# rabbitmq/ra

Measured on AMD Instinct MI355X. Metric: append_entries decisions/sec across N Raft groups; achieved HBM GB/s vs peak, higher is better.
Workload: dtype u64

## Files before the change

ra_amd/csrc/rgb_api.hip:

```cpp
#include <hip/hip_runtime.h>

#include <atomic>
#include <chrono>
#include <condition_variable>
#include <cstdio>
#include <cstdlib>
#include <cstring>
#include <memory>
#include <mutex>
#include <thread>
#include <new>
#include <vector>

#if defined(__x86_64__)
#include <emmintrin.h>
#endif

#include "rgb_internal.h"
#include "../../include/ra_gpu_batch_synth.h"

#define RGB_STREAM_COPY_MIN (1u << 20)
#ifndef RGB_COPY_STREAM_MIN
#define RGB_COPY_STREAM_MIN (2u << 20)
#endif
// ... 209 lines not shown
  if (s.d_res) (void)hipFree(s.d_res);
  if (s.h_stamps) (void)hipHostFree(s.h_stamps);
  if (s.d_stamps) (void)hipFree(s.d_stamps);
  if (s.h_plan) (void)hipHostFree(s.h_plan);
  if (s.d_plan) (void)hipFree(s.d_plan);
  if (s.h_rows) (void)hipHostFree(s.h_rows);
  if (s.d_rows) (void)hipFree(s.d_rows);
  if (s.d_ctl) (void)hipFree(s.d_ctl);
  if (s.h_ranges) (void)hipHostFree(s.h_ranges);
  if (s.d_ranges) (void)hipFree(s.d_ranges);
  s.h_ranges = s.d_ranges = nullptr; s.ranges_cap = 0;
  if (s.h_touched) (void)hipHostFree(s.h_touched);
  if (s.d_touched) (void)hipFree(s.d_touched);
  if (s.d_undo) (void)hipFree(s.d_undo);
  if (s.done) (void)hipEventDestroy(s.done);
  if (s.copied) (void)hipEventDestroy(s.copied);
  s.copied = nullptr;
  s.h_msgs = nullptr; s.h_dec = nullptr; s.d_msgs = nullptr; s.d_dec = nullptr; s.d_rpcs = nullptr; s.h_rpcs = nullptr;
  s.h_nrpc = nullptr; s.d_res = nullptr;
  s.h_stamps = s.d_stamps = nullptr; s.h_plan = s.d_plan = nullptr; s.h_rows = s.d_rows = nullptr; s.done = nullptr;
  s.d_ctl = nullptr; s.h_touched = s.d_touched = nullptr; s.d_undo = nullptr;
  s.h_pos = s.d_pos = nullptr;
}

void rgb_close(rgb_ctx *ctx) {
  if (!ctx) return;
  if (ctx->stream) (void)hipStreamSynchronize(ctx->stream);
  rgb_wal_release(ctx);
  rgb_seg_release(ctx);
  for (u32 k = 0; k < ctx->ring_size; ++k) free_slot(ctx->ring_mem[k]);
  if (ctx->dev.dbg_buf) (void)hipFree(ctx->dev.dbg_buf);
  if (ctx->dev.hot) (void)hipFree(ctx->dev.hot);
  if (ctx->dev.peers) (void)hipFree(ctx->dev.peers);
  if (ctx->dev.runs) (void)hipFree(ctx->dev.runs);
  if (ctx->dev.cond) (void)hipFree(ctx->dev.cond);
  if (ctx->dev.qry) (void)hipFree(ctx->dev.qry);
  if (ctx->dev.seq) (void)hipFree(ctx->dev.seq);
  if (ctx->d_stage) (void)hipFree(ctx->d_stage);
  if (ctx->h_stage) (void)hipHostFree(ctx->h_stage);
  if (ctx->d_rows) (void)hipFree(ctx->d_rows);
  if (ctx->d_sums) (void)hipFree(ctx->d_sums);
  if (ctx->lb_stream) { (void)hipStreamSynchronize(ctx->lb_stream); (void)hipStreamDestroy(ctx->lb_stream); }
  if (ctx->copy_stream) { (void)hipStreamSynchronize(ctx->copy_stream); (void)hipStreamDestroy(ctx->copy_stream); }
  if (ctx->d_lb_gather) (void)hipFree(ctx->d_lb_gather);
  if (ctx->h_lb_pinned) (void)hipHostFree(ctx->h_lb_pinned);
  if (ctx->lb_event) (void)hipEventDestroy(ctx->lb_event);
  if (ctx->d_synth) (void)hipFree(ctx->d_synth);
  if (ctx->d_synth_sent) (void)hipFree(ctx->d_synth_sent);
  if (ctx->d_train_ctl) (void)hipFree(ctx->d_train_ctl);
  if (ctx->d_seq_cnt) (void)hipFree(ctx->d_seq_cnt);

  if (ctx->stream) (void)hipStreamDestroy(ctx->stream);
  delete ctx;
}

int rgb_open(const rgb_config *cfg_in, rgb_ctx **out) {
  if (!out) return RGB_E_INVAL;
  *out = nullptr;
  rgb_config cfg;
  if (cfg_in) cfg = *cfg_in; else rgb_default_config(&cfg);
  if (cfg.abi_version != RGB_ABI_VERSION) return RGB_E_INVAL;
  if (cfg.max_runs < 2 || cfg.max_runs > RGB_MAX_RUNS) return RGB_E_INVAL;
  if (cfg.ring_slots < 1 || cfg.ring_slots > 64 || cfg.ring_capacity < 1) return RGB_E_INVAL;
  if (cfg.max_pipeline_count == 0) cfg.max_pipeline_count = RGB_DEFAULT_MAX_PIPELINE_COUNT;
  if (cfg.max_aer_batch == 0) cfg.max_aer_batch = RGB_AER_CHUNK_SIZE;
  if (cfg.max_aer_batch > 65535) return RGB_E_INVAL;
  int ndev = 0;
  hipError_t e = hipGetDeviceCount(&ndev);
  if (e != hipSuccess || ndev <= 0) return RGB_E_NODEVICE;
  if (cfg.device < 0 || cfg.device >= ndev) return RGB_E_INVAL;
  rgb_ctx *ctx = new (std::nothrow) rgb_ctx();
  if (!ctx) return RGB_E_NOMEM;
  ctx->cfg = cfg;
  memset(&ctx->dev, 0, sizeof ctx->dev);
  e = hipSetDevice(cfg.device);
  if (e == hipSuccess) e = hipStreamCreateWithFlags(&ctx->stream, hipStreamNonBlocking);
  if (e == hipSuccess) e = hipStreamCreateWithFlags(&ctx->copy_stream, hipStreamNonBlocking);

  if (e != hipSuccess) { delete ctx; return RGB_E_HIP; }
  *out = ctx;
  return RGB_OK;
}

uint32_t rgb_n_servers(const rgb_ctx *ctx) { return ctx ? ctx->dev.n_servers : 0; }

static int alloc_slot(rgb_ctx *ctx, rgb_slot &s) {
  const u32 cap = ctx->cfg.ring_capacity;
  HIPCHK(ctx, hipHostMalloc((void **)&s.h_msgs, (size_t)cap * (sizeof(rgb_msg) + sizeof(u32)), hipHostMallocDefault));
  HIPCHK(ctx, hipHostMalloc((void **)&s.h_dec, (size_t)cap * sizeof(rgb_decision), hipHostMallocDefault));
  HIPCHK(ctx, hipMalloc((void **)&s.d_msgs, (size_t)cap * (sizeof(rgb_msg) + sizeof(u32))));
  HIPCHK(ctx, hipMalloc((void **)&s.d_dec, (size_t)cap * sizeof(rgb_decision)));
  s.h_pos = reinterpret_cast<u32 *>(s.h_msgs + cap); s.d_pos = reinterpret_cast<u32 *>(s.d_msgs + cap);
  HIPCHK(ctx, hipMalloc((void **)&s.d_rpcs, (size_t)ctx->rpc_cap * sizeof(rgb_rpc)));
  HIPCHK(ctx, hipHostMalloc((void **)&s.h_rpcs, (size_t)ctx->rpc_cap * sizeof(rgb_rpc), hipHostMallocDefault));
  HIPCHK(ctx, hipEventCreateWithFlags(&s.done, hipEventDisableTiming));
  HIPCHK(ctx, hipEventCreateWithFlags(&s.copied, hipEventDisableTiming));
  HIPCHK(ctx, hipHostMalloc((void **)&s.h_nrpc, 64, hipHostMallocDefault));
  HIPCHK(ctx, hipMalloc((void **)&s.d_res, ((size_t)rgb_results_blocks(cap) + 1u) * sizeof(u32)));
  HIPCHK(ctx, hipMemsetAsync(s.d_res, 0, ((size_t)rgb_results_blocks(cap) + 1u) * sizeof(u32), ctx->stream));
  HIPCHK(ctx, hipHostMalloc((void **)&s.h_stamps, cap, hipHostMallocDefault));
  HIPCHK(ctx, hipMalloc((void **)&s.d_stamps, cap));
  HIPCHK(ctx, hipHostMalloc((void **)&s.h_plan, RGB_SUBMIT_TRAIN_ROUNDS * sizeof(rgb_train_tick), hipHostMallocDefault));
  HIPCHK(ctx, hipMalloc((void **)&s.d_plan, RGB_SUBMIT_TRAIN_ROUNDS * sizeof(rgb_train_tick)));
  s.rows_cap = (cap / 32u + 2u * RGB_N_CLASSES * RGB_SUBMIT_TRAIN_ROUNDS + 64u);
  HIPCHK(ctx, hipHostMalloc((void **)&s.h_rows, (size_t)s.rows_cap * RGB_SUBMIT_TRAIN_ROUNDS * sizeof(u32), hipHostMallocDefault));
  HIPCHK(ctx, hipMalloc((void **)&s.d_rows, (size_t)s.rows_cap * RGB_SUBMIT_TRAIN_ROUNDS * sizeof(u32)));
  HIPCHK(ctx, hipMalloc((void **)&s.d_ctl, RGB_TRAIN_CTL_WORDS * sizeof(u32)));
  HIPCHK(ctx, hipMemsetAsync(s.d_ctl, 0, RGB_TRAIN_CTL_WORDS * sizeof(u32), ctx->stream));
  HIPCHK(ctx, hipHostMalloc((void **)&s.h_touched, (size_t)cap * sizeof(u32), hipHostMallocDefault));
  HIPCHK(ctx, hipMalloc((void **)&s.d_touched, (size_t)cap * sizeof(u32)));
  return RGB_OK;
}

int rgb_upload_state(rgb_ctx *ctx, uint32_t first, uint32_t n, const rgb_server_state *in);

int rgb_register_groups(rgb_ctx *ctx, uint32_t n_groups, uint32_t n_members) {
  if (!ctx) return RGB_E_INVAL;
  if (ctx->registered) return RGB_E_STATE;
  if (n_members < 1 || n_members > RGB_MAX_MEMBERS || n_groups < 1) return RGB_E_INVAL;
  const uint64_t S64 = (uint64_t)n_groups * n_members;
  if (S64 > 0x7FFFFFFFull) return RGB_E_INVAL;
  const u32 S = (u32)S64;
  HIPCHK(ctx, hipSetDevice(ctx->cfg.device));
  rgb_dev &d = ctx->dev;
  d.n_servers = S; d.n_members = n_members; d.max_runs = ctx->cfg.max_runs;
  d.peer_stride = rgb_peer_stride(n_members);
  d.max_pipeline_count = ctx->cfg.max_pipeline_count;
  d.max_aer_batch = ctx->cfg.max_aer_batch;
  d.dbg = 0; d.dbg_buf = nullptr;
  d.synth_hint = ctx->synth_hint;
  d.fuse_pipeline = (ctx->cfg.flags & RGB_CFG_FUSE_PIPELINE) ? 1u : 0u;
  d.seq_ranges = nullptr; d.n_seq_ranges = 0;
#ifdef RGB_PROFILE
  { const char *e = getenv("RGB_DEBUG"); d.dbg = e ? (u32)atoi(e) : 0u; }
  if (d.dbg & 16u) {
    HIPCHK(ctx, hipMalloc((void **)&d.dbg_buf, (size_t)(S / 64 + 16) * 8 * sizeof(u64)));
    HIPCHK(ctx, hipMemsetAsync(d.dbg_buf, 0, (size_t)(S / 64 + 16) * 8 * sizeof(u64), ctx->stream));
  }
#endif
#ifdef RGB_X_DECLINE_HIST
  HIPCHK(ctx, hipMalloc((void **)&d.dbg_buf, 128 * sizeof(u64)));
  HIPCHK(ctx, hipMemsetAsync(d.dbg_buf, 0, 128 * sizeof(u64), ctx->stream));
#endif
#ifdef RGB_X_TRAIN_TIMELINE
  HIPCHK(ctx, hipMalloc((void **)&d.dbg_buf, (size_t)(1u << 20) * 8 * sizeof(u64)));
  HIPCHK(ctx, hipMemsetAsync(d.dbg_buf, 0, (size_t)(1u << 20) * 8 * sizeof(u64), ctx->stream));
#endif
  HIPCHK(ctx, hipMalloc((void **)&d.hot, (size_t)S * RGB_HOT_WORDS * sizeof(u64)));
  HIPCHK(ctx, hipMalloc((void **)&d.peers, (size_t)S * d.peer_stride * sizeof(u64)));
  HIPCHK(ctx, hipMalloc((void **)&d.runs, (size_t)S * d.max_runs * 2 * sizeof(u64)));
  HIPCHK(ctx, hipMalloc((void **)&d.cond, (size_t)S * 4 * sizeof(u64)));
  HIPCHK(ctx, hipMalloc((void **)&d.qry, (size_t)S * RGB_QRY_WORDS * sizeof(u64)));
  HIPCHK(ctx, hipMemsetAsync(d.runs, 0, (size_t)S * d.max_runs * 2 * sizeof(u64), ctx->stream));
  d.seq_stride = (((n_groups + RGB_TRAIN_SHARDS - 1u) / RGB_TRAIN_SHARDS) * n_members * RGB_SEQ_SPREAD + 255u) & ~255u;
  HIPCHK(ctx, hipMalloc((void **)&d.seq, (size_t)d.seq_stride * RGB_TRAIN_SHARDS));
  HIPCHK(ctx, hipMemsetAsync(d.seq, 0, (size_t)d.seq_stride * RGB_TRAIN_SHARDS, ctx->stream));
  ctx->stage_cap = S < 16384u ? S : 16384u;
  HIPCHK(ctx, hipMalloc((void **)&ctx->d_stage, (size_t)ctx->stage_cap * sizeof(rgb_server_state)));
  HIPCHK(ctx, hipHostMalloc((void **)&ctx->h_stage, (size_t)ctx->stage_cap * sizeof(rgb_server_state),
                            hipHostMallocDefault));
  HIPCHK(ctx, hipMalloc((void **)&ctx->d_rows, (size_t)n_groups * sizeof(rgb_leaderboard_row)));
  HIPCHK(ctx, hipMalloc((void **)&ctx->d_sums, (size_t)S * sizeof(u64)));
  ctx->rpc_stride = n_members > 1 ? n_members - 1 : 1;
  ctx->rpc_cap = ctx->cfg.ring_capacity * ctx->rpc_stride;
  ctx->ring_mem.reset(new (std::nothrow) rgb_slot[ctx->cfg.ring_slots]);
  if (!ctx->ring_mem) return RGB_E_NOMEM;
  ctx->ring_size = ctx->cfg.ring_slots;
  for (u32 k = 0; k < ctx->ring_size; ++k) {
    rgb_slot &s = ctx->ring_mem[k];
    int rc = alloc_slot(ctx, s);
    if (rc) return rc;
  }
  ctx->registered = true;
  std::vector<rgb_server_state> init(ctx->stage_cap);
  for (u32 base = 0; base < S; base += ctx->stage_cap) {
    u32 cnt = S - base < ctx->stage_cap ? S - base : ctx->stage_cap;
    for (u32 k = 0; k < cnt; ++k) {
      rgb_server_state &h = init[k];
      memset(&h, 0, sizeof h);
      h.snapshot_index = RGB_UNDEF; h.snapshot_term = RGB_UNDEF;
      h.pending_first = 1;
      for (unsigned i = 0; i < n_members; ++i) h.next_index[i] = 1;
      h.role = RGB_ROLE_FOLLOWER; h.self = (uint8_t)((base + k) % n_members);
      h.n_members = (uint8_t)n_members; h.voted_for = RGB_NONE; h.leader_id = RGB_NONE;
      h.cond_leader = RGB_NONE; h.n_runs = 1;
      h.present_mask = (uint8_t)((1u << n_members) - 1u); h.voter_mask = h.present_mask;
      h.status_mask = 0xFF;
    }
    int rc = rgb_upload_state(ctx, base, cnt, init.data());
    if (rc) return rc;
  }
  return RGB_OK;
}

static int validate_state(const rgb_ctx *ctx, const rgb_server_state &h) {
  if (h.n_members != ctx->dev.n_members) return RGB_E_INVAL;
  if (h.self >= RGB_MAX_MEMBERS) return RGB_E_INVAL;
  if (h.role > RGB_ROLE_AWAIT_CONDITION || h.cond_reason > RGB_COND_TRANSFER_LEADERSHIP) return RGB_E_INVAL;
  if (h.n_runs > RGB_MAX_RUNS || h.votes > 15) return RGB_E_INVAL;
  if (h.voted_for != RGB_NONE && h.voted_for >= RGB_MAX_MEMBERS) return RGB_E_INVAL;
  if (h.leader_id != RGB_NONE && h.leader_id >= RGB_MAX_MEMBERS) return RGB_E_INVAL;
  if (h.cond_leader != RGB_NONE && h.cond_leader >= RGB_MAX_MEMBERS) return RGB_E_INVAL;
  if (h.first_index <= h.last_index) {
    if (h.n_runs == 0 || h.run_start[0] != h.first_index) return RGB_E_INVAL;
    for (unsigned r = 1; r < h.n_runs; ++r)
      if (!(h.run_start[r] > h.run_start[r - 1] && h.run_start[r] <= h.last_index)) return RGB_E_INVAL;
    if (h.run_term[h.n_runs - 1] != h.last_term) return RGB_E_INVAL;
  }
  if (h.n_pending_old > 2) return RGB_E_INVAL;
  uint64_t above = h.pending_first;
  for (int k = (int)h.n_pending_old - 1; k >= 0; --k) {
    const uint64_t s = h.pending_old[k][0], e = h.pending_old[k][1];
    if (s > e || e == RGB_UNDEF || !(e + 1 < above)) return RGB_E_INVAL;
    above = s;
  }
  return RGB_OK;
}

int rgb_upload_state(rgb_ctx *ctx, uint32_t first, uint32_t n, const rgb_server_state *in) {
  if (!ctx || (!in && n)) return RGB_E_INVAL;
  if (!ctx->registered) return RGB_E_STATE;
  if ((uint64_t)first + n > ctx->dev.n_servers) return RGB_E_INVAL;
  for (u32 k = 0; k < n; ++k) {
    int rc = validate_state(ctx, in[k]);
    if (rc) return rc;
  }
  HIPCHK(ctx, hipSetDevice(ctx->cfg.device));
  rgb_stream_turn turn(ctx);
  if (turn.rc) return turn.rc;
  for (u32 base = 0; base < n; base += ctx->stage_cap) {
    u32 cnt = n - base < ctx->stage_cap ? n - base : ctx->stage_cap;
    memcpy(ctx->h_stage, in + base, (size_t)cnt * sizeof(rgb_server_state));
    HIPCHK(ctx, hipMemcpyAsync(ctx->d_stage, ctx->h_stage, (size_t)cnt * sizeof(rgb_server_state),
                               hipMemcpyHostToDevice, ctx->stream));
    int rc = rgb_launch_pack(ctx->dev, ctx->d_stage, first + base, cnt, ctx->stream);
    if (rc) { ctx->last_hip.store(rc, std::memory_order_relaxed); return RGB_E_HIP; }
    HIPCHK(ctx, hipStreamSynchronize(ctx->stream));
  }
  return RGB_OK;
}

int rgb_download_state(rgb_ctx *ctx, uint32_t first, uint32_t n, rgb_server_state *out) {
  if (!ctx || (!out && n)) return RGB_E_INVAL;
  if (!ctx->registered) return RGB_E_STATE;
  if ((uint64_t)first + n > ctx->dev.n_servers) return RGB_E_INVAL;
  HIPCHK(ctx, hipSetDevice(ctx->cfg.device));
  rgb_stream_turn turn(ctx);
  if (turn.rc) return turn.rc;
  for (u32 base = 0; base < n; base += ctx->stage_cap) {
    u32 cnt = n - base < ctx->stage_cap ? n - base : ctx->stage_cap;
    int rc = rgb_launch_unpack(ctx->dev, ctx->d_stage, first + base, cnt, ctx->stream);
    if (rc) { ctx->last_hip.store(rc, std::memory_order_relaxed); return RGB_E_HIP; }
    HIPCHK(ctx, hipMemcpyAsync(ctx->h_stage, ctx->d_stage, (size_t)cnt * sizeof(rgb_server_state),
                               hipMemcpyDeviceToHost, ctx->stream));
    HIPCHK(ctx, hipStreamSynchronize(ctx->stream));
    memcpy(out + base, ctx->h_stage, (size_t)cnt * sizeof(rgb_server_state));
  }
  return RGB_OK;
}

static int validate_msg(const rgb_ctx *ctx, const rgb_msg &m) {
  if (m.kind > RGB_MSG_KIND_MAX) return RGB_E_INVAL;
  if (m.kind == RGB_MSG_NOP) return RGB_OK;
  if (m.server >= ctx->dev.n_servers) return RGB_E_INVAL;
  if (m.from != RGB_NONE && m.from >= RGB_MAX_MEMBERS) return RGB_E_INVAL;
  if (m.kind == RGB_MSG_AER && m.n_run0 > m.n_entries) return RGB_E_INVAL;
  if (m.kind == RGB_MSG_WRITTEN && m.a > m.b) return RGB_E_INVAL;
  if (m.kind == RGB_MSG_WRITTEN && (m.flags & RGB_MF_SEQ2) &&
      !(m.run0_term <= m.run1_term && m.run1_term != RGB_UNDEF && m.run1_term + 1 < m.a)) return RGB_E_INVAL;
  if (m.kind == RGB_MSG_WRITTEN && (m.flags & RGB_MF_SEQX) && !(m.flags & RGB_MF_SEQ2)) return RGB_E_INVAL;
  return RGB_OK;
}
static int validate_seqx(const rgb_msg &m, const uint64_t *ranges, uint32_t n_ranges) {
  if (m.kind != RGB_MSG_WRITTEN || !(m.flags & RGB_MF_SEQX)) return RGB_OK;
  if (!ranges || m.n_entries == 0 || m.c > n_ranges || (uint64_t)m.c + m.n_entries > n_ranges) return RGB_E_INVAL;
  uint64_t prev_last = 0; bool have = false;
  for (uint32_t k = 0; k < m.n_entries; ++k) {
    const uint64_t f = ranges[2 * (m.c + k)], l = ranges[2 * (m.c + k) + 1];
    if (f > l || l == RGB_UNDEF || (have && !(prev_last + 1 < f))) return RGB_E_INVAL;
    prev_last = l; have = true;
  }
  return prev_last + 1 < m.run0_term ? RGB_OK : RGB_E_INVAL;
}

static int train_scratch(rgb_ctx *ctx);

#define RGB_FAULT_STAMP 1u
#define RGB_FAULT_SHARD 2u

static rgb_dev slot_dev(const rgb_ctx *ctx, const rgb_slot &s) {
  rgb_dev d = ctx->dev;
  d.seq_ranges = s.n_ranges ? s.d_ranges : nullptr;
  d.n_seq_ranges = s.n_ranges;
  return d;
}

static int enqueue_rounds(rgb_ctx *ctx, rgb_slot &s) {
  const rgb_dev dv = slot_dev(ctx, s);
  auto fail = [&](int lr) { ctx->last_hip.store(lr, std::memory_order_relaxed); return RGB_E_HIP; };
  for (u32 r = 0; r < s.n_rounds; ++r) {
    const u32 off = s.round_start[r], cnt = s.round_start[r + 1] - s.round_start[r];
    u32 cc[RGB_N_CLASSES], real = 0, before_written = 0;
    for (int c = 0; c < RGB_N_CLASSES; ++c) {
      cc[c] = s.round_cc[(size_t)r * RGB_N_CLASSES + c];
      real += cc[c];
      if (c < 2) before_written += cc[c];
// ... 1043 lines not shown
```

ra_amd/csrc/rgb_internal.h:

```cpp
#ifndef RGB_INTERNAL_H
#define RGB_INTERNAL_H

#include <stdint.h>
#include "../../include/ra_gpu_batch.h"

typedef unsigned long long u64;
typedef uint32_t u32;

#define RGB_HOT_WORDS 16
#define RGB_QRY_WORDS 16

#define HOT_CT    0
#define HOT_PK    1
#define HOT_LRT   2
#define HOT_PRS   3
#define HOT_CI    4
#define HOT_LA    5
#define HOT_LI    6
#define HOT_LT    7
#define HOT_SI    8
#define HOT_ST    9
#define HOT_FIRST 10
#define HOT_LRS   11
#define HOT_LWI   12
#define HOT_LWT   13
#define HOT_PRT   14
#define HOT_PEND  15
#define HOT_P_TERM  0
#define HOT_P_LRT   1
#define HOT_P_CI    2
#define HOT_P_LI    3
#define HOT_P_SI    4
#define HOT_P_FIRST 5
#define HOT_P_LW    6
#define HOT_P_PEND  7
#define PEER_MI(i, N) (2u * (unsigned)(i))
#define PEER_NI(i, N) (2u * (unsigned)(i) + 1u)
#define PEER_CS(i, N) (2u * (unsigned)(N) + (unsigned)(i))

#define PK_ROLE_SH      0
#define PK_COND_SH      3
#define PK_SELF_SH      5
#define PK_VOTES_SH     9
#define PK_NRUNS_SH     13
#define PK_NONVOTER_SH  18
#define PK_CONDTO_SH    19
#define PK_VOTED_SH     20
#define PK_LEADER_SH    24
#define PK_CONDLDR_SH   28
#define PK_PRESENT_SH   32
#define PK_VOTER_SH     40
#define PK_STATUS_SH    48
#define PK_QSELF_SH     56
#define PK_QPEER_SH     57
#define PK_BACKOFF_SH   58
#define PK_PENDX_SH     59
static inline __host__ __device__ unsigned pk_cond_reason(u64 pk) {
  const unsigned c = (unsigned)((pk >> PK_COND_SH) & 3ull), to = (unsigned)((pk >> PK_CONDTO_SH) & 1ull);
  return to == 0u ? c : c == RGB_COND_WAL_DOWN ? (unsigned)RGB_COND_WAL_DOWN_LEADER : (unsigned)RGB_COND_TRANSFER_LEADERSHIP;
}
static inline __host__ __device__ u64 pk_with_cond_reason(u64 pk, unsigned reason) {
  const u64 c = reason == RGB_COND_WAL_DOWN_LEADER ? (u64)RGB_COND_WAL_DOWN : reason == RGB_COND_TRANSFER_LEADERSHIP ? 0ull : (u64)reason;
  const u64 to = (reason == RGB_COND_WAL_DOWN_LEADER || reason == RGB_COND_TRANSFER_LEADERSHIP) ? 1ull : 0ull;
  return (pk & ~((3ull << PK_COND_SH) | (1ull << PK_CONDTO_SH))) | (c << PK_COND_SH) | (to << PK_CONDTO_SH);
}
#define QRY_PEND_LO     12
#define QRY_PEND_HI     14
#define QRY_BACKOFF     9
#define QRY_TOKEN       10
#define QRY_MACVER      11

#define RGB_N_CLASSES 15
static inline __host__ __device__ unsigned rgb_kind_rank(unsigned kind) {
  switch (kind) {
    case RGB_MSG_AER: return 0;
    case RGB_MSG_AER_REPLY: return 1;
    case RGB_MSG_WRITTEN: return 2;
    case RGB_MSG_APPEND: return 3;
    case RGB_MSG_PIPELINE_RPCS: return 4;
    case RGB_MSG_REQUEST_VOTE: return 5;
    case RGB_MSG_VOTE_RESULT: return 6;
    case RGB_MSG_AWAIT_TIMEOUT: return 7;
    case RGB_MSG_ELECTION_TIMEOUT: return 8;
    case RGB_MSG_PRE_VOTE_RPC: return 9;
    case RGB_MSG_PRE_VOTE_RESULT: return 10;
    case RGB_MSG_SNAPSHOT_WRITTEN: return 11;
    case RGB_MSG_HEARTBEAT_RPC: return 12;
    case RGB_MSG_HEARTBEAT_REPLY: return 13;
    case RGB_MSG_CONSISTENT_QUERY: return 14;
    case RGB_MSG_TRANSFER_LEADERSHIP: return 14;
    default: return 15;
  }
}
#define RGB_N_FAMILIES 32
static inline __host__ __device__ unsigned rgb_family(unsigned kind, unsigned flags) {
  return 2u * rgb_kind_rank(kind) + ((flags & RGB_MF_SUCCESS) ? 1u : 0u);
}
static inline unsigned rgb_class_of_kind(unsigned kind) { return rgb_kind_rank(kind); }

#define RGB_TRAIN_SHARDS 8u
#define RGB_N_BUCKETS ((RGB_N_CLASSES + 1u) * RGB_TRAIN_SHARDS * 2u)
#define RGB_TRAIN_CTL_WORDS (320u + 32u * 64u)
static inline __host__ __device__ unsigned rgb_shard_of_server(unsigned server, unsigned n_members) {
  return (server / n_members) & (RGB_TRAIN_SHARDS - 1u);
}
static inline __host__ __device__ unsigned rgb_bucket(unsigned kind, unsigned flags, unsigned server, unsigned n_members) {
  return (rgb_kind_rank(kind) * RGB_TRAIN_SHARDS + rgb_shard_of_server(server, n_members)) * 2u +
         ((flags & RGB_MF_SUCCESS) ? 1u : 0u);
}
static inline __host__ __device__ unsigned rgb_bucket_hinted(unsigned kind, unsigned flags, unsigned server,
                                                             unsigned n_members, bool off_steady) {
  const bool hinted_kind = kind == RGB_MSG_WRITTEN || kind == RGB_MSG_AER;
  return rgb_bucket(kind, flags, server, n_members) | ((hinted_kind && off_steady) ? 1u : 0u);
}
#ifndef RGB_SEQ_SPREAD
#define RGB_SEQ_SPREAD 1u
#endif
static inline __host__ __device__ unsigned rgb_seq_index(unsigned server, unsigned n_members, unsigned seq_stride) {
  const unsigned g = server / n_members, m = server - g * n_members;
  return (g & (RGB_TRAIN_SHARDS - 1u)) * seq_stride + ((g / RGB_TRAIN_SHARDS) * n_members + m) * RGB_SEQ_SPREAD;
}
#define RGB_TRAIN_MAX_TICKS 255u
#define RGB_N_PCLASSES (2u * RGB_N_CLASSES)
#define RGB_PC_SNAP RGB_N_PCLASSES
#define RGB_SNAP_LEAD 0.5f
struct rgb_train_tick {
  u32 n_rows;
  u32 msg_base;
  u32 snap;
  u32 pad[13];
  u32 off[RGB_N_PCLASSES][RGB_TRAIN_SHARDS];
  u32 cnt[RGB_N_PCLASSES][RGB_TRAIN_SHARDS];
};
#define RGB_SYNTH_FIXED_WORDS (RGB_N_FAMILIES + 2u * RGB_N_BUCKETS)
u32 rgb_synth_scratch_words(u32 n_groups);

static inline __host__ __device__ unsigned rgb_peer_stride(unsigned n_members) {
  return (3u * n_members + 7u) & ~7u;
}

struct rgb_dev {
  u64 *hot;
  u64 *peers;
  u64 *runs;
  u64 *cond;
  u64 *qry;
  u32 n_servers;
  u32 n_members;
  u32 max_runs;
  u32 peer_stride;
  u32 max_pipeline_count;
  u32 max_aer_batch;
  unsigned char *seq;
  u32 seq_stride;
  const u64 *seq_ranges;
  u32 n_seq_ranges;
  u32 fuse_pipeline;
  u32 synth_hint;
  u32 dbg;
  u64 *dbg_buf;
};

#define RGB_TICK_CLS_WRITTEN_SEQX 32
#define RGB_TICK_CLS_NOP 33
int rgb_launch_tick(const rgb_dev &dev, int cls, const rgb_msg *d_msgs, u32 n, const u32 *d_n,
                    rgb_decision *d_dec, rgb_rpc *d_rpcs, u32 rpc_slot_base, u32 msg_index_base, void *stream);
int rgb_launch_tick_classes(const rgb_dev &dev, const rgb_msg *d_msgs, const u32 counts[RGB_N_CLASSES],
                            const u32 *d_family_totals, u32 max_msgs, rgb_decision *d_dec, rgb_rpc *d_rpcs,
                            u32 rpc_slot_base, u32 msg_index_base, void *stream);
int rgb_launch_synth(const rgb_dev &dev, u64 seed, u64 tick, rgb_msg *d_msgs, u32 *d_scratch,
                     u32 *d_kind_counts, u32 *d_n, u32 *d_bucket_counts, unsigned char *d_stamps, unsigned char *d_sent,
                     void *stream);
int rgb_launch_train(const rgb_dev &dev, const rgb_msg *d_msgs, const unsigned char *d_stamps, u32 tick_stride,
                     const rgb_train_tick *d_plan, const u32 *d_row_tab, u32 n_ticks, u32 bpt, rgb_decision *d_dec,
                     rgb_rpc *d_rpcs, u32 rpc_ring, u32 index_base, u32 *d_ctl, u32 n_xcc, u32 n_blocks, void *stream,
                     const unsigned char *d_snap_stamps = nullptr, rgb_leaderboard_row *d_snap_rows = nullptr,
                     u32 tab_rpt = 0 );
u32 rgb_train_resident_blocks(unsigned n_members);
int rgb_launch_train_verify(u32 *d_ctl, void *stream);
int rgb_launch_train_seq(const rgb_dev &dev, const rgb_msg *d_msgs, u32 n, unsigned char *d_seq_cnt,
                         unsigned char *d_stamps, void *stream);
int rgb_launch_train_calibrate(u32 *d_out, void *stream);
u32 rgb_train_make_tick(const u32 *bucket_counts, unsigned n_members, rgb_train_tick *out, u32 *row_tab, u32 row_cap,
                        u32 snap_rows = 0);
int rgb_launch_train_plan(const u32 *d_bucket_counts, rgb_train_tick *d_ticks, u32 *d_rows, u32 rpt, u32 first_tick,
                          u32 n_ticks, u32 snapshot_every, u32 n_groups, u32 n_members, u32 *d_err, void *stream);
u32 rgb_train_rows_bound(u32 n_servers, u32 n_members, bool with_snapshot);
static inline u32 rgb_train_snap_rows(u32 n_groups) {
  return ((n_groups + RGB_TRAIN_SHARDS - 1u) / RGB_TRAIN_SHARDS + 63u) / 64u;
}
int rgb_launch_seq_bump(unsigned char *d_seq, unsigned char *d_out, u32 n_bytes, void *stream);
int rgb_launch_pack(const rgb_dev &dev, const rgb_server_state *d_in, u32 first, u32 n, void *stream);
int rgb_launch_unpack(const rgb_dev &dev, rgb_server_state *d_out, u32 first, u32 n, void *stream);
int rgb_launch_leaderboard(const rgb_dev &dev, rgb_leaderboard_row *d_rows, void *stream);
int rgb_launch_checksum(const rgb_dev &dev, u32 first, u32 n, u64 *d_out, void *stream);
int rgb_launch_stamp_rounds(const rgb_dev &dev, const rgb_msg *d_msgs, u32 n, unsigned char *d_stamps, void *stream);
u32 rgb_results_blocks(u32 n);
int rgb_launch_results(const rgb_decision *d_dec, const u32 *d_pos, u32 n, u32 cap, const rgb_rpc *d_rpcs, u32 rpc_stride, u32 *d_scratch,
                       const u32 *d_ctl, rgb_decision *out_dec, rgb_rpc *out_rpcs, u32 *out_hdr, void *stream);
u32 rgb_undo_pieces(const rgb_dev &dev);
int rgb_launch_undo(const rgb_dev &dev, const u32 *d_ids, u32 n, void *d_undo, u32 restore, void *stream);

#endif
```

ra_amd/csrc/rgb_kernels.hip:

```cpp
#include <hip/hip_runtime.h>
#include "rgb_internal.h"

#define UNDEF 0xFFFFFFFFFFFFFFFFull
#define SLOT_NONE4 0xFu

#ifdef RGB_PROFILE
#define RGB_KNOB(dev, bit) (((dev).dbg & (bit)) != 0)
#else
#define RGB_KNOB(dev, bit) false
#endif

#ifndef RGB_TICK_BLOCK
#define RGB_TICK_BLOCK 64
#endif
#ifndef RGB_CLASS_MIN_WAVES
#define RGB_CLASS_MIN_WAVES(N) ((N) <= 5 ? 4 : 3)
#endif
#ifndef RGB_MIN_WAVES
#define RGB_MIN_WAVES(N) 2
#endif

namespace {

#ifndef RGB_X_LEAD32
#define RGB_X_LEAD32 1
#endif
__host__ __device__ constexpr bool rgb_lead_class(int c) { return c == 1 || c == 3 || c == 4; }
#ifndef RGB_X_HINT
#define RGB_X_HINT 1
#endif
#ifndef RGB_X_HALFMSG
#define RGB_X_HALFMSG 1
#endif
__host__ __device__ constexpr bool rgb_half_msg_class(int c) {
  return RGB_X_HALFMSG && (c == 2 || c == 4 || c == 5 || c == 6 || c == 7 || c == 11 || c == 12 || c == 13 || c == 14);
}
__host__ __device__ __forceinline__ constexpr u32 rgb_class_slice(int c, unsigned n_members) {
  return (RGB_X_LEAD32 && rgb_lead_class(c) && ((3u * n_members + 7u) & ~7u) == 16u) ? 32u : (u32)RGB_TICK_BLOCK;
}
#ifndef RGB_X_NORPC
#define RGB_X_NORPC 0
#endif
#ifndef RGB_X_LEAD32_WIDE
#define RGB_X_LEAD32_WIDE 1
#endif
#ifndef RGB_TRAIN_RUNS_LDS
#define RGB_TRAIN_RUNS_LDS 1
#endif
__host__ __device__ __forceinline__ constexpr bool rgb_wide_peers(unsigned n_members) { return ((3u * n_members + 7u) & ~7u) == 24u; }
__host__ __device__ __forceinline__ constexpr u32 rgb_train_class_slice(int c, unsigned n_members) {
  return (RGB_X_LEAD32 && RGB_X_LEAD32_WIDE && RGB_TRAIN_RUNS_LDS && rgb_lead_class(c) && rgb_wide_peers(n_members)) ? 32u
                                                                                                                  : rgb_class_slice(c, n_members);
}


__device__ __forceinline__ void store16_nt(void *p, ulonglong2 v) {
  typedef unsigned v4u __attribute__((ext_vector_type(4)));
  v4u d;
  d.x = (unsigned)v.x; d.y = (unsigned)(v.x >> 32); d.z = (unsigned)v.y; d.w = (unsigned)(v.y >> 32);
  __builtin_nontemporal_store(d, reinterpret_cast<v4u *>(p));
}
#define ST16(ptr, val) do { *(ptr) = (val); } while (0)
#define ST8(ptr, val) do { *(ptr) = (val); } while (0)

#ifndef RGB_X_RPC_ST8
#define RGB_X_RPC_ST8 0
#endif
typedef unsigned long long rgb_u64x2_a8 __attribute__((ext_vector_type(2), aligned(8)));
__device__ __forceinline__ void store_rpc(rgb_rpc *slot, u64 w0, u64 w1, u64 w2, u64 w3, u64 w4, u64 w5, u64 w6) {
  u64 *o = reinterpret_cast<u64 *>(slot);
#if RGB_X_RPC_ST8 || defined(RGB_HOST_EMULATION)
  ST8(o + 0, w0); ST8(o + 1, w1); ST8(o + 2, w2); ST8(o + 3, w3); ST8(o + 4, w4); ST8(o + 5, w5); ST8(o + 6, w6);
#else
  rgb_u64x2_a8 a, b, c;
  a.x = w0; a.y = w1; b.x = w2; b.y = w3; c.x = w4; c.y = w5;
  *reinterpret_cast<rgb_u64x2_a8 *>(o + 0) = a;
  *reinterpret_cast<rgb_u64x2_a8 *>(o + 2) = b;
  *reinterpret_cast<rgb_u64x2_a8 *>(o + 4) = c;
  ST8(o + 6, w6);
#endif
}
#ifndef RGB_X_RPC_DEFER
#define RGB_X_RPC_DEFER 1
#endif
template <class Lane>
__device__ __forceinline__ void emit_rpc(Lane &L, rgb_rpc *rpcs, u32 slot_base, unsigned ord, u32 msg_index, u64 w1,
                                         u64 rp_idx, u64 rp_term, u64 new_ni) {
  if (rpcs == nullptr || RGB_X_NORPC) return;
  if (RGB_X_RPC_DEFER && L.rpc_stash != nullptr && ord < 4u) {
    L.rpc_stash[2u * ord] = make_ulonglong2(w1, rp_idx);
    L.rpc_stash[2u * ord + 1u] = make_ulonglong2(rp_term, new_ni);
    return;
  }
  store_rpc(rpcs + (size_t)slot_base + ord, (u64)msg_index | ((u64)L.server << 32), w1, L.ct, rp_idx, rp_term, L.ci, new_ni);
}

#if defined(RGB_X_MARK) && !defined(RGB_HOST_EMULATION)
#define RGB_MARK(what, rank) asm volatile("; RGB_MARK " what " %0" ::"n"(rank));
#else
#define RGB_MARK(what, rank)
#endif

enum { GLDS_DEFAULT = 0, GLDS_NT = 2, GLDS_SC1 = 16 };
template <int POLICY>
__device__ __forceinline__ void glds16(const void *g, void *lds_base) {
#ifdef RGB_HOST_EMULATION
  memcpy(static_cast<char *>(lds_base) + 16 * emu::lane(), g, 16);
#else
  __builtin_amdgcn_global_load_lds((const __attribute__((address_space(1))) void *)g,
                                   (__attribute__((address_space(3))) void *)lds_base, 16, 0, POLICY);
#endif
}
__device__ __forceinline__ void glds_wait() {
#ifndef RGB_HOST_EMULATION
  __builtin_amdgcn_s_waitcnt(0x0F70);
  asm volatile("" ::: "memory");
#endif
}

__device__ __forceinline__ void lds_barrier() {
#ifdef RGB_HOST_EMULATION
  __syncthreads();
#else
  __builtin_amdgcn_fence(__ATOMIC_RELEASE, "workgroup", "local");
  __builtin_amdgcn_s_barrier();
  __builtin_amdgcn_fence(__ATOMIC_ACQUIRE, "workgroup", "local");
#endif
}

typedef unsigned long long v2u64 __attribute__((ext_vector_type(2)));
template <bool NT>
__device__ __forceinline__ ulonglong2 ld16(const ulonglong2 *p) {
  if (NT) {
    v2u64 v = __builtin_nontemporal_load(reinterpret_cast<const v2u64 *>(p));
    return make_ulonglong2(v.x, v.y);
  }
  return *p;
}

__device__ __forceinline__ u64 ldg8(bool coh, const u64 *p) {
#ifndef RGB_HOST_EMULATION
  if (coh) return __hip_atomic_load(p, __ATOMIC_RELAXED, __HIP_MEMORY_SCOPE_AGENT);
#endif
  return *p;
}
__device__ __forceinline__ ulonglong2 ldg16(bool coh, const ulonglong2 *p) {
#ifndef RGB_HOST_EMULATION
  if (coh) {
    const u64 *q = reinterpret_cast<const u64 *>(p);
    const u64 x = __hip_atomic_load(q, __ATOMIC_RELAXED, __HIP_MEMORY_SCOPE_AGENT);
    const u64 y = __hip_atomic_load(q + 1, __ATOMIC_RELAXED, __HIP_MEMORY_SCOPE_AGENT);
    return make_ulonglong2(x, y);
  }
#endif
  return *p;
}

__device__ __forceinline__ u64 pk_get(u64 pk, int sh, int w) { return (pk >> sh) & ((1ull << w) - 1ull); }
__device__ __forceinline__ u64 pk_set(u64 pk, int sh, int w, u64 v) {
  const u64 m = ((1ull << w) - 1ull) << sh;
  return (pk & ~m) | ((v << sh) & m);
}
__device__ __forceinline__ unsigned slot8to4(unsigned s) { return s >= 8u ? SLOT_NONE4 : s; }
__device__ __forceinline__ unsigned slot4to8(unsigned s) { return s >= 8u ? (unsigned)RGB_NONE : s; }

template <bool COH, bool WC = false, bool SEQX = false>
struct LaneT {
  static constexpr bool coh = COH;
  static constexpr bool seqx_ok = SEQX;
  static constexpr bool walk_cache = WC;
  int wc_k;
  u64 wc_start, wc_term, wc_next;
  u64 ct, ci, la, li, lt, lwi, lwt, pk, si, st, first, lrs, lrt, prs, prt, pend;
  u64 token, macver;
  u32 server, n_entries, n_run0;
  unsigned kind, from, mflags, gap;
  u64 term, a, b, c, run0_term, run1_term;
  const u64 *seqx;
  u32 n_seqx;
  const u64 *runs;
  u64 *peers;
  const ulonglong2 *peers_lds;
  unsigned peers_swz;
  const ulonglong2 *runs_lds;
  ulonglong2 *rpc_stash;
  u32 max_runs;
  u32 flags;
  u32 inv;
  bool has_reply;
  unsigned reply_to;
  u64 r_term, r_next, r_last, r_lterm;
  u64 w_first, w_last;
  bool vote_reqs;
  unsigned n_runs;
  unsigned push_cnt;
  bool cond_dirty;
  u64 cr0, cr1, cr2, cr3;
  u64 po_floor, po_cut;
  u64 pmi[8], pni[8], pcs[8];
  unsigned dmi, dni, dcs;
  unsigned pdirty;
  unsigned dcs_ci;
  bool peers_loaded;
  u64 *qry_base;
  u64 qself, qp[8];
  bool q_loaded;
  unsigned q_dirty;
  unsigned hb_mask;
  unsigned cancel_mask;
#ifdef RGB_X_DECLINE_HIST
  const u64 *dbg_hist;
#endif
#ifdef RGB_PROFILE
  unsigned prof_nloads;
  bool prof_noprobe;
#endif
  u64 hb_term, hb_qi, q_consensus;
};

template <int N, class Lane>
__device__ __forceinline__ void load_peers(Lane &L) {
  if (L.peers_loaded) return;
  constexpr int PS = (3 * N + 7) & ~7;
  u64 w[PS];
  if ((PS == 16 || PS == 24) && L.peers_lds != nullptr) {
    const unsigned sw = PS == 24 ? L.peers_swz << 1 : L.peers_swz;
#pragma unroll
    for (int k = 0; k < PS / 2; ++k) {
      if (2 * k < 3 * N) { ulonglong2 v = L.peers_lds[(unsigned)k ^ sw]; w[2 * k] = v.x; w[2 * k + 1] = v.y; }
    }
  } else {
    const ulonglong2 *pp = reinterpret_cast<const ulonglong2 *>(L.peers);
#pragma unroll
    for (int k = 0; k < PS / 2; ++k) {
      if (2 * k < 3 * N) { ulonglong2 v = ldg16(L.coh, pp + k); w[2 * k] = v.x; w[2 * k + 1] = v.y; }
    }
  }
#pragma unroll
  for (int i = 0; i < N; ++i) { L.pmi[i] = w[PEER_MI(i, N)]; L.pni[i] = w[PEER_NI(i, N)]; L.pcs[i] = w[PEER_CS(i, N)]; }
  L.peers_loaded = true;
}

template <int N>
__device__ __forceinline__ u64 peer_get(const u64 (&a)[8], unsigned p) {
  u64 r = 0;
#pragma unroll
  for (int i = 0; i < N; ++i) r = ((unsigned)i == p) ? a[i] : r;
  return r;
}
template <int N>
__device__ __forceinline__ void peer_set(u64 (&a)[8], unsigned &dirty, unsigned p, u64 v) {
#pragma unroll
  for (int i = 0; i < N; ++i)
    if ((unsigned)i == p) { a[i] = v; dirty |= 1u << i; }
}

template <class Lane>
__device__ __forceinline__ unsigned prow_at(const Lane &L, unsigned w) { return (((w >> 1) ^ L.peers_swz) << 1) | (w & 1u); }
template <class Lane>
__device__ __forceinline__ u64 prow_get(const Lane &L, unsigned w) {
  return reinterpret_cast<const u64 *>(L.peers_lds)[prow_at(L, w)];
}
template <class Lane>
__device__ __forceinline__ void prow_set(Lane &L, unsigned w, u64 v) {
  const_cast<u64 *>(reinterpret_cast<const u64 *>(L.peers_lds))[prow_at(L, w)] = v;
  L.pdirty |= 1u << w;
}
template <int N, bool PL, class Lane> __device__ __forceinline__ u64 mi_get(const Lane &L, int i) { return PL ? prow_get(L, PEER_MI(i, N)) : L.pmi[i]; }
template <int N, bool PL, class Lane> __device__ __forceinline__ u64 ni_get(const Lane &L, int i) { return PL ? prow_get(L, PEER_NI(i, N)) : L.pni[i]; }
template <int N, bool PL, class Lane> __device__ __forceinline__ u64 cs_get(const Lane &L, int i) { return PL ? prow_get(L, PEER_CS(i, N)) : L.pcs[i]; }
template <int N, bool PL, class Lane> __device__ __forceinline__ void ni_set(Lane &L, int i, u64 v) {
  if (PL) prow_set(L, PEER_NI(i, N), v); else { L.pni[i] = v; L.dni |= 1u << i; }
}
template <int N, bool PL, class Lane> __device__ __forceinline__ u64 mi_of(const Lane &L, unsigned p) { return PL ? (p < (unsigned)N ? prow_get(L, PEER_MI(p, N)) : 0) : peer_get<N>(L.pmi, p); }
template <int N, bool PL, class Lane> __device__ __forceinline__ u64 ni_of(const Lane &L, unsigned p) { return PL ? (p < (unsigned)N ? prow_get(L, PEER_NI(p, N)) : 0) : peer_get<N>(L.pni, p); }
template <int N, bool PL, class Lane> __device__ __forceinline__ void mi_put(Lane &L, unsigned p, u64 v) {
  if (PL) { if (p < (unsigned)N) prow_set(L, PEER_MI(p, N), v); } else peer_set<N>(L.pmi, L.dmi, p, v);
}
template <int N, bool PL, class Lane> __device__ __forceinline__ void ni_put(Lane &L, unsigned p, u64 v) {
  if (PL) { if (p < (unsigned)N) prow_set(L, PEER_NI(p, N), v); } else peer_set<N>(L.pni, L.dni, p, v);
}

template <class Lane>
__device__ __forceinline__ bool range_nonempty(const Lane &L) { return L.first <= L.li; }

#define RGB_RUNS_LDS 8
#ifndef RGB_TRAIN_RUNS_LDS
#define RGB_TRAIN_RUNS_LDS 1
#endif
template <class Lane>
__device__ __forceinline__ ulonglong2 run_pair(const Lane &L, int k) {
  if (L.runs_lds != nullptr && k < RGB_RUNS_LDS) return L.runs_lds[(unsigned)k ^ L.peers_swz];
  return ldg16(L.coh, reinterpret_cast<const ulonglong2 *>(L.runs) + k);
}
template <class Lane>
__device__ __forceinline__ u64 run_word(const Lane &L, int i) {
#ifdef RGB_PROFILE
  const_cast<Lane &>(L).prof_nloads += 1;
#endif
  if (L.runs_lds != nullptr && i < 2 * RGB_RUNS_LDS) {
    const ulonglong2 v = L.runs_lds[(unsigned)(i >> 1) ^ L.peers_swz];
    return (i & 1) ? v.y : v.x;
  }
  return ldg8(L.coh, L.runs + i);
}

template <class Lane>
__device__ __forceinline__ int run_search(const Lane &L, u64 idx, u64 &term) {
  int k = (int)L.n_runs - 3;
  if (k < 0) return -1;
  if (Lane::walk_cache && L.wc_k >= 0 && L.wc_k <= k && idx >= L.wc_start && idx < L.wc_next) {
    term = L.wc_term;
    return L.wc_k;
  }
  ulonglong2 cur = run_pair(L, k);
  u64 upper = L.prs;
#pragma unroll 1
  for (; k >= 0; --k) {
    const ulonglong2 nxt = run_pair(L, k > 0 ? k - 1 : 0);
#ifdef RGB_PROFILE
    const_cast<Lane &>(L).prof_nloads += 2u;
#endif
    if (idx >= cur.x) {
      term = cur.y;
      if (Lane::walk_cache) {
        Lane &M = const_cast<Lane &>(L);
        M.wc_k = k; M.wc_start = cur.x; M.wc_term = cur.y; M.wc_next = upper;
      }
      return k;
    }
    upper = cur.x;
    cur = nxt;
  }
  return -1;
}

template <class Lane>
__device__ __forceinline__ u64 fetch_term(const Lane &L, u64 idx) {
  if (!(range_nonempty(L) && idx >= L.first && idx <= L.li)) return UNDEF;
  if (idx >= L.lrs) return L.lrt;
#ifdef RGB_PROFILE
  if (L.prof_noprobe) return L.lrt;
#endif
  if (L.n_runs >= 2 && idx >= L.prs) return L.prt;
  u64 term = UNDEF;
  run_search(L, idx, term);
  return term;
}

template <class Lane>
__device__ __forceinline__ u64 srv_fetch_term(const Lane &L, u64 idx) {
  u64 t = fetch_term(L, idx);
  if (t == UNDEF && L.si != UNDEF && L.si == idx) return L.st;
  return t;
}

template <class Lane>
__device__ __forceinline__ int find_run(const Lane &L, u64 idx) {
  if (L.n_runs == 0) return -1;
  if (idx >= L.lrs) return (int)L.n_runs - 1;
#ifdef RGB_PROFILE
  if (L.prof_noprobe) return (int)L.n_runs - 1;
#endif
  if (L.n_runs >= 2 && idx >= L.prs) return (int)L.n_runs - 2;
  u64 term;
  return run_search(L, idx, term);
}


template <class Lane>
__device__ __forceinline__ u64 next_log_index(const Lane &L) {
  if (range_nonempty(L)) return L.li + 1;
  if (L.si != UNDEF) return L.si + 1;
  return 0;
}

enum { HLE_OK = 0, HLE_MISMATCH = 1, HLE_MISSING = 2 };
template <class Lane>
__device__ __forceinline__ int has_log_entry_or_snapshot(const Lane &L, u64 idx, u64 term) {
  u64 t = fetch_term(L, idx);
  if (t == UNDEF) {
    if (L.si != UNDEF && L.si == idx) return L.st == term ? HLE_OK : HLE_MISMATCH;
    return HLE_MISSING;
  }
  return t == term ? HLE_OK : HLE_MISMATCH;
}

template <class Lane>
__device__ __forceinline__ unsigned role_of(const Lane &L) { return (unsigned)pk_get(L.pk, PK_ROLE_SH, 3); }
template <class Lane>
__device__ __forceinline__ unsigned self_of(const Lane &L) { return (unsigned)pk_get(L.pk, PK_SELF_SH, 4); }
template <class Lane>
__device__ __forceinline__ bool present(const Lane &L, unsigned i) {
  return i < 8u && ((L.pk >> (PK_PRESENT_SH + i)) & 1ull);
}
template <class Lane>
__device__ __forceinline__ bool voter(const Lane &L, unsigned i) { return (L.pk >> (PK_VOTER_SH + i)) & 1ull; }
template <class Lane>
__device__ __forceinline__ bool status_normal(const Lane &L, unsigned i) { return (L.pk >> (PK_STATUS_SH + i)) & 1ull; }

template <class Lane>
__device__ __forceinline__ void set_role(Lane &L, unsigned role) {
  unsigned old = role_of(L);
  if (old != role) L.flags |= RGB_F_ROLE_CHANGED;
  if (role == RGB_ROLE_FOLLOWER && old != RGB_ROLE_FOLLOWER) {
    L.pk = pk_set(L.pk, PK_STATUS_SH, 8, 0xFF);
    L.pk = pk_set(L.pk, PK_BACKOFF_SH, 1, 0);
  }
  if (role != RGB_ROLE_AWAIT_CONDITION) L.pk &= ~((3ull << PK_COND_SH) | (1ull << PK_CONDTO_SH));
  L.pk = pk_set(L.pk, PK_ROLE_SH, 3, role);
}

template <class Lane>
__device__ __forceinline__ void update_term_and_voted_for(Lane &L, u64 term, unsigned voted4) {
  unsigned cur = (unsigned)pk_get(L.pk, PK_VOTED_SH, 4);
  if (term == L.ct && voted4 == cur) return;
  L.flags |= RGB_F_PERSIST;
  L.ct = term;
  L.pk = pk_set(L.pk, PK_VOTED_SH, 4, voted4);
  if (pk_get(L.pk, PK_QPEER_SH, 1)) {
    L.pk = pk_set(L.pk, PK_QPEER_SH, 1, 0);
    if (L.q_loaded) {
#pragma unroll
      for (int i = 0; i < 8; ++i) L.qp[i] = 0;
    }
  }
}

template <class Lane>
__device__ __forceinline__ u64 *qry_row(const Lane &L) { return L.qry_base + (size_t)L.server * RGB_QRY_WORDS; }

template <int N, class Lane>
__device__ __forceinline__ void load_qry(Lane &L) {
  if (L.q_loaded) return;
  const ulonglong2 *qp = reinterpret_cast<const ulonglong2 *>(qry_row(L));
  u64 w[N + 2];
#pragma unroll
  for (int k = 0; k < (N + 2) / 2; ++k) { ulonglong2 v = ldg16(L.coh, qp + k); w[2 * k] = v.x; w[2 * k + 1] = v.y; }
  L.qself = w[0];
  if (pk_get(L.pk, PK_QPEER_SH, 1)) {
#pragma unroll
    for (int i = 0; i < N; ++i) L.qp[i] = w[1 + i];
  }
  L.q_loaded = true;
}

template <class Lane>
__device__ __forceinline__ void heartbeat_reply(Lane &L, u64 term, u64 query_index, unsigned to8) {
  L.has_reply = true;
  L.flags |= RGB_F_REPLY | RGB_F_REPLY_HEARTBEAT;
  L.r_term = term; L.r_next = query_index; L.r_last = 0; L.r_lterm = 0;
  L.reply_to = to8;
}
// ... 433 lines not shown
    if (c + 1 > L.pend) L.pend = c + 1;
    pend_canon(L);
  }
  pend_old_floor(L, c + 1);
  if (first_clause) {
    changed = !(L.lwi == c && L.lwt == term);
    L.lwi = c; L.lwt = term;
  }
  return 0;
}

template <class Lane>
__device__ __forceinline__ bool log_snapshot_written(Lane &L, u64 idx, u64 term) {
  if (!(range_nonempty(L) && idx >= L.first)) return false;
  bool changed = false;
  if (!(L.lwi > idx)) {
    changed = !(L.lwi == idx && L.lwt == term);
    L.lwi = idx; L.lwt = term;
  }
  if (idx >= L.li) {
    L.li = idx; L.lt = term; L.first = idx + 1; L.n_runs = 0;
  } else {
    const u64 nf = idx + 1;
    const int k = find_run(L, nf);
    u64 *runs = const_cast<u64 *>(L.runs);
    if (k > 0) {
      ulonglong2 *rp = reinterpret_cast<ulonglong2 *>(runs);
      const int n_mem = (int)L.n_runs - 2 - k;
#ifdef RGB_X_DECLINE_HIST
      atomicAdd(const_cast<u64 *>(L.dbg_hist) + 96 + (n_mem < 0 ? 0 : n_mem > 15 ? 15 : n_mem), 1ull);
#endif
#pragma unroll 1
      for (int i = 0; i < n_mem; i += 4) {
        ulonglong2 t0 = make_ulonglong2(0, 0), t1 = t0, t2 = t0, t3 = t0;
        t0 = ldg16(L.coh, rp + k + i);
        if (i + 1 < n_mem) t1 = ldg16(L.coh, rp + k + i + 1);
        if (i + 2 < n_mem) t2 = ldg16(L.coh, rp + k + i + 2);
        if (i + 3 < n_mem) t3 = ldg16(L.coh, rp + k + i + 3);
        ST16(rp + i, t0);
        if (i + 1 < n_mem) ST16(rp + i + 1, t1);
        if (i + 2 < n_mem) ST16(rp + i + 2, t2);
        if (i + 3 < n_mem) ST16(rp + i + 3, t3);
      }
      if ((int)L.n_runs - 2 >= k) ST16(rp + (L.n_runs - 2 - (unsigned)k), make_ulonglong2(L.prs, L.prt));
      ST16(rp + (L.n_runs - 1 - (unsigned)k), make_ulonglong2(L.lrs, L.lrt));
      L.n_runs -= (unsigned)k;
    }
    if (L.n_runs > 0) runs[0] = nf;
    if (L.lrs < nf) L.lrs = nf;
    if (L.n_runs == 2) L.prs = nf;
    L.first = nf;
  }
  L.si = idx; L.st = term;
  if (idx + 1 > L.pend) L.pend = idx + 1;
  pend_old_floor(L, idx + 1);
  pend_canon(L);
  return changed;
}


template <int N>
__device__ __forceinline__ u64 agreed_commit(const u64 (&v)[N], const bool (&use)[N], int n) {
  if (n <= 0) return UNDEF;
  u64 a[N];
#pragma unroll
  for (int i = 0; i < N; ++i) a[i] = use[i] ? v[i] : 0ull;
#pragma unroll
  for (int r = 0; r < N; ++r) {
#pragma unroll
    for (int i = r & 1; i + 1 < N; i += 2) {
      const bool sw = a[i + 1] > a[i];
      const u64 hi = sw ? a[i + 1] : a[i], lo = sw ? a[i] : a[i + 1];
      a[i] = hi; a[i + 1] = lo;
    }
  }
  const int k = n / 2;
  u64 res = a[0];
#pragma unroll
  for (int i = 1; i < N; ++i) res = (k == i) ? a[i] : res;
  return res;
}

template <int N, bool PL = false, class Lane>
__device__ __forceinline__ void evaluate_quorum(Lane &L) {
  u64 v[N + 1];
  bool use[N + 1];
  const unsigned self = self_of(L);
  int n = 1;
  v[N] = L.lwi; use[N] = true;
#pragma unroll
  for (int i = 0; i < N; ++i) {
    bool u = ((unsigned)i != self) && present(L, i) && voter(L, i);
    v[i] = mi_get<N, PL>(L, i); use[i] = u;
    n += u ? 1 : 0;
  }
  const u64 ci0 = L.ci;
  u64 p = agreed_commit<N + 1>(v, use, n);
  u64 t = srv_fetch_term(L, p);
  if (t != UNDEF && t == L.ct) L.ci = p;
  if (L.ci > ci0) L.flags |= RGB_F_AUX_EVAL;
  if (apply_to(L, L.ci)) L.flags |= RGB_F_APPLIED;
}

template <int N, bool EMIT, bool PL = false, class Lane>
__device__ __forceinline__ int pipeline_rpcs(Lane &L, bool force, u32 max_pipe, u32 max_batch, bool &more,
                             unsigned &n_out, rgb_rpc *rpcs, u32 slot_base, u32 msg_index) {
  const unsigned self = self_of(L);
  const u64 next_log = next_log_index(L);
  more = false;
  n_out = 0;
#pragma unroll
  for (int i = 0; i < N; ++i) {
    if ((unsigned)i == self || !present(L, i) || !status_normal(L, i)) continue;
    const u64 mi = mi_get<N, PL>(L, i), ni = ni_get<N, PL>(L, i), cis = cs_get<N, PL>(L, i);
    if (!(ni < next_log || cis < L.ci)) continue;
    long long inflight = (long long)(ni - mi) - 1;
    if (!(inflight < (long long)max_pipe || force)) continue;
    long long room = (long long)max_pipe - inflight;
    long long bs = (long long)max_batch < room ? (long long)max_batch : room;
    if (bs < 1) bs = 1;
    u64 prev = ni - 1;
    u64 prev_term = fetch_term(L, prev);
    u64 new_ni, rp_idx, rp_term;
    unsigned kind, n_ent = 0;
    if (prev_term == UNDEF && !(L.si != UNDEF && L.si == prev)) {
      if (L.si == UNDEF || !(ni == 0 || prev < L.si)) return RGB_INV_PIPELINE_PREV_UNDEFINED;
      kind = RGB_RPC_SNAPSHOT; rp_idx = L.si; rp_term = L.st; new_ni = L.si;
      if (EMIT) L.flags |= RGB_F_SEND_SNAPSHOT;
    } else {
      if (prev_term == UNDEF) prev_term = L.st;
      u64 to = prev + (u64)bs < L.li ? prev + (u64)bs : L.li;
      kind = RGB_RPC_AER; rp_idx = prev; rp_term = prev_term;
      n_ent = (unsigned)(to >= prev + 1 ? to - prev : 0);
      new_ni = to + 1;
    }
    if (!(new_ni >= ni)) return RGB_INV_NEXT_INDEX_REGRESSED;
    n_out += 1;
    long long new_inflight = (long long)(new_ni - mi) - 1;
    if (new_ni < next_log && new_inflight < (long long)max_pipe) more = true;
    if (EMIT) {
      ni_set<N, PL>(L, i, new_ni);
      L.dcs_ci |= 1u << i;
      emit_rpc(L, rpcs, slot_base, n_out - 1u, msg_index, (u64)(unsigned)i | ((u64)kind << 8) | ((u64)(n_ent & 0xFFFFu) << 16),
               rp_idx, rp_term, new_ni);
    }
  }
  return 0;
}


template <int N, class Lane>
__device__ __forceinline__ void become_leader(Lane &L) {
  const u64 ni = next_log_index(L);
  load_peers<N>(L);
#pragma unroll
  for (int i = 0; i < N; ++i) {
    if (!present(L, i)) continue;
    L.pmi[i] = 0; L.pni[i] = ni; L.pcs[i] = 0;
    L.dmi |= 1u << i; L.dni |= 1u << i; L.dcs |= 1u << i;
  }
  L.pk = pk_set(L.pk, PK_STATUS_SH, 8, 0xFF);
  L.pk = pk_set(L.pk, PK_BACKOFF_SH, 1, 0);
  set_leader_id(L, self_of(L));
  L.pk = pk_set(L.pk, PK_VOTES_SH, 4, 0);
  set_role(L, RGB_ROLE_LEADER);
  L.flags |= RGB_F_BECAME_LEADER;
}

template <int N, class Lane>
__device__ __forceinline__ void candidate_vote_granted(Lane &L) {
  unsigned nv = (unsigned)pk_get(L.pk, PK_VOTES_SH, 4) + 1;
  if (nv == required_quorum(L)) become_leader<N>(L);
  else L.pk = pk_set(L.pk, PK_VOTES_SH, 4, nv);
}

template <class Lane>
__device__ __forceinline__ void vote_requests(Lane &L, u64 term, bool pre) {
  L.flags &= ~(u32)RGB_F_PRE_VOTE_REQS;
  L.flags |= RGB_F_SEND_VOTE_REQUESTS | (pre ? RGB_F_PRE_VOTE_REQS : 0u);
  L.has_reply = false;
  L.r_term = term; L.r_next = pre ? L.token : 0; L.r_last = L.li; L.r_lterm = L.lt;
  L.vote_reqs = true;
}

template <int N, class Lane>
__device__ __forceinline__ void call_for_election_candidate(Lane &L) {
  const u64 new_term = L.ct + 1;
  update_term_and_voted_for(L, new_term, self_of(L));
  set_leader_id(L, SLOT_NONE4);
  L.pk = pk_set(L.pk, PK_VOTES_SH, 4, 0);
  set_role(L, RGB_ROLE_CANDIDATE);
  vote_requests(L, new_term, false);
  candidate_vote_granted<N>(L);
}

template <int N, class Lane>
__device__ __forceinline__ void call_for_election_pre_vote(Lane &L, u64 token) {
  update_term_and_voted_for(L, L.ct, self_of(L));
  set_leader_id(L, SLOT_NONE4);
  L.pk = pk_set(L.pk, PK_VOTES_SH, 4, 0);
  L.token = token;
  set_role(L, RGB_ROLE_PRE_VOTE);
  vote_requests(L, L.ct, true);
  if (!pk_get(L.pk, PK_NONVOTER_SH, 1)) {
    unsigned nv = (unsigned)pk_get(L.pk, PK_VOTES_SH, 4) + 1;
    if (nv == required_quorum(L)) call_for_election_candidate<N>(L);
    else L.pk = pk_set(L.pk, PK_VOTES_SH, 4, nv);
  }
}

template <class Lane>
__device__ __forceinline__ int process_pre_vote(Lane &L) {
  const u64 token = L.c;
  if (L.term >= L.ct) {
    update_term(L, L.term);
    const bool up = (L.b > L.lt) || (L.b == L.lt && L.a >= L.li);
    const u32 theirs = L.n_entries, ours = (u32)(L.macver & 0xFFFFFFFFull), eff = (u32)(L.macver >> 32);
    if (up && L.gap > RGB_PROTO_VERSION) {
      pre_vote_reply(L, L.term, token, false, L.from);
    } else if (up && (theirs == eff || (theirs >= eff && theirs <= ours))) {
      pre_vote_reply(L, L.term, token, true, L.from);
    } else if (up) {
      pre_vote_reply(L, L.term, token, false, L.from);
      L.flags |= RGB_F_START_ELECTION_TIMEOUT;
    } else if (role_of(L) == RGB_ROLE_FOLLOWER) {
      L.flags |= RGB_F_START_ELECTION_TIMEOUT;
    } else {
      pre_vote_reply(L, L.term, token, false, L.from);
    }
    return 0;
  }
  pre_vote_reply(L, L.ct, token, false, L.from);
  return 0;
}

template <int N, bool PL = false, class Lane>
__device__ __forceinline__ int make_all_rpcs(Lane &L, unsigned &n_out, rgb_rpc *rpcs, u32 slot_base,
                                             u32 msg_index, bool only_stale = false) {
  const unsigned self = self_of(L);
  update_heartbeat_rpc_effects<N>(L);
  if (!PL) load_peers<N>(L);
  n_out = 0;
  unsigned backoff = 0;
  if (!only_stale && pk_get(L.pk, PK_BACKOFF_SH, 1)) backoff = (unsigned)ldg8(L.coh, qry_row(L) + QRY_BACKOFF) & 0xFFu;
#pragma unroll
  for (int i = 0; i < N; ++i) {
    if ((unsigned)i == self || !present(L, i)) continue;
    if (!status_normal(L, i)) {
      if (!((backoff >> i) & 1u)) continue;
      L.cancel_mask |= 1u << i;
      L.flags |= RGB_F_CANCEL_SNAPSHOT_RETRY;
    }
    const u64 ni_i = ni_get<N, PL>(L, i);
    if (only_stale && !(mi_get<N, PL>(L, i) + 1 < ni_i || cs_get<N, PL>(L, i) < L.ci)) continue;
    const u64 prev = ni_i - 1;
    u64 prev_term = fetch_term(L, prev);
    u64 rp_idx, rp_term, new_ni;
    unsigned kind, n_ent = 0;
    if (prev_term == UNDEF && !(L.si != UNDEF && L.si == prev)) {
      if (L.si == UNDEF || !(ni_i == 0 || prev < L.si)) return RGB_INV_PIPELINE_PREV_UNDEFINED;
      kind = RGB_RPC_SNAPSHOT; rp_idx = L.si; rp_term = L.st; new_ni = L.si;
      L.flags |= RGB_F_SEND_SNAPSHOT;
    } else {
      if (prev_term == UNDEF) prev_term = L.st;
      u64 to = prev + 1 < L.li ? prev + 1 : L.li;
      kind = RGB_RPC_AER; rp_idx = prev; rp_term = prev_term;
      n_ent = (unsigned)(to >= prev + 1 ? to - prev : 0);
      new_ni = to + 1;
    }
    n_out += 1;
    emit_rpc(L, rpcs, slot_base, n_out - 1u, msg_index, (u64)(unsigned)i | ((u64)kind << 8) | ((u64)(n_ent & 0xFFFFu) << 16),
             rp_idx, rp_term, new_ni);
  }
  return 0;
}


template <class Lane>
__device__ __forceinline__ u32 drop_existing(const Lane &L) {
  if (L.n_entries == 0) return 0;
  const u64 base = L.a + 1 + (u64)L.gap;
  if (!range_nonempty(L) || base > L.li || base < L.first) return 0;
  u32 k = 0;
  for (int seg = 0; seg < 2; ++seg) {
    u32 cnt = seg == 0 ? L.n_run0 : L.n_entries - L.n_run0;
    if (seg == 0 && cnt > L.n_entries) cnt = L.n_entries;
    if (cnt == 0) continue;
    u64 s = base + k, e = s + cnt - 1;
    u64 t = seg == 0 ? L.run0_term : L.run1_term;
    if (s > L.li) return k;
    int r = find_run(L, s);
    if (r < 0) return k;
    const bool cached = Lane::walk_cache && r == L.wc_k;
    u64 rterm = ((unsigned)r == L.n_runs - 1) ? L.lrt : ((unsigned)r == L.n_runs - 2) ? L.prt :
                cached ? L.wc_term : run_word(L, 2 * r + 1);
    if (rterm != t) return k;
    u64 rend = ((unsigned)r == L.n_runs - 1) ? L.li : ((unsigned)r == L.n_runs - 2) ? L.lrs - 1 :
               ((unsigned)r == L.n_runs - 3) ? L.prs - 1 : cached ? L.wc_next - 1 : run_word(L, 2 * (r + 1)) - 1;
    if (rend >= e) { k += cnt; continue; }
    k += (u32)(rend - s + 1);
    return k;
  }
  return k;
}

template <class Lane>
__device__ __forceinline__ int follower_aer(Lane &L) {
// ... 440 lines not shown
      }
      return 0;
    }
    case RGB_MSG_SNAPSHOT_WRITTEN:
      log_snapshot_written(L, L.a, L.b);
      return 0;
    case RGB_MSG_HEARTBEAT_RPC:
      if (L.term >= L.ct) {
        update_term(L, L.term);
        L.pk = pk_set(L.pk, PK_VOTES_SH, 4, 0);
        set_role(L, RGB_ROLE_FOLLOWER);
        reprocess = true;
        return 0;
      }
      heartbeat_reply(L, L.ct, L.a, L.from);
      return 0;
    case RGB_MSG_HEARTBEAT_REPLY:
      if (L.term > L.ct) {
        update_term(L, L.term);
        L.pk = pk_set(L.pk, PK_VOTES_SH, 4, 0);
        set_role(L, RGB_ROLE_FOLLOWER);
        return 0;
      }
      L.flags |= RGB_F_UNHANDLED;
      return 0;
    case RGB_MSG_PRE_VOTE_RPC: return process_pre_vote(L);
    case RGB_MSG_ELECTION_TIMEOUT:
      call_for_election_pre_vote<N>(L, L.c);
      return 0;
    case RGB_MSG_TRANSFER_LEADERSHIP:
      call_reply(L, RGB_CALL_UNSUPPORTED, RGB_NONE);
      return 0;
    default: L.flags |= RGB_F_UNHANDLED; return 0;
  }
}

template <int N, class Lane>
__device__ __forceinline__ int handle_await_condition(Lane &L, bool &reprocess, const u64 *cond_row) {
  const bool wal_down = pk_get(L.pk, PK_COND_SH, 2) == RGB_COND_WAL_DOWN;
  const bool transfer = pk_cond_reason(L.pk) == RGB_COND_TRANSFER_LEADERSHIP;
  const bool can_write = (L.mflags & RGB_MF_CAN_WRITE) != 0;
  const unsigned back = pk_get(L.pk, PK_CONDTO_SH, 1) ? RGB_ROLE_LEADER : RGB_ROLE_FOLLOWER;
  switch (L.kind) {
    case RGB_MSG_REQUEST_VOTE:
      set_role(L, RGB_ROLE_FOLLOWER);
      reprocess = true;
      return 0;
    case RGB_MSG_AWAIT_TIMEOUT: {
      if (wal_down) {
        if (back == RGB_ROLE_LEADER && !can_write &&
            (pk_get(L.pk, PK_PRESENT_SH, 8) & ~(1ull << self_of(L))) != 0ull)
          L.flags |= RGB_F_TRANSFER_LEADERSHIP;
        set_role(L, back);
        return 0;
      }
      if (transfer) {
        set_role(L, RGB_ROLE_LEADER);
        return 0;
      }
      L.has_reply = true;
      L.flags |= RGB_F_REPLY | RGB_F_LEADER_MSG;
      L.r_term = ldg8(L.coh, cond_row); L.r_next = ldg8(L.coh, cond_row + 1);
      L.r_last = ldg8(L.coh, cond_row + 2); L.r_lterm = ldg8(L.coh, cond_row + 3);
      L.reply_to = slot4to8((unsigned)pk_get(L.pk, PK_CONDLDR_SH, 4));
      set_role(L, RGB_ROLE_FOLLOWER);
      return 0;
    }
    case RGB_MSG_WRITTEN:
      { bool changed; return log_written(L, L.term, L.a, L.b, changed); }
    case RGB_MSG_SNAPSHOT_WRITTEN:
      log_snapshot_written(L, L.a, L.b);
      return 0;
    case RGB_MSG_PRE_VOTE_RPC: return process_pre_vote(L);
    case RGB_MSG_ELECTION_TIMEOUT:
      if (pk_get(L.pk, PK_NONVOTER_SH, 1)) return 0;
      call_for_election_pre_vote<N>(L, L.c);
      return 0;
    case RGB_MSG_AER: {
      bool pred = false;
      if (wal_down) {
        pred = can_write;
      } else if (transfer) {
        pred = L.term > L.ct;
      } else if (L.term >= L.ct) {
        int h = has_log_entry_or_snapshot(L, L.a, L.b);
        if (h == HLE_OK) pred = true;
        else if (h == HLE_MISMATCH) pred = pk_get(L.pk, PK_COND_SH, 2) == RGB_COND_MISSING;
      }
      if (pred) { set_role(L, wal_down ? back : (unsigned)RGB_ROLE_FOLLOWER); reprocess = true; }
      return 0;
    }
    default:
      if (wal_down && can_write) { set_role(L, back); reprocess = true; }
      return 0;
  }
}

struct Dec { u64 w[8]; };

__device__ __forceinline__ void make_decision(Dec &d, u32 server, unsigned role, unsigned reply_to,
                                              unsigned n_rpcs, unsigned kind, u32 flags, u32 inv, u64 w2,
                                              u64 w3, u64 w4, u64 w5, u64 ci, u64 la, unsigned hb_mask = 0,
                                              unsigned cancel_mask = 0) {
  d.w[0] = (u64)server | ((u64)(role & 0xFF) << 32) | ((u64)(reply_to & 0xFF) << 40) |
           ((u64)(n_rpcs & 0xFF) << 48) | ((u64)(kind & 0xFF) << 56);
  d.w[1] = (u64)flags | ((u64)(inv & 0xFFFFu) << 32) | ((u64)(hb_mask & 0xFFu) << 48) |
           ((u64)(cancel_mask & 0xFFu) << 56);
  d.w[2] = w2; d.w[3] = w3; d.w[4] = w4; d.w[5] = w5; d.w[6] = ci; d.w[7] = la;
}

#ifndef RGB_X_COMPACT
#define RGB_X_COMPACT 1
#endif
__device__ __forceinline__ bool compact_decision(Dec &d) {
  if (!RGB_X_COMPACT) return false;
  const u32 flags = (u32)d.w[1];
  const unsigned kind = (unsigned)(d.w[0] >> 56);
  if ((d.w[1] >> 32) != 0ull || (flags & RGB_F_COMPACT)) return false;
  const u32 plain = RGB_F_LEADER_MSG | RGB_F_APPLIED | RGB_F_AUX_EVAL | RGB_F_PIPELINE;
  u64 A, B; u32 aux = 0;
  if ((flags & ~plain) == 0u && (kind == RGB_MSG_AER_REPLY || kind == RGB_MSG_WRITTEN)) {
    if ((d.w[2] | d.w[3] | d.w[4] | d.w[5]) != 0ull) return false;
    A = d.w[6]; B = d.w[7];
  } else if ((flags & ~plain) == RGB_F_WROTE && kind == RGB_MSG_AER) {
    const u64 fst = d.w[3], lst = d.w[4], la = d.w[7];
    if ((d.w[2] | d.w[5]) != 0ull || fst > lst || lst - fst > 0xFFFFull || la > lst || lst - la > 0xFFFFull) return false;
    A = lst; B = d.w[6];
    aux = (u32)(lst - fst) | ((u32)(lst - la) << 16);
  } else if ((flags & ~plain) == (RGB_F_REPLY | RGB_F_REPLY_SUCCESS) && (kind == RGB_MSG_AER || kind == RGB_MSG_WRITTEN)) {
    const u64 term = d.w[2], next = d.w[3], last = d.w[4], lterm = d.w[5], ci = d.w[6], la = d.w[7];
    if (next == 0ull) return false;
    A = next - 1ull; B = term;
    const u64 d1 = A - last, d2 = term - lterm, d3 = ci + 512ull - A, d4 = A + 1ull - la;
    if (last > A || d1 > 0xFFull || lterm > term || d2 > 0xFull || ci + 512ull < A || d3 > 0x3FFull || la > A + 1ull ||
        d4 > 0x3FFull)
      return false;
    aux = (u32)d1 | ((u32)d2 << 8) | ((u32)d3 << 12) | ((u32)d4 << 22);
  } else {
    return false;
  }
  d.w[1] = (u64)(flags | RGB_F_COMPACT) | ((u64)aux << 32);
  d.w[2] = A; d.w[3] = B;
  return true;
}

template <int N, int KIND, bool PRE = false, bool TR = false, bool SEQXP = (KIND < 0)>
__device__ __forceinline__ void process_message(const rgb_dev &dev, const ulonglong2 m0, const ulonglong2 m1,
                                                const ulonglong2 m2, const ulonglong2 m3, u32 i,
                                                rgb_rpc *__restrict__ rpcs, u32 rpc_slot_base,
                                                u32 msg_index_base, Dec &out, u64 *t_loaded = nullptr,
                                                const ulonglong2 *pre = nullptr, unsigned swz = 0,
                                                const ulonglong2 *prepeers = nullptr,
                                                const ulonglong2 *preruns = nullptr, ulonglong2 *rpc_stash = nullptr) {
  LaneT<TR, (N >= 6 && KIND == RGB_MSG_AER), SEQXP> L;
  L.rpc_stash = rpc_stash;
  L.wc_k = -1; L.wc_start = L.wc_term = L.wc_next = 0;
  L.server = (u32)(m0.x & 0xFFFFFFFFull);
  const unsigned wire_kind = (unsigned)((m0.x >> 32) & 0xFF);
  L.kind = KIND >= 0 ? (unsigned)KIND : wire_kind;
  L.from = (unsigned)((m0.x >> 40) & 0xFF);
  L.mflags = (unsigned)((m0.x >> 48) & 0xFF);
  L.gap = (unsigned)((m0.x >> 56) & 0xFF);
  L.term = m0.y; L.a = m1.x; L.b = m1.y; L.c = m2.x;
  L.n_entries = (u32)(m2.y & 0xFFFFFFFFull);
  L.n_run0 = (u32)(m2.y >> 32);
  L.run0_term = m3.x; L.run1_term = m3.y;
  if (L.n_run0 > L.n_entries) L.n_run0 = L.n_entries;

  if (L.kind == RGB_MSG_NOP) {
    make_decision(out, L.server, 0, RGB_NONE, 0, 0, 0, 0, 0, 0, 0, 0, 0, 0);
    return;
  }
  if (L.server >= dev.n_servers || wire_kind != L.kind) {
    make_decision(out, L.server, 0xFF, RGB_NONE, 0, wire_kind, RGB_F_UNHANDLED, 0, 0, 0, 0, 0, 0, 0);
    return;
  }
  u64 *hot = dev.hot + (size_t)L.server * RGB_HOT_WORDS;
  const ulonglong2 *hp = reinterpret_cast<const ulonglong2 *>(hot);
  ulonglong2 h0, h1, h2, h3, h4, h5, h6, h7;
  if (RGB_KNOB(dev, 8u)) { h0 = h1 = h2 = h3 = h4 = h5 = h6 = h7 = make_ulonglong2(0, 0); h0.y = 0x1Full << PK_PRESENT_SH; }
  else if (PRE) {
    h0 = pre[HOT_P_TERM ^ swz]; h1 = pre[HOT_P_CI ^ swz]; h2 = pre[HOT_P_LI ^ swz]; h3 = pre[HOT_P_LW ^ swz];
    h4 = pre[HOT_P_SI ^ swz]; h5 = pre[HOT_P_FIRST ^ swz]; h6 = pre[HOT_P_LRT ^ swz]; h7 = pre[HOT_P_PEND ^ swz];
  } else {
    h0 = ldg16(TR, hp + HOT_P_TERM); h1 = ldg16(TR, hp + HOT_P_CI); h2 = ldg16(TR, hp + HOT_P_LI); h3 = ldg16(TR, hp + HOT_P_LW);
    h4 = ldg16(TR, hp + HOT_P_SI); h5 = ldg16(TR, hp + HOT_P_FIRST); h6 = ldg16(TR, hp + HOT_P_LRT); h7 = ldg16(TR, hp + HOT_P_PEND);
  }
#ifdef RGB_PROFILE
  L.prof_noprobe = RGB_KNOB(dev, 32u); L.prof_nloads = 0;
#endif
#ifdef RGB_X_DECLINE_HIST
  L.dbg_hist = dev.dbg_buf;
#endif
  if (decltype(L)::seqx_ok) { L.seqx = dev.seq_ranges; L.n_seqx = dev.n_seq_ranges; } else { L.seqx = nullptr; L.n_seqx = 0; }
  L.qry_base = dev.qry;
  L.q_loaded = false; L.q_dirty = 0; L.hb_mask = 0;
  L.qself = 0; L.hb_term = L.hb_qi = L.q_consensus = 0; L.cancel_mask = 0;
#pragma unroll
  for (int i = 0; i < 8; ++i) L.qp[i] = 0;
  L.runs = dev.runs + (size_t)L.server * dev.max_runs * 2;
  L.peers = dev.peers + (size_t)L.server * dev.peer_stride;
  L.max_runs = dev.max_runs;
  L.peers_loaded = false; L.dmi = L.dni = L.dcs = 0; L.dcs_ci = 0;
  L.peers_lds = prepeers; L.peers_swz = swz; L.pdirty = 0;
  L.runs_lds = preruns;
#ifndef RGB_X_COMMIT_WAIT
#define RGB_X_COMMIT_WAIT 1
#endif
#ifndef RGB_X_PL
#define RGB_X_PL 0
#endif
#ifndef RGB_X_PL_TICK
#define RGB_X_PL_TICK 1
#endif
#ifndef RGB_X_REREAD_TICK
#define RGB_X_REREAD_TICK 1
#endif
  constexpr bool PL = (TR ? RGB_X_PL : RGB_X_PL_TICK) && PRE && rgb_class_slice(1, (unsigned)N) == 32u &&
                      (KIND == RGB_MSG_AER_REPLY || KIND == RGB_MSG_APPEND || KIND == RGB_MSG_PIPELINE_RPCS);
  if (!PL && (L.kind == RGB_MSG_AER_REPLY || L.kind == RGB_MSG_APPEND || L.kind == RGB_MSG_PIPELINE_RPCS ||
              L.kind == RGB_MSG_TRANSFER_LEADERSHIP) &&
      !RGB_KNOB(dev, 64u)) {
    load_peers<N>(L);
  }
#ifdef RGB_PROFILE
  if (RGB_KNOB(dev, 64u)) {
#pragma unroll
    for (int i = 0; i < 8; ++i) { L.pmi[i] = 0; L.pni[i] = 1; L.pcs[i] = 0; }
    L.peers_loaded = true;
  }
#endif
  if (t_loaded && RGB_KNOB(dev, 16u)) {
#ifndef RGB_HOST_EMULATION
    asm volatile("s_waitcnt vmcnt(0)" ::"v"(h0.x), "v"(h6.y) : "memory");
#endif
    *t_loaded = wall_clock64();
  }
  L.ct = h0.x; L.pk = h0.y; L.ci = h1.x; L.la = h1.y; L.li = h2.x; L.lt = h2.y; L.lwi = h3.x;
  L.lwt = h3.y; L.si = h4.x; L.st = h4.y; L.first = h5.x; L.lrs = h5.y; L.lrt = h6.x;
  L.prs = h6.y; L.prt = h7.x; L.pend = h7.y; L.vote_reqs = false;
  constexpr bool TM = KIND < 0 || KIND == RGB_MSG_ELECTION_TIMEOUT || KIND == RGB_MSG_PRE_VOTE_RPC ||
                      KIND == RGB_MSG_PRE_VOTE_RESULT;
  u64 token0 = 0;
  L.token = 0; L.macver = 0;
  if (TM && (L.kind == RGB_MSG_ELECTION_TIMEOUT || L.kind == RGB_MSG_PRE_VOTE_RPC || L.kind == RGB_MSG_PRE_VOTE_RESULT)) {
    const ulonglong2 tm = ldg16(TR, reinterpret_cast<const ulonglong2 *>(qry_row(L) + QRY_TOKEN));
    L.token = token0 = tm.x; L.macver = tm.y;
  }
  L.flags = 0; L.inv = 0; L.has_reply = false; L.reply_to = RGB_NONE;
  L.r_term = L.r_next = L.r_last = L.r_lterm = 0; L.w_first = L.w_last = 0;
  L.n_runs = (unsigned)pk_get(L.pk, PK_NRUNS_SH, 5);
  L.push_cnt = 0;
  L.cond_dirty = false; L.cr0 = L.cr1 = L.cr2 = L.cr3 = 0;
  L.po_floor = 0; L.po_cut = UNDEF;

  const unsigned role0 = role_of(L);
  const unsigned pkhi0 = (unsigned)(L.pk >> 56);
  const u64 ci0 = L.ci, la0 = L.la;
  const unsigned n_runs0 = L.n_runs;
  unsigned n_rpcs = 0;
  int rc = 0;
  unsigned role1 = role0;
  bool go = true;
  if (role0 == RGB_ROLE_AWAIT_CONDITION) {
    bool reprocess = false;
    rc = handle_await_condition<N>(L, reprocess, dev.cond + (size_t)L.server * 4);
    go = !rc && reprocess;
    if (go) { L.flags |= RGB_F_REPROCESSED; role1 = role_of(L); }
  }
  if (go && role1 != RGB_ROLE_FOLLOWER) {
    bool reprocess = false;
    switch (role1) {
      case RGB_ROLE_LEADER:          rc = handle_leader<N, PL>(L, reprocess, dev, rpcs,
                                                           (rpc_slot_base + i) * (N > 1 ? N - 1 : 1),
                                                           msg_index_base + i, n_rpcs); break;
      case RGB_ROLE_CANDIDATE:       rc = handle_candidate<N>(L, reprocess); break;
      case RGB_ROLE_PRE_VOTE:        rc = handle_pre_vote<N>(L, reprocess); break;
      default: L.flags |= RGB_F_UNHANDLED; break;
    }
    go = !rc && reprocess;
    if (go) L.flags |= RGB_F_REPROCESSED;
  }
  if (go) rc = handle_follower<N>(L);
#ifdef RGB_PROFILE
  if (t_loaded && RGB_KNOB(dev, 16u)) t_loaded[2] = wall_clock64();
#endif
  if (rc) {
    make_decision(out, L.server, role0, RGB_NONE, 0, L.kind, RGB_F_INVARIANT, (u32)rc, 0, 0, 0, 0, ci0, la0);
    return;
  }

#if RGB_X_COMMIT_WAIT && !defined(RGB_HOST_EMULATION)
  __builtin_amdgcn_s_waitcnt(0x0F70);
#endif
  if (RGB_KNOB(dev, 1u)) { L.n_runs = n_runs0; L.push_cnt = 0; L.cond_dirty = false; L.dmi = L.dni = L.dcs = 0; L.dcs_ci = 0; L.pdirty = 0; }
  if (L.n_runs != n_runs0 || L.push_cnt) {
    u64 *runs = const_cast<u64 *>(L.runs);
    unsigned nr = L.n_runs;
    if (nr > L.max_runs) {
      unsigned shift = nr - L.max_runs;
      unsigned in_mem = nr - L.push_cnt;
      for (unsigned k = shift; k < in_mem; ++k) {
        const u64 rs = ldg8(TR, runs + 2 * k), rt = ldg8(TR, runs + 2 * k + 1);
        runs[2 * (k - shift)] = rs;
        runs[2 * (k - shift) + 1] = rt;
      }
      nr = L.max_runs;
      L.flags |= RGB_F_RUNS_OVERFLOW;
      u64 nf;
      if (L.push_cnt >= nr) nf = (L.push_cnt == 2 && nr == 2) ? L.prs : L.lrs;
      else nf = ldg8(TR, runs);
      L.first = nf;
      L.n_runs = nr;
    }
    if (L.push_cnt == 2) { runs[2 * (nr - 2)] = L.prs; runs[2 * (nr - 2) + 1] = L.prt; }
    if (L.push_cnt >= 1) { runs[2 * (nr - 1)] = L.lrs; runs[2 * (nr - 1) + 1] = L.lrt; }
  }
  L.pk = pk_set(L.pk, PK_NRUNS_SH, 5, L.n_runs);
  if (L.cond_dirty) {
    ulonglong2 *cp = reinterpret_cast<ulonglong2 *>(dev.cond + (size_t)L.server * 4);
    ST16(cp, make_ulonglong2(L.cr0, L.cr1));
    ST16(cp + 1, make_ulonglong2(L.cr2, L.cr3));
  }
  const bool q_reset = ((pkhi0 >> (PK_QPEER_SH - 56)) & 1u) && !pk_get(L.pk, PK_QPEER_SH, 1);
  if ((L.q_dirty || q_reset) && !RGB_KNOB(dev, 1u)) {
    u64 *q = qry_row(L);
    if (L.q_dirty & 1u) q[0] = L.qself;
#pragma unroll
    for (int i = 0; i < N; ++i)
      if (q_reset || (L.q_dirty & (2u << i))) q[1 + i] = L.qp[i];
  }
  if (PL) {
    if (L.pdirty | L.dcs_ci) {
#pragma unroll
      for (int w = 0; w < 2 * N; ++w)
        if (L.pdirty & (1u << w)) ST8(L.peers + w, prow_get(L, (unsigned)w));
#pragma unroll
      for (int k = 0; k < N; ++k)
        if (L.dcs_ci & (1u << k)) ST8(L.peers + PEER_CS(k, N), L.ci);
    }
  } else if (L.dmi | L.dni | L.dcs | L.dcs_ci) {
#pragma unroll
    for (int k = 0; k < N; ++k) {
      if (L.dmi & (1u << k)) ST8(L.peers + PEER_MI(k, N), L.pmi[k]);
      if (L.dni & (1u << k)) ST8(L.peers + PEER_NI(k, N), L.pni[k]);
      if (L.dcs & (1u << k)) ST8(L.peers + PEER_CS(k, N), L.pcs[k]);
      else if (L.dcs_ci & (1u << k)) ST8(L.peers + PEER_CS(k, N), L.ci);
    }
  }
  if (((pkhi0 >> (PK_PENDX_SH - 56)) & 1u) && !RGB_KNOB(dev, 1u)) {
    u64 *q = qry_row(L);
    u64 s0 = ldg8(TR, q + QRY_PEND_LO), e0 = ldg8(TR, q + QRY_PEND_LO + 1), s1 = ldg8(TR, q + QRY_PEND_HI),
        e1 = ldg8(TR, q + QRY_PEND_HI + 1);
    if (s0 < L.po_floor) s0 = L.po_floor;
    if (s1 < L.po_floor) s1 = L.po_floor;
    if (L.po_cut != UNDEF) {
      if (L.po_cut == 0) { s0 = 1; e0 = 0; s1 = 1; e1 = 0; }
      else { if (e0 >= L.po_cut) e0 = L.po_cut - 1; if (e1 >= L.po_cut) e1 = L.po_cut - 1; }
    }
    bool v0 = s0 <= e0, v1 = s1 <= e1;
    const bool newest = range_nonempty(L) && L.pend <= L.li;
    if (v1 && newest && e1 + 1 == L.pend) { L.pend = s1; v1 = false; }
    else if (v1 && !newest && range_nonempty(L) && e1 == L.li) { L.pend = s1; v1 = false; }
    else if (!v1 && v0 && newest && e0 + 1 == L.pend) { L.pend = s0; v0 = false; }
    else if (!v1 && v0 && !newest && range_nonempty(L) && e0 == L.li) { L.pend = s0; v0 = false; }
    if (!v1 && v0) { s1 = s0; e1 = e0; v1 = true; v0 = false; }
    q[QRY_PEND_LO] = v0 ? s0 : 1; q[QRY_PEND_LO + 1] = v0 ? e0 : 0;
    q[QRY_PEND_HI] = v1 ? s1 : 1; q[QRY_PEND_HI + 1] = v1 ? e1 : 0;
    L.pk = pk_set(L.pk, PK_PENDX_SH, 1, v1 ? 1 : 0);
  }
  ulonglong2 *ho = reinterpret_cast<ulonglong2 *>(hot);
  if (!RGB_KNOB(dev, 1u)) {
  if (L.n_runs < 2) { L.prs = 0; L.prt = 0; }
#ifndef RGB_X_REREAD
#define RGB_X_REREAD 0
#endif
  if ((TR ? RGB_X_REREAD : RGB_X_REREAD_TICK) && PRE) {
#pragma unroll
    for (int k = 0; k < 8; ++k) {
      const ulonglong2 o = pre[(unsigned)k ^ swz];
      ulonglong2 n;
      switch (k) {
        case HOT_P_TERM: n = make_ulonglong2(L.ct, L.pk); break;
        case HOT_P_CI: n = make_ulonglong2(L.ci, L.la); break;
        case HOT_P_LI: n = make_ulonglong2(L.li, L.lt); break;
        case HOT_P_LW: n = make_ulonglong2(L.lwi, L.lwt); break;
        case HOT_P_SI: n = make_ulonglong2(L.si, L.st); break;
        case HOT_P_FIRST: n = make_ulonglong2(L.first, L.lrs); break;
        case HOT_P_LRT: n = make_ulonglong2(L.lrt, L.prs); break;
        default: n = make_ulonglong2(L.prt, L.pend); break;
      }
      if (n.x != o.x || n.y != o.y) ST16(ho + k, n);
    }
  } else {
  if (L.ct != h0.x || L.pk != h0.y) ST16(ho + HOT_P_TERM, make_ulonglong2(L.ct, L.pk));
  if (L.ci != h1.x || L.la != h1.y) ST16(ho + HOT_P_CI, make_ulonglong2(L.ci, L.la));
  if (L.li != h2.x || L.lt != h2.y) ST16(ho + HOT_P_LI, make_ulonglong2(L.li, L.lt));
  if (L.lwi != h3.x || L.lwt != h3.y) ST16(ho + HOT_P_LW, make_ulonglong2(L.lwi, L.lwt));
  if (L.si != h4.x || L.st != h4.y) ST16(ho + HOT_P_SI, make_ulonglong2(L.si, L.st));
  if (L.first != h5.x || L.lrs != h5.y) ST16(ho + HOT_P_FIRST, make_ulonglong2(L.first, L.lrs));
  if (L.lrt != h6.x || L.prs != h6.y) ST16(ho + HOT_P_LRT, make_ulonglong2(L.lrt, L.prs));
  if (L.prt != h7.x || L.pend != h7.y) ST16(ho + HOT_P_PEND, make_ulonglong2(L.prt, L.pend));
  }
  if (TM && L.token != token0) ST8(qry_row(L) + QRY_TOKEN, L.token);
  }

  u64 w2 = 0, w3 = 0, w4 = 0, w5 = 0;
  if (L.has_reply || L.vote_reqs) { w2 = L.r_term; w3 = L.r_next; w4 = L.r_last; w5 = L.r_lterm; }
  else if (L.flags & RGB_F_WROTE) { w3 = L.w_first; w4 = L.w_last; }
  if ((L.flags & RGB_F_SEND_HEARTBEATS) || L.kind == RGB_MSG_CONSISTENT_QUERY) { w2 = L.hb_term; w5 = L.hb_qi; }
  if (L.flags & RGB_F_QUERY_QUORUM) w3 = L.q_consensus;
  make_decision(out, L.server, role_of(L), L.has_reply ? L.reply_to : (unsigned)RGB_NONE, n_rpcs, L.kind,
                L.flags, 0, w2, w3, w4, w5, L.ci, L.la, L.hb_mask, L.cancel_mask);
#ifdef RGB_PROFILE
  if (t_loaded) { t_loaded[1] = L.prof_nloads; if (RGB_KNOB(dev, 16u)) t_loaded[3] = wall_clock64(); }
#endif
}

template <int N, bool TR>
__device__ __forceinline__ void fuse_pipeline_step(const rgb_dev &dev, Dec &d, u32 i, rgb_rpc *__restrict__ rpcs,
                                                   u32 rpc_slot_base, u32 msg_index_base) {
#ifndef RGB_HOST_EMULATION
  __builtin_amdgcn_s_waitcnt(0x0F70);
  asm volatile("" ::: "memory");
#endif
  const u64 m0x = (d.w[0] & 0xFFFFFFFFull) | ((u64)RGB_MSG_PIPELINE_RPCS << 32) | ((u64)RGB_NONE << 40);
  Dec e;
  process_message<N, RGB_MSG_PIPELINE_RPCS, false, TR>(dev, make_ulonglong2(m0x, 0), make_ulonglong2(0, 0), make_ulonglong2(0, 0),
                                                        make_ulonglong2(0, 0), i, rpcs, rpc_slot_base, msg_index_base, e);
  const u32 ef = (u32)e.w[1];
  if (ef & (RGB_F_INVARIANT | RGB_F_UNHANDLED)) return;
  d.w[0] = (d.w[0] & ~(0xFFull << 48)) | (e.w[0] & (0xFFull << 48));
  d.w[1] = (d.w[1] & ~(u64)RGB_F_PIPELINE) | (u64)ef;
}
__device__ __forceinline__ bool fuse_wanted(const rgb_dev &dev, const Dec &d) {
  const unsigned kind = (unsigned)(d.w[0] >> 56), role = (unsigned)((d.w[0] >> 32) & 0xFF);
  return dev.fuse_pipeline && ((u32)d.w[1] & RGB_F_PIPELINE) && !((u32)d.w[1] & RGB_F_INVARIANT) && role == RGB_ROLE_LEADER &&
         (kind == RGB_MSG_AER_REPLY || kind == RGB_MSG_WRITTEN);
}

#ifndef RGB_X_FAST
#define RGB_X_FAST 1
#endif
#if defined(RGB_X_DECLINE_HIST) && !defined(RGB_HOST_EMULATION)
#define FP_DECLINE(cls, code) do { atomicAdd(dev.dbg_buf + (cls) * 32 + (code), 1ull); return false; } while (0)
#define FP_TAKEN(cls) atomicAdd(dev.dbg_buf + (cls) * 32, 1ull)
#else
#define FP_DECLINE(cls, code) return false
#define FP_TAKEN(cls) do { } while (0)
#endif

#ifndef RGB_X_PAIR_STORE
#define RGB_X_PAIR_STORE 1
#endif
struct PairSt {
  ulonglong2 *p;
  ulonglong2 a, b;
  unsigned m;
};
__device__ __forceinline__ void pair_record(PairSt *ps, ulonglong2 *p, bool sa, const ulonglong2 a, bool sb, const ulonglong2 b) {
  if (RGB_X_PAIR_STORE && ps != nullptr) {
    ps->p = p; ps->a = a; ps->b = b; ps->m = (sa ? 1u : 0u) | (sb ? 2u : 0u);
  } else {
    if (sa) ST16(p, a);
    if (sb) ST16(p + 1, b);
  }
}
__device__ __forceinline__ u64 shfl64(u64 v, int src) {
  return (u64)(u32)__shfl((int)(u32)v, src, 64) | ((u64)(u32)__shfl((int)(u32)(v >> 32), src, 64) << 32);
}
__device__ __forceinline__ void pair_store(const PairSt &st, u32 lane) {
  const int t = (int)(threadIdx.x & ~63u) + (int)(lane & ~1u);
#pragma unroll
  for (int k = 0; k < 2; ++k) {
    const int src = t + k;
    const u64 pp = shfl64((u64)(uintptr_t)st.p, src);
    const unsigned m = (unsigned)__shfl((int)st.m, src, 64);
    const bool second = (lane & 1u) != 0u;
    const u64 ax = shfl64(st.a.x, src), ay = shfl64(st.a.y, src), bx = shfl64(st.b.x, src), by = shfl64(st.b.y, src);
    if (m & (second ? 2u : 1u))
      ST16(reinterpret_cast<ulonglong2 *>((uintptr_t)pp) + (second ? 1 : 0), second ? make_ulonglong2(bx, by) : make_ulonglong2(ax, ay));
  }
}

__device__ __forceinline__ bool fast_aer(const rgb_dev &dev, const ulonglong2 m0, const ulonglong2 m1, const ulonglong2 m2,
                                         const ulonglong2 m3, const ulonglong2 *pre, unsigned swz, Dec &out,
                                         PairSt *pst = nullptr) {
  const u32 server = (u32)(m0.x & 0xFFFFFFFFull);
  const unsigned wire_kind = (unsigned)((m0.x >> 32) & 0xFF), from = (unsigned)((m0.x >> 40) & 0xFF);
  const unsigned mflags = (unsigned)((m0.x >> 48) & 0xFF), gap = (unsigned)((m0.x >> 56) & 0xFF);
  const u32 n_entries = (u32)(m2.y & 0xFFFFFFFFull), n_run0 = (u32)(m2.y >> 32);
  if (wire_kind != RGB_MSG_AER || server >= dev.n_servers || from >= 8u || mflags != 0) FP_DECLINE(0, 1);
  if (gap != 0) FP_DECLINE(0, 2);
  if (n_run0 < n_entries) FP_DECLINE(0, 4);
  const ulonglong2 h0 = pre[HOT_P_TERM ^ swz], h1 = pre[HOT_P_CI ^ swz], h2 = pre[HOT_P_LI ^ swz], h3 = pre[HOT_P_LW ^ swz],
                   h5 = pre[HOT_P_FIRST ^ swz], h6 = pre[HOT_P_LRT ^ swz], h7 = pre[HOT_P_PEND ^ swz];
  const u64 ct = h0.x, pk = h0.y, la = h1.y, li = h2.x, lt = h2.y, lwi = h3.x, first = h5.x, lrs = h5.y, lrt = h6.x,
            pend = h7.y;
  if (pk_get(pk, PK_ROLE_SH, 3) != RGB_ROLE_FOLLOWER) FP_DECLINE(0, 5);
  if (pk_get(pk, PK_LEADER_SH, 4) != from) FP_DECLINE(0, 6);
  if (pk_get(pk, PK_PENDX_SH, 1) || pk_get(pk, PK_NRUNS_SH, 5) == 0) FP_DECLINE(0, 7);
  const u64 term = m0.y, pli = m1.x, plt = m1.y, leader_commit = m2.x, eterm = m3.x;
  if (term != ct) FP_DECLINE(0, 8);
  if (!(first <= li) || li == UNDEF) FP_DECLINE(0, 9);
  if (pli != li) FP_DECLINE(0, 10);
  if (li < lrs) FP_DECLINE(0, 11);
  if (plt != lrt) FP_DECLINE(0, 12);
  if (lt != lrt) FP_DECLINE(0, 13);
  if (n_entries != 0 && eterm != lrt) FP_DECLINE(0, 14);
  if (la > li + 1 || lwi > li || pend > li + 1) FP_DECLINE(0, 15);
  if (pk_get(pk, PK_NRUNS_SH, 5) < 2 && (h6.y | h7.x) != 0) FP_DECLINE(0, 16);
  FP_TAKEN(0);
  const u64 fst = li + 1, lst = li + n_entries;
  u32 flags = RGB_F_LEADER_MSG;
  const u64 ci = leader_commit;
  u64 nla = la;
  const u64 at = lst < ci ? lst : ci;
  if (at > la) { nla = at; flags |= RGB_F_APPLIED | RGB_F_AUX_EVAL; }
  ulonglong2 *ho = reinterpret_cast<ulonglong2 *>(dev.hot + (size_t)server * RGB_HOT_WORDS);
  static_assert(HOT_P_LI == HOT_P_CI + 1 && (HOT_P_CI & 1) == 0, "commit and last_index pieces: one aligned 32-byte unit");
  pair_record(pst, ho + HOT_P_CI, ci != h1.x || nla != la, make_ulonglong2(ci, nla), n_entries != 0, make_ulonglong2(li + n_entries, lt));
  if (n_entries == 0) {
    make_decision(out, server, RGB_ROLE_FOLLOWER, from, 0, RGB_MSG_AER, flags | RGB_F_REPLY | RGB_F_REPLY_SUCCESS, 0, term,
                  li + 1, lwi, h3.y, ci, nla);
    return true;
  }
  flags |= RGB_F_WROTE;
  make_decision(out, server, RGB_ROLE_FOLLOWER, RGB_NONE, 0, RGB_MSG_AER, flags, 0, 0, fst, lst, 0, ci, nla);
  return true;
}

__device__ __forceinline__ bool fast_written(const rgb_dev &dev, const ulonglong2 m0, const ulonglong2 m1,
                                             const ulonglong2 *pre, unsigned swz, Dec &out, PairSt *pst = nullptr) {
  const u32 server = (u32)(m0.x & 0xFFFFFFFFull);
  const unsigned wire_kind = (unsigned)((m0.x >> 32) & 0xFF), mflags = (unsigned)((m0.x >> 48) & 0xFF);
  if (wire_kind != RGB_MSG_WRITTEN || server >= dev.n_servers || mflags != 0) FP_DECLINE(2, 1);
  const ulonglong2 h0 = pre[HOT_P_TERM ^ swz], h1 = pre[HOT_P_CI ^ swz], h2 = pre[HOT_P_LI ^ swz], h3 = pre[HOT_P_LW ^ swz],
                   h4 = pre[HOT_P_SI ^ swz], h5 = pre[HOT_P_FIRST ^ swz], h6 = pre[HOT_P_LRT ^ swz], h7 = pre[HOT_P_PEND ^ swz];
  const u64 ct = h0.x, pk = h0.y, li = h2.x, si = h4.x, first = h5.x, lrs = h5.y, lrt = h6.x, pend = h7.y;
  const unsigned l4 = (unsigned)pk_get(pk, PK_LEADER_SH, 4);
  if (pk_get(pk, PK_ROLE_SH, 3) != RGB_ROLE_FOLLOWER) FP_DECLINE(2, 2);
  if (l4 == SLOT_NONE4) FP_DECLINE(2, 3);
  if (pk_get(pk, PK_PENDX_SH, 1) || pk_get(pk, PK_NRUNS_SH, 5) == 0) FP_DECLINE(2, 4);
  const u64 term = m0.y, from = m1.x, to = m1.y;
  if (!(first <= li) || li == UNDEF || from > to) FP_DECLINE(2, 5);
  if (to > li) FP_DECLINE(2, 6);
  if (to < lrs) FP_DECLINE(2, 7);
  if (to < first) FP_DECLINE(2, 8);
  if (lrt != term) FP_DECLINE(2, 9);
  if (si != UNDEF && si >= first) FP_DECLINE(2, 10);
  if (pend > li + 1) FP_DECLINE(2, 11);
  if (pk_get(pk, PK_NRUNS_SH, 5) < 2 && (h6.y | h7.x) != 0) FP_DECLINE(2, 12);
  if (pend <= li && pend <= to && pend < from) FP_DECLINE(2, 13);
  FP_TAKEN(2);
  u64 npend = pend;
  if (pend <= li && to + 1 > pend) npend = to + 1;
  const bool changed = !(h3.x == to && h3.y == term);
  ulonglong2 *ho = reinterpret_cast<ulonglong2 *>(dev.hot + (size_t)server * RGB_HOT_WORDS);
  static_assert(HOT_P_PEND == HOT_P_LW + 1 && (HOT_P_LW & 1) == 0, "last_written and pending pieces: one aligned 32-byte unit");
  pair_record(pst, ho + HOT_P_LW, changed, make_ulonglong2(to, term), npend != pend, make_ulonglong2(h7.x, npend));
  u32 flags = 0;
  u64 w2 = 0, w3 = 0, w4 = 0, w5 = 0;
  unsigned reply_to = RGB_NONE;
  if (changed) {
    flags = RGB_F_REPLY | RGB_F_REPLY_SUCCESS;
    w2 = ct; w3 = li + 1; w4 = to; w5 = term; reply_to = slot4to8(l4);
  }
  make_decision(out, server, RGB_ROLE_FOLLOWER, reply_to, 0, RGB_MSG_WRITTEN, flags, 0, w2, w3, w4, w5, h1.x, h1.y);
  return true;
}

template <int N, bool TR = false, bool PROW = false>
__device__ __forceinline__ bool fast_aer_reply(const rgb_dev &dev, const ulonglong2 m0, const ulonglong2 m1,
                                               const ulonglong2 *pre, unsigned swz, Dec &out,
                                               const ulonglong2 *prow = nullptr,
                                               const ulonglong2 *rrow = nullptr) {
  const u32 server = (u32)(m0.x & 0xFFFFFFFFull);
  const unsigned wire_kind = (unsigned)((m0.x >> 32) & 0xFF), peer = (unsigned)((m0.x >> 40) & 0xFF);
  const unsigned mflags = (unsigned)((m0.x >> 48) & 0xFF);
  const ulonglong2 h0 = pre[HOT_P_TERM ^ swz], h1 = pre[HOT_P_CI ^ swz], h2 = pre[HOT_P_LI ^ swz], h3 = pre[HOT_P_LW ^ swz],
                   h4 = pre[HOT_P_SI ^ swz], h5 = pre[HOT_P_FIRST ^ swz], h6 = pre[HOT_P_LRT ^ swz], h7 = pre[HOT_P_PEND ^ swz];
  const u64 ct = h0.x, pk = h0.y, ci0 = h1.x, la = h1.y, li = h2.x, lwi = h3.x, si = h4.x, st = h4.y, first = h5.x,
            lrs = h5.y, lrt = h6.x, prs = h6.y, prt = h7.x;
  const unsigned present = (unsigned)pk_get(pk, PK_PRESENT_SH, 8), voters = (unsigned)pk_get(pk, PK_VOTER_SH, 8);
  const unsigned self = (unsigned)pk_get(pk, PK_SELF_SH, 4), n_runs = (unsigned)pk_get(pk, PK_NRUNS_SH, 5);
#if defined(RGB_X_DECLINE_HIST) && !defined(RGB_HOST_EMULATION)
  if (wire_kind != RGB_MSG_AER_REPLY || server >= dev.n_servers || peer >= (unsigned)N) FP_DECLINE(1, 1);
  if (mflags != RGB_MF_SUCCESS) FP_DECLINE(1, 2);
  if (dev.fuse_pipeline) FP_DECLINE(1, 9);
  if (pk_get(pk, PK_ROLE_SH, 3) != RGB_ROLE_LEADER) FP_DECLINE(1, 3);
  if (m0.y != ct) FP_DECLINE(1, 4);
  if (!((present >> peer) & 1u)) FP_DECLINE(1, 5);
  if (n_runs < 2 && (h6.y | h7.x) != 0) FP_DECLINE(1, 6);
#else
  const bool ok = (wire_kind == RGB_MSG_AER_REPLY) & (server < dev.n_servers) & (peer < (unsigned)N) &
                  (mflags == RGB_MF_SUCCESS) & (dev.fuse_pipeline == 0u) &
                  (pk_get(pk, PK_ROLE_SH, 3) == RGB_ROLE_LEADER) & (m0.y == ct) & (((present >> (peer & 7u)) & 1u) != 0u) &
                  !((n_runs < 2) & ((h6.y | h7.x) != 0));
  if (!ok) return false;
#endif
  u64 *peers = dev.peers + (size_t)server * dev.peer_stride;
  u64 wm[N], wn[N];
  if (PROW || prow != nullptr) {
    const unsigned psw = rgb_wide_peers((unsigned)N) ? swz << 1 : swz;
#pragma unroll
    for (int k = 0; k < N; ++k) { const ulonglong2 v = prow[(unsigned)k ^ psw]; wm[k] = v.x; wn[k] = v.y; }
  } else {
    const ulonglong2 *pp = reinterpret_cast<const ulonglong2 *>(peers);
#pragma unroll
    for (int k = 0; k < N; ++k) { const ulonglong2 v = ldg16(TR, pp + k); wm[k] = v.x; wn[k] = v.y; }
  }
  u64 mi_new = 0, ni_new = 0; bool mi_dirty = false, ni_dirty = false;
  if (PROW) {
    const unsigned psw = rgb_wide_peers((unsigned)N) ? swz << 1 : swz;
    const ulonglong2 pv = prow[peer ^ psw];
    mi_dirty = m1.y > pv.x; ni_dirty = m1.x > pv.y;
    mi_new = mi_dirty ? m1.y : pv.x; ni_new = ni_dirty ? m1.x : pv.y;
#pragma unroll
    for (int i = 0; i < N; ++i) wm[i] = ((unsigned)i == peer) ? mi_new : wm[i];
  } else {
#pragma unroll
    for (int i = 0; i < N; ++i) {
      if ((unsigned)i != peer) continue;
      mi_new = wm[i]; ni_new = wn[i];
      if (m1.y > wm[i]) { mi_new = m1.y; mi_dirty = true; wm[i] = m1.y; }
      if (m1.x > wn[i]) { ni_new = m1.x; ni_dirty = true; }
    }
  }
  u64 v[N + 1]; bool use[N + 1]; int n = 1;
  v[N] = lwi; use[N] = true;
#pragma unroll
  for (int i = 0; i < N; ++i) {
    const bool u = ((unsigned)i != self) && ((present >> i) & 1u) && ((voters >> i) & 1u);
    v[i] = wm[i]; use[i] = u; n += u ? 1 : 0;
  }
  const u64 p = agreed_commit<N + 1>(v, use, n);
  u64 t = UNDEF;
  if (first <= li && p >= first && p <= li) {
    if (p >= lrs) t = lrt;
    else if (n_runs >= 2 && p >= prs) t = prt;
    else {
      bool found = false;
      const ulonglong2 *rt = reinterpret_cast<const ulonglong2 *>(dev.runs + (size_t)server * dev.max_runs * 2u);
      const int lds_runs = rrow != nullptr ? RGB_RUNS_LDS : 0;
#pragma unroll 1
      for (int k = (int)n_runs - 3; k >= lds_runs && !found; --k) {
        const ulonglong2 r = ldg16(TR, rt + k);
        if (p >= r.x) { t = r.y; found = true; }
      }
      if (rrow != nullptr) {
#pragma unroll
        for (int k = RGB_RUNS_LDS - 1; k >= 0; --k) {
          if (!found && (unsigned)k + 3u <= n_runs) {
            const ulonglong2 r = rrow[(unsigned)k ^ swz];
            if (p >= r.x) { t = r.y; found = true; }
          }
        }
      }
      if (!found) FP_DECLINE(1, 8);
    }
  }
  FP_TAKEN(1);
  if (t == UNDEF && si != UNDEF && si == p) t = st;
  u64 ci = ci0, nla = la;
  u32 flags = RGB_F_PIPELINE;
  if (t != UNDEF && t == ct) ci = p;
  if (ci > ci0) flags |= RGB_F_AUX_EVAL;
  if (ci > la) { const u64 to = li < ci ? li : ci; if (to >= la + 1) { nla = to; flags |= RGB_F_APPLIED; } }
  if (mi_dirty | ni_dirty) ST16(reinterpret_cast<ulonglong2 *>(peers) + peer, make_ulonglong2(mi_new, ni_new));
  if (ci != ci0 || nla != la)
    ST16(reinterpret_cast<ulonglong2 *>(dev.hot + (size_t)server * RGB_HOT_WORDS) + HOT_P_CI, make_ulonglong2(ci, nla));
  make_decision(out, server, RGB_ROLE_LEADER, RGB_NONE, 0, RGB_MSG_AER_REPLY, flags, 0, 0, 0, 0, 0, ci, nla);
  return true;
}

#define RGB_IO_SLOT 5
#define RGB_HOT_SLOT 9

template <int N, int KIND, bool SEQXP = (KIND < 0)>
__global__ __launch_bounds__(RGB_TICK_BLOCK, RGB_MIN_WAVES(N)) void rgb_tick_kernel(rgb_dev dev, const rgb_msg *__restrict__ msgs,
                                                                  u32 n, const u32 *__restrict__ n_dev,
                                                                  rgb_decision *__restrict__ dec,
                                                                  rgb_rpc *__restrict__ rpcs, u32 rpc_slot_base,
                                                                  u32 msg_index_base) {
  __shared__ ulonglong2 io[RGB_TICK_BLOCK * RGB_IO_SLOT];
  const u32 lane = threadIdx.x;
  const u32 base = blockIdx.x * RGB_TICK_BLOCK;
  if (n_dev != nullptr) {
    const u32 nd = *n_dev;
    n = nd < n ? nd : n;
    if (base >= n) return;
  }
  const u32 cnt = n - base < RGB_TICK_BLOCK ? n - base : RGB_TICK_BLOCK;
  const ulonglong2 *src = reinterpret_cast<const ulonglong2 *>(msgs + base);
  {
    const u32 last = cnt * 4u - 1u;
    ulonglong2 v[4];
#pragma unroll
    for (int k = 0; k < 4; ++k) {
      const u32 piece = k * RGB_TICK_BLOCK + lane;
      v[k] = ld16<true>(src + (piece < last ? piece : last));
    }
#pragma unroll
    for (int k = 0; k < 4; ++k) {
      const u32 piece = k * RGB_TICK_BLOCK + lane;
      io[(piece >> 2) * RGB_IO_SLOT + (piece & 3u)] = v[k];
    }
  }
  lds_barrier();
  const bool active = lane < cnt;
  Dec d;
  if (active) {
    const ulonglong2 m0 = io[lane * RGB_IO_SLOT + 0], m1 = io[lane * RGB_IO_SLOT + 1],
                     m2 = io[lane * RGB_IO_SLOT + 2], m3 = io[lane * RGB_IO_SLOT + 3];
    process_message<N, KIND, false, false, SEQXP>(dev, m0, m1, m2, m3, base + lane, rpcs, rpc_slot_base, msg_index_base, d);
    if (fuse_wanted(dev, d)) fuse_pipeline_step<N, false>(dev, d, base + lane, rpcs, rpc_slot_base, msg_index_base);
    (void)compact_decision(d);
    io[lane * RGB_IO_SLOT + 0] = make_ulonglong2(d.w[0], d.w[1]);
    io[lane * RGB_IO_SLOT + 1] = make_ulonglong2(d.w[2], d.w[3]);
    io[lane * RGB_IO_SLOT + 2] = make_ulonglong2(d.w[4], d.w[5]);
    io[lane * RGB_IO_SLOT + 3] = make_ulonglong2(d.w[6], d.w[7]);
  }
  lds_barrier();
  if (RGB_KNOB(dev, 2u)) return;
  ulonglong2 *dst = reinterpret_cast<ulonglong2 *>(dec + base);
#pragma unroll
  for (int k = 0; k < 4; ++k) {
    const u32 piece = k * RGB_TICK_BLOCK + lane;
    const u32 j = piece >> 2, part = piece & 3u;
    if (j < cnt && (part < 2u || !((u32)io[j * RGB_IO_SLOT].y & RGB_F_COMPACT)))
      store16_nt((void *)(dst + piece), io[j * RGB_IO_SLOT + part]);
  }
}


struct rgb_tick_plan {
  u32 blk_end[RGB_N_CLASSES];
  u32 off[RGB_N_CLASSES];
  u32 cnt[RGB_N_CLASSES];
};

#define RGB_CLASS_ORDER 0x201CDEB756A8943ull
__host__ __device__ constexpr int rgb_class_at(unsigned q) { return (int)((RGB_CLASS_ORDER >> (4u * q)) & 0xFu); }
static_assert(rgb_class_at(0) == 3 && rgb_class_at(1) == 4 && rgb_class_at(2) == 9 && rgb_class_at(3) == 8 &&
              rgb_class_at(4) == 10 && rgb_class_at(5) == 6 && rgb_class_at(6) == 5 && rgb_class_at(7) == 7 &&
              rgb_class_at(8) == 11 && rgb_class_at(9) == 14 && rgb_class_at(10) == 13 && rgb_class_at(11) == 12 &&
              rgb_class_at(12) == 1 && rgb_class_at(13) == 0 && rgb_class_at(14) == 2, "class order");

__host__ __device__ __forceinline__ void rgb_make_plan(const u32 (&n)[RGB_N_CLASSES], rgb_tick_plan &p, unsigned n_members) {
  u32 blocks = 0;
#pragma unroll
  for (int q = 0; q < RGB_N_CLASSES; ++q) {
    const int c = rgb_class_at((unsigned)q);
    u32 off = 0, cnt = 0;
#pragma unroll
    for (int k = 0; k < RGB_N_CLASSES; ++k) { off += k < c ? n[k] : 0u; cnt = k == c ? n[k] : cnt; }
    const u32 sl = rgb_class_slice(c, n_members);
    blocks += (cnt + sl - 1) / sl;
    p.blk_end[q] = blocks; p.off[q] = off; p.cnt[q] = cnt;
  }
}

__device__ __forceinline__ u32 rgb_xcc_id() {
#ifdef RGB_HOST_EMULATION
  return 0;
#else
  u32 xcc;
  asm volatile("s_getreg_b32 %0, hwreg(HW_REG_XCC_ID, 0, 4)" : "=s"(xcc));
  return xcc;
#endif
}

#ifndef RGB_TRAIN_SPIN_LIMIT
#ifdef RGB_HOST_EMULATION
#define RGB_TRAIN_SPIN_LIMIT 16u
#else
#define RGB_TRAIN_SPIN_LIMIT 20000u
#endif
#endif

#ifndef RGB_X_TICKET_AT
#define RGB_X_TICKET_AT 0
#endif
__device__ __forceinline__ u32 rgb_take_ticket(u32 *ctr, const u32 *err) {
  u32 v = 0;
#ifdef RGB_HOST_EMULATION
  if (threadIdx.x == 0) v = atomicAdd(ctr, 1u);
  if (threadIdx.x == 1) v = *err;
#else
#ifdef RGB_X_TICKET_WG
  if (threadIdx.x == 0) v = __hip_atomic_fetch_add(ctr, 1u, __ATOMIC_RELAXED, __HIP_MEMORY_SCOPE_WORKGROUP);
#else
  if (threadIdx.x == 0) v = __hip_atomic_fetch_add(ctr, 1u, __ATOMIC_RELAXED, __HIP_MEMORY_SCOPE_AGENT);
#endif
  if (threadIdx.x == 1) v = __hip_atomic_load(err, __ATOMIC_RELAXED, __HIP_MEMORY_SCOPE_AGENT);
#endif
  return v;
}
__device__ __forceinline__ u32 rgb_ticket_value(u32 raw) {
#ifdef RGB_HOST_EMULATION
  return __shfl(raw, 0, 64);
#else
  return (u32)__builtin_amdgcn_readfirstlane((int)raw);
#endif
}
__device__ __forceinline__ u32 rgb_ticket_err(u32 raw) {
#ifdef RGB_HOST_EMULATION
  return __shfl(raw, 1, 64);
#else
  return (u32)__builtin_amdgcn_readlane((int)raw, 1);
#endif
}

template <int N, bool TR>
__device__ __forceinline__ bool rgb_tick_slice(const rgb_dev &dev, ulonglong2 *io, const int cls, const u32 base,
                                               const u32 cnt, const u32 SL, const rgb_msg *__restrict__ msgs,
                                               rgb_decision *__restrict__ dec, rgb_rpc *__restrict__ rpcs,
                                               u32 rpc_slot_base, u32 msg_index_base, u32 *__restrict__ ctl,
                                               const unsigned char *__restrict__ stamps,
                                               u32 *__restrict__ ticket_ctr = nullptr, u32 *next_ticket = nullptr,
                                               u32 shard = 0, u32 lane_in = 0, const u32 *place_word = nullptr,
                                               u32 place_bit = 0) {
  const u32 lane = TR ? lane_in : (u32)threadIdx.x;
#ifdef RGB_PROFILE
  u64 t0 = 0, t1 = 0, t2 = 0, t2b = 0, tl[4] = {0, 0, 0, 0};
  if (!TR && RGB_KNOB(dev, 16u)) t0 = wall_clock64();
#endif
  const bool lead_cls = rgb_lead_class(cls);
  constexpr bool PEERS_LDS = rgb_class_slice(1, (unsigned)N) == 32u;
  constexpr bool PEERS_WIDE = TR && rgb_train_class_slice(1, (unsigned)N) == 32u && !PEERS_LDS;
  const bool RUNS_LDS = TR && RGB_TRAIN_RUNS_LDS && (PEERS_LDS || PEERS_WIDE) && dev.max_runs >= (u32)RGB_RUNS_LDS;
  bool AER_RUNS = false;
#if defined(RGB_X_TRAIN_TIMELINE) && !defined(RGB_HOST_EMULATION)
  u64 tt[7] = {0, 0, 0, 0, 0, 0, 0};
  unsigned tt_spins = 0;
#define RGB_TT(k) do { if (TR) tt[k] = wall_clock64(); } while (0)
#else
#define RGB_TT(k) do { } while (0)
#endif
  RGB_TT(0);
  if (TR && RGB_X_TICKET_AT == 2 && ticket_ctr != nullptr) *next_ticket = rgb_take_ticket(ticket_ctr, ctl);
  const ulonglong2 *src = reinterpret_cast<const ulonglong2 *>(msgs + base);
  unsigned need_raw = 0;
  if (TR && lane < cnt) need_raw = (unsigned)stamps[base + lane];
  {
    const u32 last = cnt * 4u - 1u;
    const bool half = rgb_half_msg_class(cls);
#pragma unroll
    for (int k = 0; k < 4; ++k) {
      if ((u32)k * 16u >= SL) break;
      const u32 piece = k * RGB_TICK_BLOCK + lane;
      const u32 r = piece >> 2;
      const u32 sp = (r << 2) | ((piece & 3u) ^ ((r >> 2) & 3u));
      if (!half || (sp & 2u) == 0u) glds16<GLDS_NT>(src + (sp < last ? sp : last), io + k * RGB_TICK_BLOCK);
    }
    glds_wait();
  }
  lds_barrier();
#ifdef RGB_PROFILE
  if (!TR && RGB_KNOB(dev, 16u)) t1 = wall_clock64();
#endif
  const bool active = lane < cnt;
  const u32 mswz = (lane >> 2) & 3u;
  const ulonglong2 m0 = io[lane * 4 + (0 ^ mswz)], m1 = io[lane * 4 + (1 ^ mswz)];
  ulonglong2 m2 = io[lane * 4 + (2 ^ mswz)], m3 = io[lane * 4 + (3 ^ mswz)];
  if (rgb_half_msg_class(cls)) {
    m2 = make_ulonglong2(0, 0); m3 = make_ulonglong2(0, 0);
    if (cls == 2 && active && (((m0.x >> 48) & 0xFFull) & RGB_MF_SEQ2)) m3 = ld16<true>(src + lane * 4u + 3u);
  }
  RGB_TT(1);
  if (TR && RGB_TRAIN_RUNS_LDS && !PEERS_LDS && cls == 0 && dev.max_runs >= (u32)RGB_RUNS_LDS)
    AER_RUNS = __ballot(active && m1.y != m0.y) != 0ull;
  const u32 sv = (u32)(m0.x & 0xFFFFFFFFull);
  const bool has_srv = TR && active && sv < dev.n_servers && ((m0.x >> 32) & 0xFFull) != RGB_MSG_NOP;
  unsigned char *seqp = nullptr;
  unsigned need = 0;
  if (TR) {
    if (__ballot(has_srv && rgb_shard_of_server(sv, (unsigned)N) != shard) != 0ull) {
      if (lane == 0) atomicOr(ctl, (u32)RGB_TRAIN_ERR_ORDER);
      return false;
    }
    seqp = dev.seq + rgb_seq_index(has_srv ? sv : 0u, dev.n_members, dev.seq_stride);
    need = has_srv ? need_raw : 0u;
    unsigned spins = 0;
    bool late = has_srv;
#ifdef RGB_X_TRAIN_NODEPS
    if (RGB_X_TRAIN_NODEPS == 1 || RGB_X_TRAIN_NODEPS == 3) late = false;
#endif
    for (;;) {
      if (late) {
#ifdef RGB_HOST_EMULATION
        const unsigned cur = *seqp;
#elif defined(RGB_X_POLL32)
        const uintptr_t pa = reinterpret_cast<uintptr_t>(seqp);
        const unsigned cur = (__hip_atomic_load(reinterpret_cast<const u32 *>(pa & ~(uintptr_t)3), __ATOMIC_RELAXED,
                                                __HIP_MEMORY_SCOPE_AGENT) >> (8u * (unsigned)(pa & 3u))) & 0xFFu;
#else
        const unsigned cur = __hip_atomic_load(seqp, __ATOMIC_RELAXED, __HIP_MEMORY_SCOPE_AGENT);
#endif
        late = cur != need;
#ifdef RGB_X_TRAIN_NODEPS
        if (RGB_X_TRAIN_NODEPS == 2) late = false;
#endif
      }
      if (__ballot(late) == 0ull) break;
      spins += 1;
#if defined(RGB_X_TRAIN_TIMELINE) && !defined(RGB_HOST_EMULATION)
      tt_spins = spins;
#endif
      bool give_up = spins > RGB_TRAIN_SPIN_LIMIT;
#ifndef RGB_HOST_EMULATION
      if ((spins & 15u) == 0u && __hip_atomic_load(ctl, __ATOMIC_RELAXED, __HIP_MEMORY_SCOPE_AGENT) != 0u) give_up = true;
#ifndef RGB_TRAIN_SLEEP
#define RGB_TRAIN_SLEEP 4
#endif
      __builtin_amdgcn_s_sleep(RGB_TRAIN_SLEEP);
      if (spins > 64u) __builtin_amdgcn_s_sleep(127);
#endif
      if (give_up) {
        if (lane == 0) atomicOr(ctl, (u32)RGB_TRAIN_ERR_SPIN);
        return false;
      }
    }
  }
  RGB_TT(2);
  constexpr bool PRE = true;
  constexpr int ROWS = TR ? GLDS_SC1 : GLDS_DEFAULT;
  u64 pf0 = 0, pf1 = 0;
  lds_barrier();
  {
    const u32 srv = (active && sv < dev.n_servers) ? sv : 0u;
    if (lead_cls && !PEERS_LDS && !PEERS_WIDE) {
      const u64 *pp = dev.peers + (size_t)srv * dev.peer_stride;
      pf0 = ldg8(TR, pp);
      if (3 * N > 16) pf1 = ldg8(TR, pp + 16);
    }
#pragma unroll
    for (int k = 0; k < 8; ++k) {
      if ((u32)k * 8u >= SL) break;
      const u32 r = 8 * k + (lane >> 3);
      const u32 sj = __shfl(srv, (int)r, 64);
      glds16<ROWS>(reinterpret_cast<const ulonglong2 *>(dev.hot + (size_t)sj * RGB_HOT_WORDS) + ((lane & 7u) ^ ((r >> 1) & 7u)),
                   io + k * RGB_TICK_BLOCK);
    }
    if (!PEERS_LDS && AER_RUNS) {
#pragma unroll
      for (int k = 0; k < 8; ++k) {
        const u32 r = 8 * k + (lane >> 3);
        const u32 sj = __shfl(srv, (int)r, 64);
        glds16<ROWS>(reinterpret_cast<const ulonglong2 *>(dev.runs + (size_t)sj * dev.max_runs * 2u) + ((lane & 7u) ^ ((r >> 1) & 7u)),
                     io + (8 + k) * RGB_TICK_BLOCK);
      }
    }
    if (PEERS_WIDE && lead_cls) {
#pragma unroll
      for (int k = 0; k < 8; ++k) {
        const u32 r = 4 * k + (lane >> 4);
        const u32 sj = __shfl(srv, (int)r, 64);
        const u32 pcx = (lane & 15u) ^ (((r >> 1) & 7u) << 1);
        if (pcx < 12u)
          glds16<ROWS>(reinterpret_cast<const ulonglong2 *>(dev.peers + (size_t)sj * 24u) + pcx, io + (4 + k) * RGB_TICK_BLOCK);
      }
      if (RUNS_LDS) {
#pragma unroll
        for (int k = 0; k < 4; ++k) {
          const u32 r = 8 * k + (lane >> 3);
          const u32 sj = __shfl(srv, (int)r, 64);
          glds16<ROWS>(reinterpret_cast<const ulonglong2 *>(dev.runs + (size_t)sj * dev.max_runs * 2u) + ((lane & 7u) ^ ((r >> 1) & 7u)),
                       io + (12 + k) * RGB_TICK_BLOCK);
        }
      }
    }
    if (PEERS_LDS && lead_cls) {
#pragma unroll
      for (int k = 0; k < 4; ++k) {
        const u32 r = 8 * k + (lane >> 3);
        const u32 sj = __shfl(srv, (int)r, 64);
        glds16<ROWS>(reinterpret_cast<const ulonglong2 *>(dev.peers + (size_t)sj * 16u) + ((lane & 7u) ^ ((r >> 1) & 7u)),
                     io + (4 + k) * RGB_TICK_BLOCK);
      }
      if (RUNS_LDS) {
#pragma unroll
        for (int k = 0; k < 4; ++k) {
          const u32 r = 8 * k + (lane >> 3);
          const u32 sj = __shfl(srv, (int)r, 64);
          glds16<ROWS>(reinterpret_cast<const ulonglong2 *>(dev.runs + (size_t)sj * dev.max_runs * 2u) + ((lane & 7u) ^ ((r >> 1) & 7u)),
                       io + (8 + k) * RGB_TICK_BLOCK);
        }
      }
    }
    glds_wait();
  }
  lds_barrier();
  RGB_TT(3);
  if (TR && RGB_X_TICKET_AT == 1 && ticket_ctr != nullptr) *next_ticket = rgb_take_ticket(ticket_ctr, ctl);
  const ulonglong2 *hrow = io + lane * 8;
  const unsigned hswz = (lane >> 1) & 7u;
  const ulonglong2 *prow = (PEERS_LDS && lead_cls) ? io + 4 * RGB_TICK_BLOCK + lane * 8
                           : (PEERS_WIDE && lead_cls) ? io + 4 * RGB_TICK_BLOCK + lane * 16 : nullptr;
  const ulonglong2 *rrow = (RUNS_LDS && PEERS_WIDE && lead_cls) ? io + 12 * RGB_TICK_BLOCK + lane * 8
                           : ((RUNS_LDS && PEERS_LDS && lead_cls) || (!PEERS_LDS && AER_RUNS)) ? io + 8 * RGB_TICK_BLOCK + lane * 8 : nullptr;
#ifndef RGB_HOST_EMULATION
  asm volatile("" ::"v"(pf0), "v"(pf1));
#endif
  Dec d;
  u64 *tlp = nullptr;
#ifdef RGB_PROFILE
  if (!TR) tlp = tl;
#endif
  const bool STASH = TR && RGB_X_RPC_DEFER && (PEERS_LDS || PEERS_WIDE) && lead_cls && rpcs != nullptr;
  ulonglong2 *stash = STASH ? io + lane * 8 : nullptr;
  u64 ct0 = 0;
  if (STASH) ct0 = hrow[HOT_P_TERM ^ hswz].x;
  bool done = false;
#if RGB_X_FAST
  PairSt pst;
  pst.p = nullptr; pst.a = pst.b = make_ulonglong2(0, 0); pst.m = 0;
  if (active) {
    if (cls == 0) done = fast_aer(dev, m0, m1, m2, m3, hrow, hswz, d, &pst);
    else if (cls == 1) done = fast_aer_reply<N, TR, (PEERS_LDS || PEERS_WIDE)>(dev, m0, m1, hrow, hswz, d, prow, rrow);
    else if (cls == 2) done = fast_written(dev, m0, m1, hrow, hswz, d, &pst);
  }
  if (RGB_X_PAIR_STORE && (cls == 0 || cls == 2)) pair_store(pst, lane);
#endif
#if defined(RGB_PROFILE) && !defined(RGB_HOST_EMULATION)
  u64 tf = 0; unsigned n_fast = 0;
  if (!TR && RGB_KNOB(dev, 16u)) { tf = wall_clock64(); n_fast = (unsigned)__popcll(__ballot(done)); }
#endif
  if (active && !done) {
#define RGB_CASE(RANK, KIND)                                                                            \
  case RANK:                                                                                            \
    RGB_MARK("begin", RANK)                                                                             \
    process_message<N, KIND, PRE, TR>(dev, m0, m1, m2, m3, base + lane, rpcs, rpc_slot_base, msg_index_base, d, tlp, \
                                      hrow, hswz, prow, rrow, stash);                                   \
    RGB_MARK("end", RANK)                                                                               \
    break;
    switch (cls) {
      RGB_CASE(0, RGB_MSG_AER) RGB_CASE(1, RGB_MSG_AER_REPLY) RGB_CASE(2, RGB_MSG_WRITTEN)
      RGB_CASE(3, RGB_MSG_APPEND) RGB_CASE(4, RGB_MSG_PIPELINE_RPCS) RGB_CASE(5, RGB_MSG_REQUEST_VOTE)
      RGB_CASE(6, RGB_MSG_VOTE_RESULT) RGB_CASE(7, RGB_MSG_AWAIT_TIMEOUT)
      RGB_CASE(8, RGB_MSG_ELECTION_TIMEOUT) RGB_CASE(9, RGB_MSG_PRE_VOTE_RPC)
      RGB_CASE(10, RGB_MSG_PRE_VOTE_RESULT) RGB_CASE(11, RGB_MSG_SNAPSHOT_WRITTEN)
      RGB_CASE(12, RGB_MSG_HEARTBEAT_RPC) RGB_CASE(13, RGB_MSG_HEARTBEAT_REPLY)
      default:
        if (((m0.x >> 32) & 0xFFull) == RGB_MSG_TRANSFER_LEADERSHIP)
          process_message<N, RGB_MSG_TRANSFER_LEADERSHIP, PRE, TR>(dev, m0, m1, m2, m3, base + lane, rpcs, rpc_slot_base,
                                                                   msg_index_base, d, tlp, hrow, hswz, prow);
        else
          process_message<N, RGB_MSG_CONSISTENT_QUERY, PRE, TR>(dev, m0, m1, m2, m3, base + lane, rpcs, rpc_slot_base,
                                                                msg_index_base, d, tlp, hrow, hswz, prow);
        break;
    }
#undef RGB_CASE
#if defined(RGB_PROFILE) && !defined(RGB_HOST_EMULATION)
    if (!TR && RGB_KNOB(dev, 16u)) { t2 = wall_clock64(); asm volatile("s_waitcnt vmcnt(0)" ::: "memory"); t2b = wall_clock64(); }
#endif
  }
  const unsigned n_parked = (STASH && active) ? (unsigned)((d.w[0] >> 48) & 0xFFull) : 0u;
  if (dev.fuse_pipeline && (cls == 1 || cls == 2)) {
    const bool want = active && fuse_wanted(dev, d);
    if (__ballot(want) != 0ull && want) fuse_pipeline_step<N, TR>(dev, d, base + lane, rpcs, rpc_slot_base, msg_index_base);
  }
  const bool is_compact = active && compact_decision(d);
  const u64 cmask = __ballot(is_compact);
  RGB_TT(4);
  if (TR) {
#if !defined(RGB_HOST_EMULATION) && !defined(RGB_X_TRAIN_NOWAIT)
    __builtin_amdgcn_s_waitcnt(0x0F70);
    asm volatile("" ::: "memory");
#endif
#if defined(RGB_X_TRAIN_NODEPS) && RGB_X_TRAIN_NODEPS == 3
    if (RGB_X_TRAIN_NODEPS == 1)
#endif
#if defined(RGB_X_XOR_PUBLISH) && !defined(RGB_HOST_EMULATION)
    if (has_srv && seqp != nullptr) {
      const uintptr_t a = reinterpret_cast<uintptr_t>(seqp);
      (void)__hip_atomic_fetch_xor(reinterpret_cast<u32 *>(a & ~(uintptr_t)3), ((need ^ (need + 1u)) & 0xFFu) << (8u * (unsigned)(a & 3u)),
                                   __ATOMIC_RELAXED, __HIP_MEMORY_SCOPE_AGENT);
    }
#else
    if (has_srv && seqp != nullptr) *seqp = (unsigned char)(need + 1u);
#endif
    if (RGB_X_TICKET_AT == 0 && ticket_ctr != nullptr) *next_ticket = rgb_take_ticket(ticket_ctr, ctl);
    if (place_word != nullptr && lane == 0) {
#ifdef RGB_HOST_EMULATION
      *const_cast<u32 *>(place_word) |= place_bit;
#else
      (void)__hip_atomic_fetch_or(const_cast<u32 *>(place_word), place_bit, __ATOMIC_RELAXED, __HIP_MEMORY_SCOPE_AGENT);
#endif
    }
  }
  if (STASH) {
    const unsigned n_rp = n_parked;
    if (__ballot(n_rp != 0u) != 0ull) {
      rgb_rpc *slot0 = rpcs + (size_t)(rpc_slot_base + base + lane) * (N > 1 ? N - 1 : 1);
      const u64 w0 = (u64)(msg_index_base + base + lane) | ((d.w[0] & 0xFFFFFFFFull) << 32);
#pragma unroll
      for (unsigned j = 0; j < (N > 1 ? (unsigned)N - 1u : 1u) && j < 4u; ++j) {
        if (j < n_rp) {
          const ulonglong2 a = stash[2u * j], b = stash[2u * j + 1u];
          store_rpc(slot0 + j, w0, a.x, ct0, a.y, b.x, d.w[6], b.y);
        }
      }
    }
  }
  RGB_TT(5);
  lds_barrier();
  if (active) {
    io[lane * RGB_IO_SLOT + 0] = make_ulonglong2(d.w[0], d.w[1]);
    io[lane * RGB_IO_SLOT + 1] = make_ulonglong2(d.w[2], d.w[3]);
    if (!is_compact) {
      io[lane * RGB_IO_SLOT + 2] = make_ulonglong2(d.w[4], d.w[5]);
      io[lane * RGB_IO_SLOT + 3] = make_ulonglong2(d.w[6], d.w[7]);
    }
  }
  lds_barrier();
  if (!TR && RGB_KNOB(dev, 2u)) return true;
#ifdef RGB_X_TRAIN_NODEC
  if (TR) return true;
#endif
  ulonglong2 *dst = reinterpret_cast<ulonglong2 *>(dec + base);
#pragma unroll
  for (int k = 0; k < 4; ++k) {
    const u32 piece = k * RGB_TICK_BLOCK + lane;
    const u32 j = piece >> 2, part = piece & 3u;
#ifdef RGB_X_HALFDEC
    if (j < cnt && part < 2u) store16_nt((void *)(dst + piece), io[j * RGB_IO_SLOT + part]);
#else
    if (j < cnt && (part < 2u || !((cmask >> j) & 1ull)))
      store16_nt((void *)(dst + piece), io[j * RGB_IO_SLOT + part]);
#endif
  }
#if defined(RGB_X_TRAIN_TIMELINE) && !defined(RGB_HOST_EMULATION)
  if (TR && dev.dbg_buf != nullptr && lane == 0 && blockIdx.x < (1u << 20)) {
    u64 *o = dev.dbg_buf + (size_t)blockIdx.x * 8;
    tt[6] = wall_clock64();
    for (int k = 0; k < 7; ++k) o[k] = tt[k];
    o[7] = (u64)(unsigned)cls | ((u64)cnt << 8) | ((u64)tt_spins << 32) | ((u64)rgb_xcc_id() << 56);
  }
#endif
#ifdef RGB_PROFILE
  if (!TR && RGB_KNOB(dev, 16u)) {
    unsigned mx = (unsigned)tl[1], sm = (unsigned)tl[1], nz = tl[1] ? 1u : 0u;
#pragma unroll
    for (int o = 32; o >= 1; o >>= 1) {
      const unsigned a = __shfl_xor(mx, o, 64), b = __shfl_xor(sm, o, 64), c = __shfl_xor(nz, o, 64);
      mx = a > mx ? a : mx; sm += b; nz += c;
    }
    if (lane == 0) {
      u64 *o = dev.dbg_buf + (size_t)blockIdx.x * 8;
      o[0] = t0; o[1] = t1 | ((tl[0] > t1 ? tl[0] - t1 : 0) << 40);
      o[2] = t2 | ((t2b > t2 ? t2b - t2 : 0) << 40) | ((u64)cls << 60); o[3] = wall_clock64();
      o[4] = mx; o[5] = sm | ((tl[2] > t1 ? tl[2] - t1 : 0) << 24); o[6] = nz | ((tl[3] > t1 ? tl[3] - t1 : 0) << 24);
      o[7] = cnt | ((u64)n_fast << 8) | ((tf > t1 ? tf - t1 : 0) << 24);
// ... 286 lines not shown

__device__ __forceinline__ u64 sm64(u64 &x) {
  x += 0x9E3779B97F4A7C15ull;
  u64 z = x;
  z = (z ^ (z >> 30)) * 0xBF58476D1CE4E5B9ull;
  z = (z ^ (z >> 27)) * 0x94D049BB133111EBull;
  return z ^ (z >> 31);
}

struct SynMember { u64 ct, ci, la, li, lt, lwi, lwt, pk, first, lrs, lrt, prs, prt; };

template <class Lane>
__device__ __forceinline__ void syn_lane(Lane &T, const SynMember &x, const u64 *runs) {
  T.first = x.first; T.li = x.li; T.lrs = x.lrs; T.lrt = x.lrt; T.prs = x.prs; T.prt = x.prt;
  T.push_cnt = 0; T.n_runs = (unsigned)pk_get(x.pk, PK_NRUNS_SH, 5);
  T.runs = runs; T.runs_lds = nullptr;
#ifdef RGB_PROFILE
  T.prof_noprobe = false; T.prof_nloads = 0;
#endif
}

struct SynMsg {
  u32 server; unsigned kind, from, flags, gap; u64 term, a, b, c; u32 n_entries, n_run0; u64 run0, run1;
  bool off_steady;
};

__device__ __forceinline__ void syn_store(rgb_msg *slot, const SynMsg &m) {
  ulonglong2 *o = reinterpret_cast<ulonglong2 *>(slot);
  u64 w0 = (u64)m.server | ((u64)(m.kind & 0xFF) << 32) | ((u64)(m.from & 0xFF) << 40) |
           ((u64)(m.flags & 0xFF) << 48) | ((u64)(m.gap & 0xFF) << 56);
  o[0] = make_ulonglong2(w0, m.term);
  o[1] = make_ulonglong2(m.a, m.b);
  o[2] = make_ulonglong2(m.c, (u64)m.n_entries | ((u64)m.n_run0 << 32));
  o[3] = make_ulonglong2(m.run0, m.run1);
}

__device__ __forceinline__ SynMsg syn_msg(u32 server, unsigned kind, unsigned from, unsigned flags, u64 term,
                                          u64 a, u64 b, u64 c, u32 n_entries = 0, u32 n_run0 = 0, u64 run0 = 0) {
  SynMsg m;
  m.server = server; m.kind = kind; m.from = from; m.flags = flags; m.gap = 0; m.term = term;
  m.a = a; m.b = b; m.c = c; m.n_entries = n_entries; m.n_run0 = n_run0; m.run0 = run0; m.run1 = 0;
  m.off_steady = false;
  return m;
}

template <int N, class Emit>
__device__ __forceinline__ void synth_group(const rgb_dev &dev, u64 seed, u64 tick, u32 g, Emit &&emit) {
  u64 rs = seed ^ (tick * 0xD1B54A32D192ED03ull) ^ ((u64)g * 0x9E3779B97F4A7C15ull);
  SynMember mb[N];
  int leader = -1, cand = -1, prev = -1, hi = 0;
  u64 lead_ct = 0, maxct = 0;
#pragma unroll
  for (int m = 0; m < N; ++m) {
    const ulonglong2 *hp = reinterpret_cast<const ulonglong2 *>(dev.hot + ((size_t)g * N + m) * RGB_HOT_WORDS);
    const ulonglong2 h0 = hp[HOT_P_TERM], h1 = hp[HOT_P_CI], h2 = hp[HOT_P_LI], h3 = hp[HOT_P_LW], h5 = hp[HOT_P_FIRST],
                     h6 = hp[HOT_P_LRT], h7 = hp[HOT_P_PEND];
    mb[m].ct = h0.x; mb[m].pk = h0.y; mb[m].ci = h1.x; mb[m].la = h1.y; mb[m].li = h2.x;
    mb[m].lt = h2.y; mb[m].lwi = h3.x; mb[m].lwt = h3.y; mb[m].first = h5.x; mb[m].lrs = h5.y;
    mb[m].lrt = h6.x; mb[m].prs = h6.y; mb[m].prt = h7.x;
  }
#pragma unroll
  for (int m = 0; m < N; ++m) {
    const unsigned role = (unsigned)pk_get(mb[m].pk, PK_ROLE_SH, 3);
    if (mb[m].ct > maxct) maxct = mb[m].ct;
    if (role == RGB_ROLE_LEADER && (leader < 0 || mb[m].ct > lead_ct)) { leader = m; lead_ct = mb[m].ct; }
  }
#pragma unroll
  for (int m = 0; m < N; ++m) {
    const unsigned role = (unsigned)pk_get(mb[m].pk, PK_ROLE_SH, 3);
    if (role == RGB_ROLE_CANDIDATE && mb[m].ct == maxct && cand < 0) cand = m;
    if (role == RGB_ROLE_PRE_VOTE && mb[m].ct == maxct && prev < 0) prev = m;
    const bool better = mb[m].ct > mb[hi].ct ||
                        (mb[m].ct == mb[hi].ct && (mb[m].lt > mb[hi].lt ||
                                                   (mb[m].lt == mb[hi].lt && mb[m].li > mb[hi].li)));
    if (better) hi = m;
  }
  auto sid = [&](int m) -> u32 { return g * N + (u32)m; };
  auto other = [&](int m, u64 r) -> int { return N > 1 ? (int)((m + 1 + r % (N - 1)) % N) : m; };

  const bool healthy = leader >= 0 && lead_ct == maxct;
  if (!healthy) {
    const u64 r = sm64(rs);
    if (leader >= 0) {
      int mh = hi == leader ? other(leader, r) : hi;
      emit(syn_msg(sid(leader), RGB_MSG_AER_REPLY, mh, 0, mb[mh].ct, mb[mh].li + 1, mb[mh].lwi, mb[mh].lwt));
    } else if (cand >= 0) {
      emit(syn_msg(sid(cand), RGB_MSG_VOTE_RESULT, other(cand, r), RGB_MF_SUCCESS, mb[cand].ct, 0, 0, 0));
    } else if (prev >= 0) {
      emit(syn_msg(sid(prev), RGB_MSG_PRE_VOTE_RESULT, other(prev, r), RGB_MF_SUCCESS, mb[prev].ct, 0, 0,
                   (dev.qry + (size_t)sid(prev) * RGB_QRY_WORDS)[QRY_TOKEN]));
    } else {
      emit(syn_msg(sid(hi), RGB_MSG_ELECTION_TIMEOUT, RGB_NONE, 0, 0, 0, 0, (r | 1ull) & 0xFFFFFFFFFFFFull));
    }
    return;
  }
  const int l = leader;
  const SynMember &ld = mb[l];
  bool used[N];
#pragma unroll
  for (int m = 0; m < N; ++m) used[m] = false;
  const u64 rc = sm64(rs);
  if (rc % 100 < 5 && !RGB_KNOB(dev, 128u)) {
    const int churn = (int)((rc >> 8) % N);
    const u64 r2 = sm64(rs);
    const u64 lli = mb[churn].li + (r2 % 3) > 0 ? mb[churn].li + (r2 % 3) - 1 : 0;
    emit(syn_msg(sid(churn), RGB_MSG_REQUEST_VOTE, other(churn, r2 >> 8), 0, mb[churn].ct + 1, lli,
                 mb[churn].lt, 0));
    used[churn] = true;
  }
#pragma unroll
  for (int m = 0; m < N; ++m) {
    if (used[m]) continue;
    const SynMember &x = mb[m];
    const unsigned nr = (unsigned)pk_get(x.pk, PK_NRUNS_SH, 5);
    if (nr < 4 || !(x.first <= x.li) || x.la < x.first || x.la > x.li) continue;
    LaneT<false> T;
    syn_lane(T, x, dev.runs + (size_t)sid(m) * dev.max_runs * 2);
    const u64 t = fetch_term(T, x.la);
    if (t == UNDEF) continue;
    emit(syn_msg(sid(m), RGB_MSG_SNAPSHOT_WRITTEN, RGB_NONE, 0, 0, x.la, t, 0));
    used[m] = true;
  }
  u64 lq = 0; int hb_lag = -1; unsigned hb_behind = 0;
  if (pk_get(ld.pk, PK_QSELF_SH, 1)) {
    const u64 *q = dev.qry + (size_t)sid(l) * RGB_QRY_WORDS;
    lq = q[0];
    const bool peers_nz = pk_get(ld.pk, PK_QPEER_SH, 1) != 0;
#pragma unroll
    for (int m = 0; m < N; ++m) {
      if (m == l) continue;
      const u64 qm = peers_nz ? q[1 + m] : 0;
      if (qm < lq) { hb_behind |= 1u << m; if (hb_lag < 0) hb_lag = m; }
    }
  }
  if (!used[l]) {
    const u64 r = sm64(rs), r2 = sm64(rs);
    const bool nonempty = ld.first <= ld.li;
    if (ld.lt != ld.ct || !nonempty) {
      emit(syn_msg(sid(l), RGB_MSG_APPEND, RGB_NONE, RGB_MF_FORCE, 0, 0, 0, 0, 1));
    } else if (ld.lwi < ld.li && (r & 3) == 0) {
      const u64 a = ld.lwi + 1 > ld.first ? ld.lwi + 1 : ld.first;
      SynMsg w = syn_msg(sid(l), RGB_MSG_WRITTEN, RGB_NONE, 0, ld.lt, a, ld.li, 0);
      w.off_steady = RGB_X_HINT && dev.synth_hint >= 1u;
      emit(w);
    } else if (hb_lag >= 0 && (r >> 40) % 3 == 0) {
      emit(syn_msg(sid(l), RGB_MSG_HEARTBEAT_REPLY, hb_lag, 0, ld.ct, lq, 0, 0));
    } else if ((r >> 44) % 50 == 0) {
      emit(syn_msg(sid(l), RGB_MSG_CONSISTENT_QUERY, RGB_NONE, 0, 0, 0, 0, 0));
    } else {
      unsigned v = (unsigned)((r >> 8) % 100);
      if (RGB_KNOB(dev, 128u) && v >= 75 && v < 80) v = 0;
      const int j = other(l, r >> 16);
      const u64 *pr = dev.peers + (size_t)sid(l) * dev.peer_stride;
      const u64 mi = pr[PEER_MI(j, N)];
      LaneT<false> T;
      syn_lane(T, ld, dev.runs + (size_t)sid(l) * dev.max_runs * 2);
      if (v < 75) {
        u64 last = mi + r2 % 5;
        if (mb[j].lwi > last) last = mb[j].lwi;
        if (last > ld.li) last = ld.li;
        u64 nxt = last + 1 + (r2 >> 8) % 3; if (nxt > ld.li + 1) nxt = ld.li + 1;
        u64 t = fetch_term(T, last); if (t == UNDEF) t = 0;
        emit(syn_msg(sid(l), RGB_MSG_AER_REPLY, j, RGB_MF_SUCCESS, ld.ct, nxt, last, t));
      } else if (v < 80) {
        u64 lo = ld.first > 0 ? ld.first - 1 : 0;
        u64 last = mi > r2 % 4 ? mi - r2 % 4 : 0; if (last < lo) last = lo;
        u64 t = fetch_term(T, last); if (t == UNDEF) t = 0;
        if ((r2 >> 8) & 1) t += 1;
        emit(syn_msg(sid(l), RGB_MSG_AER_REPLY, j, 0, ld.ct, last + 1, last, t));
      } else {
        emit(syn_msg(sid(l), RGB_MSG_APPEND, RGB_NONE, 0, 0, 0, 0, 0, 1 + (u32)(r2 % 4)));
      }
    }
  }
#pragma unroll
  for (int j = 0; j < N; ++j) {
    if (j == l || used[j]) continue;
    const SynMember &f = mb[j];
    const u64 r = sm64(rs), r2 = sm64(rs);
    if (((hb_behind >> j) & 1u) && (r >> 40) % 8 == 0) {
      emit(syn_msg(sid(j), RGB_MSG_HEARTBEAT_RPC, l, 0, ld.ct, lq, 0, 0));
    } else if ((r & 1) == 0) {
      unsigned v = (unsigned)((r >> 8) % 100);
      if (RGB_KNOB(dev, 128u)) v = 0;
      const u64 eterm = ld.ct > f.lt ? ld.ct : f.lt;
      u64 prev_i = f.li, prev_t = f.lt, run0 = eterm;
      u32 n_ent = 1 + (u32)(r2 % 8);
      if (v >= 80 && v < 85) { n_ent = 0; }
      else if (v >= 85 && v < 90) { prev_i = f.li + 1 + (r2 >> 8) % 3; prev_t = ld.ct; n_ent = (u32)((r2 >> 16) % 3); }
      else if (v >= 90 && v < 95) { prev_t = f.lt + 1; n_ent = 0; }
      else if (v >= 95) {
        const u64 back = 1 + (r2 >> 8) % 4;
        u64 floor_i = f.lrs > f.la ? f.lrs : f.la; if (f.first > floor_i) floor_i = f.first;
        if (f.first <= f.li && f.li >= back && f.li - back >= floor_i) {
          prev_i = f.li - back; prev_t = f.lt; n_ent = (u32)back; run0 = f.lt;
        }
      }
      SynMsg w = syn_msg(sid(j), RGB_MSG_AER, l, 0, ld.ct, prev_i, prev_t, ld.ci, n_ent, n_ent, run0);
      bool off = pk_get(f.pk, PK_ROLE_SH, 3) != RGB_ROLE_FOLLOWER;
      if (dev.synth_hint >= 2u)
        off = off || f.ct != ld.ct || (unsigned)pk_get(f.pk, PK_LEADER_SH, 4) != (unsigned)l || !(f.first <= f.li) ||
              prev_i != f.li || prev_t != f.lt || (n_ent != 0 && run0 != f.lt);
      w.off_steady = RGB_X_HINT && dev.synth_hint >= 1u && off;
      emit(w);
    } else if (f.lwi < f.li && f.first <= f.li && (r >> 8) % 10 < 8) {
      const u64 a = f.lwi + 1 > f.first ? f.lwi + 1 : f.first;
      SynMsg w = syn_msg(sid(j), RGB_MSG_WRITTEN, RGB_NONE, 0, f.lt, a, f.li, 0);
      bool off = pk_get(f.pk, PK_ROLE_SH, 3) != RGB_ROLE_FOLLOWER;
      if (dev.synth_hint >= 2u) off = off || (unsigned)pk_get(f.pk, PK_LEADER_SH, 4) == SLOT_NONE4;
      w.off_steady = RGB_X_HINT && dev.synth_hint >= 1u && off;
      emit(w);
    }
  }
}

template <int N, bool WRITE>
__global__ __launch_bounds__(64) void rgb_synth_kernel(rgb_dev dev, u64 seed, u64 tick, rgb_msg *__restrict__ out,
                                                       u32 *__restrict__ scratch, unsigned char *__restrict__ stamps,
                                                       unsigned char *__restrict__ sent) {
  __shared__ u32 cnt[RGB_N_BUCKETS], rank[RGB_N_BUCKETS];
  u32 *blk = scratch + RGB_SYNTH_FIXED_WORDS + (size_t)blockIdx.x * RGB_N_BUCKETS;
  for (u32 b = threadIdx.x; b < RGB_N_BUCKETS; b += blockDim.x) { cnt[b] = 0; rank[b] = 0; }
  __syncthreads();
  const u32 G = dev.n_servers / N;
  const u32 g = blockIdx.x * blockDim.x + threadIdx.x;
  auto bucket = [](const SynMsg &m) -> unsigned { return rgb_bucket_hinted(m.kind, m.flags, m.server, (unsigned)N, m.off_steady); };
  if (!WRITE) {
    if (g < G) synth_group<N>(dev, seed, tick, g, [&](const SynMsg &m) { atomicAdd(&cnt[bucket(m)], 1u); });
    __syncthreads();
    for (u32 b = threadIdx.x; b < RGB_N_BUCKETS; b += blockDim.x) blk[b] = cnt[b];
    return;
  }
  if (g < G)
    synth_group<N>(dev, seed, tick, g, [&](const SynMsg &m) {
      const unsigned b = bucket(m);
      const u32 slot = blk[b] + atomicAdd(&rank[b], 1u);
      syn_store(out + slot, m);
      if (stamps != nullptr) {
        const u32 q = rgb_seq_index(m.server, (unsigned)N, dev.seq_stride);
        const unsigned char c = sent[q];
        sent[q] = (unsigned char)(c + 1u);
        stamps[slot] = c;
      }
    });
}

__global__ void rgb_synth_scan_kernel(u32 *__restrict__ scratch, u32 n_blocks, u32 *__restrict__ kind_counts,
                                      u32 *__restrict__ d_n, u32 *__restrict__ bucket_counts) {
  __shared__ u32 tot[RGB_N_BUCKETS];
  u32 *fam_total = scratch, *bkt_total = scratch + RGB_N_FAMILIES, *bkt_base = bkt_total + RGB_N_BUCKETS;
  u32 *blk = scratch + RGB_SYNTH_FIXED_WORDS;
  const u32 b = threadIdx.x;
  u32 sum = 0;
  for (u32 k = 0; k < n_blocks; ++k) sum += blk[(size_t)k * RGB_N_BUCKETS + b];
  tot[b] = sum;
  bkt_total[b] = sum;
  if (bucket_counts != nullptr) bucket_counts[b] = sum;
  __syncthreads();
  u32 acc = 0;
  for (u32 k = 0; k < b; ++k) acc += tot[k];
  bkt_base[b] = acc;
  for (u32 k = 0; k < n_blocks; ++k) {
    const u32 c = blk[(size_t)k * RGB_N_BUCKETS + b];
    blk[(size_t)k * RGB_N_BUCKETS + b] = acc;
    acc += c;
  }
  if (b < RGB_N_FAMILIES) {
    u32 f = 0;
    for (u32 x = 0; x < RGB_TRAIN_SHARDS; ++x) f += tot[((b >> 1) * RGB_TRAIN_SHARDS + x) * 2u + (b & 1u)];
    fam_total[b] = f;
  }
  if (b == 0) {
    u32 total = 0;
    const unsigned kind_of_rank[RGB_N_CLASSES + 1] = {
        RGB_MSG_AER, RGB_MSG_AER_REPLY, RGB_MSG_WRITTEN, RGB_MSG_APPEND, RGB_MSG_PIPELINE_RPCS,
        RGB_MSG_REQUEST_VOTE, RGB_MSG_VOTE_RESULT, RGB_MSG_AWAIT_TIMEOUT, RGB_MSG_ELECTION_TIMEOUT,
        RGB_MSG_PRE_VOTE_RPC, RGB_MSG_PRE_VOTE_RESULT, RGB_MSG_SNAPSHOT_WRITTEN, RGB_MSG_HEARTBEAT_RPC,
        RGB_MSG_HEARTBEAT_REPLY, RGB_MSG_CONSISTENT_QUERY, RGB_MSG_NOP};
    for (unsigned c = 0; c <= RGB_N_CLASSES; ++c) {
      u32 ct = 0;
      for (u32 k = 0; k < 2u * RGB_TRAIN_SHARDS; ++k) ct += tot[c * 2u * RGB_TRAIN_SHARDS + k];
      total += ct;
      if (kind_counts != nullptr && ct) kind_counts[kind_of_rank[c]] += ct;
    }
    if (d_n != nullptr) *d_n = total;
  }
}


__global__ void rgb_pack_kernel(rgb_dev dev, const rgb_server_state *__restrict__ in, u32 first, u32 n) {
  const u32 k = blockIdx.x * blockDim.x + threadIdx.x;
  if (k >= n) return;
  const rgb_server_state &h = in[k];
  const u32 s = first + k;
  u64 *hot = dev.hot + (size_t)s * RGB_HOT_WORDS;
  const unsigned N = dev.n_members;
  u64 *runs = dev.runs + (size_t)s * dev.max_runs * 2;
  unsigned nr = 0;
  u64 first_index = h.first_index;
  u64 lrs = 0, lrt = 0, prs = 0, prt = 0;
  if (h.first_index <= h.last_index) {
    unsigned src_n = h.n_runs > RGB_MAX_RUNS ? RGB_MAX_RUNS : h.n_runs;
    unsigned canon = 0;
    for (unsigned r = 0; r < src_n; ++r)
      if (r == 0 || h.run_term[r] != h.run_term[r - 1]) canon++;
    unsigned skip = canon > dev.max_runs ? canon - dev.max_runs : 0;
    unsigned ci = 0;
    for (unsigned r = 0; r < src_n; ++r) {
      if (!(r == 0 || h.run_term[r] != h.run_term[r - 1])) continue;
      if (ci >= skip) {
        if (nr == 0 && skip) first_index = h.run_start[r];
        runs[2 * nr] = h.run_start[r]; runs[2 * nr + 1] = h.run_term[r];
        prs = lrs; prt = lrt;
        lrs = h.run_start[r]; lrt = h.run_term[r];
        nr++;
      }
      ci++;
    }
  }
  u64 pk = 0;
  pk = pk_set(pk, PK_ROLE_SH, 3, h.role);
  pk = pk_with_cond_reason(pk, h.cond_reason);
  pk = pk_set(pk, PK_SELF_SH, 4, h.self);
  pk = pk_set(pk, PK_VOTES_SH, 4, h.votes);
  pk = pk_set(pk, PK_NRUNS_SH, 5, nr);
  pk = pk_set(pk, PK_NONVOTER_SH, 1, h.self_nonvoter ? 1 : 0);
  pk = pk_set(pk, PK_VOTED_SH, 4, slot8to4(h.voted_for));
  pk = pk_set(pk, PK_LEADER_SH, 4, slot8to4(h.leader_id));
  pk = pk_set(pk, PK_CONDLDR_SH, 4, slot8to4(h.cond_leader));
  pk = pk_set(pk, PK_PRESENT_SH, 8, h.present_mask);
  pk = pk_set(pk, PK_VOTER_SH, 8, h.voter_mask);
  pk = pk_set(pk, PK_STATUS_SH, 8, h.status_mask);
  hot[HOT_CT] = h.current_term; hot[HOT_CI] = h.commit_index; hot[HOT_LA] = h.last_applied;
  hot[HOT_LI] = h.last_index; hot[HOT_LT] = h.last_term;
  hot[HOT_LWI] = h.last_written_index; hot[HOT_LWT] = h.last_written_term;
  hot[HOT_PK] = pk; hot[HOT_SI] = h.snapshot_index; hot[HOT_ST] = h.snapshot_term;
  hot[HOT_FIRST] = first_index; hot[HOT_LRS] = lrs; hot[HOT_LRT] = lrt;
  if (nr < 2) { prs = 0; prt = 0; }
  hot[HOT_PRS] = prs; hot[HOT_PRT] = prt;
  hot[HOT_PEND] = h.pending_first;
  {
    u64 *q = dev.qry + (size_t)s * RGB_QRY_WORDS;
    bool peer_nz = false;
    q[0] = h.query_index;
    for (unsigned i = 0; i < 8; ++i) { q[1 + i] = h.peer_query_index[i]; peer_nz = peer_nz || h.peer_query_index[i] != 0; }
    for (unsigned i = 9; i < RGB_QRY_WORDS; ++i) q[i] = 0;
    const unsigned backoff = (unsigned)h.backoff_mask & ~(unsigned)h.status_mask & (unsigned)h.present_mask &
                             ~(1u << h.self) & 0xFFu;
    q[QRY_BACKOFF] = backoff;
    q[QRY_TOKEN] = h.pre_vote_token;
    q[QRY_MACVER] = (u64)h.machine_version | ((u64)h.effective_machine_version << 32);
    const unsigned npo = h.n_pending_old > 2 ? 2u : h.n_pending_old;
    q[QRY_PEND_LO] = npo == 2 ? h.pending_old[0][0] : 1; q[QRY_PEND_LO + 1] = npo == 2 ? h.pending_old[0][1] : 0;
    q[QRY_PEND_HI] = npo ? h.pending_old[npo - 1][0] : 1; q[QRY_PEND_HI + 1] = npo ? h.pending_old[npo - 1][1] : 0;
    pk = pk_set(pk, PK_PENDX_SH, 1, npo ? 1 : 0);
    pk = pk_set(pk, PK_BACKOFF_SH, 1, backoff ? 1 : 0);
    pk = pk_set(pk, PK_QSELF_SH, 1, h.query_index != 0 ? 1 : 0);
    pk = pk_set(pk, PK_QPEER_SH, 1, peer_nz ? 1 : 0);
    hot[HOT_PK] = pk;
  }
  u64 *pr = dev.peers + (size_t)s * dev.peer_stride;
  for (unsigned i = 0; i < dev.peer_stride; ++i) pr[i] = 0;
  for (unsigned i = 0; i < N; ++i) {
    pr[PEER_MI(i, N)] = h.match_index[i]; pr[PEER_NI(i, N)] = h.next_index[i]; pr[PEER_CS(i, N)] = h.commit_index_sent[i];
  }
  u64 *cd = dev.cond + (size_t)s * 4;
  for (int i = 0; i < 4; ++i) cd[i] = h.cond_reply[i];
}

__global__ void rgb_unpack_kernel(rgb_dev dev, rgb_server_state *__restrict__ out, u32 first, u32 n) {
  const u32 k = blockIdx.x * blockDim.x + threadIdx.x;
  if (k >= n) return;
  const u32 s = first + k;
  rgb_server_state h;
  memset(&h, 0, sizeof h);
  const u64 *hot = dev.hot + (size_t)s * RGB_HOT_WORDS;
  const unsigned N = dev.n_members;
  const u64 pk = hot[HOT_PK];
  h.current_term = hot[HOT_CT]; h.commit_index = hot[HOT_CI]; h.last_applied = hot[HOT_LA];
  h.last_index = hot[HOT_LI]; h.last_term = hot[HOT_LT];
  h.last_written_index = hot[HOT_LWI]; h.last_written_term = hot[HOT_LWT];
  h.snapshot_index = hot[HOT_SI]; h.snapshot_term = hot[HOT_ST];
  h.first_index = hot[HOT_FIRST];
  const u64 *cd = dev.cond + (size_t)s * 4;
  for (int i = 0; i < 4; ++i) h.cond_reply[i] = cd[i];
  const u64 *pr = dev.peers + (size_t)s * dev.peer_stride;
  for (unsigned i = 0; i < N; ++i) {
    h.match_index[i] = pr[PEER_MI(i, N)]; h.next_index[i] = pr[PEER_NI(i, N)]; h.commit_index_sent[i] = pr[PEER_CS(i, N)];
  }
  unsigned nr = (unsigned)pk_get(pk, PK_NRUNS_SH, 5);
  const u64 *runs = dev.runs + (size_t)s * dev.max_runs * 2;
  if (!(h.first_index <= h.last_index)) { nr = 0; h.first_index = h.last_index + 1; }
  for (unsigned r = 0; r < nr && r < RGB_MAX_RUNS; ++r) { h.run_start[r] = runs[2 * r]; h.run_term[r] = runs[2 * r + 1]; }
  h.role = (uint8_t)pk_get(pk, PK_ROLE_SH, 3);
  h.cond_reason = (uint8_t)pk_cond_reason(pk);
  h.self = (uint8_t)pk_get(pk, PK_SELF_SH, 4);
  h.n_members = (uint8_t)N;
  h.voted_for = (uint8_t)slot4to8((unsigned)pk_get(pk, PK_VOTED_SH, 4));
  h.leader_id = (uint8_t)slot4to8((unsigned)pk_get(pk, PK_LEADER_SH, 4));
  h.votes = (uint8_t)pk_get(pk, PK_VOTES_SH, 4);
  h.n_runs = (uint8_t)nr;
  h.present_mask = (uint8_t)pk_get(pk, PK_PRESENT_SH, 8);
  h.voter_mask = (uint8_t)pk_get(pk, PK_VOTER_SH, 8);
  h.status_mask = (uint8_t)pk_get(pk, PK_STATUS_SH, 8);
  h.self_nonvoter = (uint8_t)pk_get(pk, PK_NONVOTER_SH, 1);
  h.cond_leader = (uint8_t)slot4to8((unsigned)pk_get(pk, PK_CONDLDR_SH, 4));
  {
    const u64 *q = dev.qry + (size_t)s * RGB_QRY_WORDS;
    h.pre_vote_token = q[QRY_TOKEN];
    h.machine_version = (uint32_t)(q[QRY_MACVER] & 0xFFFFFFFFull);
    h.effective_machine_version = (uint32_t)(q[QRY_MACVER] >> 32);
  }
  h.pending_first = hot[HOT_PEND];
  {
    const u64 *q = dev.qry + (size_t)s * RGB_QRY_WORDS;
    h.query_index = q[0];
    for (unsigned i = 0; i < 8; ++i) h.peer_query_index[i] = q[1 + i];
    h.backoff_mask = pk_get(pk, PK_BACKOFF_SH, 1) ? (uint8_t)(q[QRY_BACKOFF] & 0xFFu) : 0;
    if (pk_get(pk, PK_PENDX_SH, 1)) {
      const bool two = q[QRY_PEND_LO] <= q[QRY_PEND_LO + 1];
      h.n_pending_old = two ? 2 : 1;
      if (two) { h.pending_old[0][0] = q[QRY_PEND_LO]; h.pending_old[0][1] = q[QRY_PEND_LO + 1]; }
      h.pending_old[two ? 1 : 0][0] = q[QRY_PEND_HI]; h.pending_old[two ? 1 : 0][1] = q[QRY_PEND_HI + 1];
    }
  }
  out[k] = h;
}

__global__ void rgb_leaderboard_kernel(rgb_dev dev, rgb_leaderboard_row *__restrict__ rows, u32 n_groups) {
  const u32 g = blockIdx.x * blockDim.x + threadIdx.x;
  if (g >= n_groups) return;
  const unsigned N = dev.n_members;
  u32 leader = RGB_NONE, n_leaders = 0;
  u64 term = 0, lead_term = 0, ci = 0, la = 0, max_ci = 0, max_la = 0;
  for (unsigned m = 0; m < N; ++m) {
    const u64 *hot = dev.hot + ((size_t)g * N + m) * RGB_HOT_WORDS;
    const ulonglong2 h0 = reinterpret_cast<const ulonglong2 *>(hot)[HOT_P_TERM];
    const ulonglong2 h1 = reinterpret_cast<const ulonglong2 *>(hot)[HOT_P_CI];
    const u64 pk = hot[HOT_PK];
    const u64 ct = h0.x;
    if (ct > term) term = ct;
    if (h1.x > max_ci) max_ci = h1.x;
    if (h1.y > max_la) max_la = h1.y;
    if (pk_get(pk, PK_ROLE_SH, 3) == RGB_ROLE_LEADER) {
      n_leaders++;
      if (leader == RGB_NONE || ct > lead_term) { leader = m; lead_term = ct; ci = h1.x; la = h1.y; }
    }
  }
  rgb_leaderboard_row r;
  r.leader = leader; r.n_leaders = n_leaders; r.term = term;
  r.commit_index = leader == RGB_NONE ? max_ci : ci;
  r.last_applied = leader == RGB_NONE ? max_la : la;
  rows[g] = r;
}

__device__ __forceinline__ u64 fnv_word(u64 h, u64 w) {
#pragma unroll
  for (int i = 0; i < 8; ++i) { h ^= (w >> (8 * i)) & 0xFFull; h *= 0x100000001B3ull; }
  return h;
}

__global__ void rgb_checksum_kernel(rgb_dev dev, u32 first, u32 n, u64 *__restrict__ out) {
  const u32 k = blockIdx.x * blockDim.x + threadIdx.x;
  if (k >= n) return;
  const u32 s = first + k;
  const u64 *hot = dev.hot + (size_t)s * RGB_HOT_WORDS;
  const unsigned N = dev.n_members;
  const u64 pk = hot[HOT_PK];
  u64 li = hot[HOT_LI], fi = hot[HOT_FIRST];
  unsigned nr = (unsigned)pk_get(pk, PK_NRUNS_SH, 5);
  if (!(fi <= li)) { nr = 0; fi = li + 1; }
  u64 x = 0xCBF29CE484222325ull;
  x = fnv_word(x, hot[HOT_CT]); x = fnv_word(x, hot[HOT_CI]); x = fnv_word(x, hot[HOT_LA]);
  x = fnv_word(x, li); x = fnv_word(x, hot[HOT_LT]); x = fnv_word(x, hot[HOT_LWI]);
  x = fnv_word(x, hot[HOT_LWT]); x = fnv_word(x, hot[HOT_SI]); x = fnv_word(x, hot[HOT_ST]);
  x = fnv_word(x, fi);
  u64 packed = pk_get(pk, PK_ROLE_SH, 3) | ((u64)pk_cond_reason(pk) << 8) |
               (pk_get(pk, PK_SELF_SH, 4) << 16) | ((u64)N << 24) |
               ((u64)slot4to8((unsigned)pk_get(pk, PK_VOTED_SH, 4)) << 32) |
               ((u64)slot4to8((unsigned)pk_get(pk, PK_LEADER_SH, 4)) << 40) |
               (pk_get(pk, PK_VOTES_SH, 4) << 48) | ((u64)nr << 56);
  x = fnv_word(x, packed);
  u64 masks = pk_get(pk, PK_PRESENT_SH, 8) | (pk_get(pk, PK_VOTER_SH, 8) << 8) |
              (pk_get(pk, PK_STATUS_SH, 8) << 16) | (pk_get(pk, PK_NONVOTER_SH, 1) << 24);
  if (pk_get(pk, PK_BACKOFF_SH, 1)) masks |= ((dev.qry + (size_t)s * RGB_QRY_WORDS)[QRY_BACKOFF] & 0xFFull) << 32;
  x = fnv_word(x, masks);
  x = fnv_word(x, (dev.qry + (size_t)s * RGB_QRY_WORDS)[QRY_TOKEN]);
  x = fnv_word(x, hot[HOT_PEND]);
  if (pk_get(pk, PK_PENDX_SH, 1)) {
    const u64 *q = dev.qry + (size_t)s * RGB_QRY_WORDS;
    if (q[QRY_PEND_LO] <= q[QRY_PEND_LO + 1]) { x = fnv_word(x, q[QRY_PEND_LO]); x = fnv_word(x, q[QRY_PEND_LO + 1]); }
    x = fnv_word(x, q[QRY_PEND_HI]); x = fnv_word(x, q[QRY_PEND_HI + 1]);
  }
  {
    const u64 *q = dev.qry + (size_t)s * RGB_QRY_WORDS;
    x = fnv_word(x, q[0]);
    for (unsigned i = 0; i < N && i < 8; ++i) x = fnv_word(x, q[1 + i]);
  }
  x = fnv_word(x, (dev.qry + (size_t)s * RGB_QRY_WORDS)[QRY_MACVER]);
  const u64 *pr = dev.peers + (size_t)s * dev.peer_stride;
  for (unsigned i = 0; i < N; ++i) {
    x = fnv_word(x, pr[PEER_MI(i, N)]); x = fnv_word(x, pr[PEER_NI(i, N)]); x = fnv_word(x, pr[PEER_CS(i, N)]);
  }
  const u64 *runs = dev.runs + (size_t)s * dev.max_runs * 2;
  for (unsigned r = 0; r < nr; ++r) { x = fnv_word(x, runs[2 * r]); x = fnv_word(x, runs[2 * r + 1]); }
  out[k] = x;
}

__global__ void rgb_stamp_rounds_kernel(rgb_dev dev, const rgb_msg *__restrict__ msgs, u32 n, unsigned char *__restrict__ stamps) {
  const u32 i = blockIdx.x * blockDim.x + threadIdx.x;
  if (i >= n) return;
  const u64 w = *reinterpret_cast<const u64 *>(msgs + i);
  const u32 sv = (u32)(w & 0xFFFFFFFFull);
  if (((w >> 32) & 0xFFull) == RGB_MSG_NOP || sv >= dev.n_servers) { stamps[i] = 0; return; }
  stamps[i] = (unsigned char)(dev.seq[rgb_seq_index(sv, dev.n_members, dev.seq_stride)] + stamps[i]);
}
#define RGB_RES_BLOCK 128u
#define RGB_RES_MAX_STRIDE 7u
__global__ __launch_bounds__(RGB_RES_BLOCK) void rgb_results_sums_kernel(const rgb_decision *__restrict__ dec, const u32 *__restrict__ pos,
                                                                         u32 n, u32 rpc_stride, u32 *__restrict__ block_sums,
                                                                         u32 *__restrict__ err) {
  __shared__ u32 part[RGB_RES_BLOCK / 64u];
  const u32 i = blockIdx.x * RGB_RES_BLOCK + threadIdx.x;
  u32 v = i < n ? (u32)((reinterpret_cast<const u64 *>(dec + pos[i])[0] >> 48) & 0xFFull) : 0u;
  if (v > rpc_stride) { atomicOr(err, 1u); v = rpc_stride; }
#pragma unroll
  for (int o = 32; o >= 1; o >>= 1) v += __shfl_xor(v, o, 64);
  if ((threadIdx.x & 63u) == 0u) part[threadIdx.x >> 6] = v;
  __syncthreads();
  if (threadIdx.x == 0) {
    u32 t = 0;
#pragma unroll
    for (u32 w = 0; w < RGB_RES_BLOCK / 64u; ++w) t += part[w];
    block_sums[blockIdx.x] = t;
  }
}

__global__ __launch_bounds__(RGB_RES_BLOCK) void rgb_results_kernel(const ulonglong2 *__restrict__ dec, const u32 *__restrict__ pos, u32 n,
                                                                    const u32 *__restrict__ block_sums, const u64 *__restrict__ rpcs,
                                                                    u32 rpc_stride, u32 *__restrict__ err, const u32 *__restrict__ ctl,
                                                                    ulonglong2 *__restrict__ out_dec, u64 *__restrict__ out_rpcs,
                                                                    u32 *__restrict__ out_hdr) {
  __shared__ ulonglong2 sdec[RGB_RES_BLOCK * 4u];
  __shared__ u64 srec[RGB_RES_BLOCK * RGB_RES_MAX_STRIDE * 7u];
  __shared__ u32 sscan[RGB_RES_BLOCK];
  __shared__ u32 sred[RGB_RES_BLOCK];
  const u32 tid = threadIdx.x, b = blockIdx.x;
  const u32 i = b * RGB_RES_BLOCK + tid;
  u32 partial = 0;
  for (u32 k = tid; k < b; k += RGB_RES_BLOCK) partial += block_sums[k];
  sred[tid] = partial;
  u32 nr = 0, p = 0;
  if (i < n) {
    p = pos[i];
    const ulonglong2 *src = dec + (size_t)p * 4u;
    ulonglong2 a = src[0], bb = src[1], c, e;
    nr = (u32)((a.x >> 48) & 0xFFull);
    if (nr > rpc_stride) nr = rpc_stride;
    const u32 flags = (u32)a.y;
    if (flags & RGB_F_COMPACT) {
      const u32 aux = (u32)(a.y >> 32), f = flags & ~(u32)RGB_F_COMPACT;
      const u64 A = bb.x, B = bb.y;
      u64 w2 = 0, w3 = 0, w4 = 0, w5 = 0, ci, la;
      if (f & RGB_F_REPLY) {
        w3 = A + 1ull; w2 = B; w4 = A - (u64)(aux & 0xFFu); w5 = B - (u64)((aux >> 8) & 0xFu);
        ci = A + (u64)((aux >> 12) & 0x3FFu) - 512ull; la = A + 1ull - (u64)((aux >> 22) & 0x3FFu);
      } else if (f & RGB_F_WROTE) {
        w4 = A; w3 = A - (u64)(aux & 0xFFFFu); ci = B; la = A - (u64)(aux >> 16);
      } else { ci = A; la = B; }
      a.y = (u64)f;
      bb = make_ulonglong2(w2, w3); c = make_ulonglong2(w4, w5); e = make_ulonglong2(ci, la);
    } else { c = src[2]; e = src[3]; }
    sdec[tid * 4u + 0u] = a; sdec[tid * 4u + 1u] = bb; sdec[tid * 4u + 2u] = c; sdec[tid * 4u + 3u] = e;
  }
  sscan[tid] = nr;
  __syncthreads();
  for (u32 o = 1; o < RGB_RES_BLOCK; o <<= 1) {
    const u32 add = tid >= o ? sscan[tid - o] : 0u;
    const u32 r2 = (tid + o < RGB_RES_BLOCK && (tid & (2u * o - 1u)) == 0u) ? sred[tid + o] : 0u;
    __syncthreads();
    sscan[tid] += add;
    sred[tid] += r2;
    __syncthreads();
  }
  const u32 base = sred[0], mine = sscan[RGB_RES_BLOCK - 1u], off = sscan[tid] - nr;
  for (u32 q = 0; q < nr; ++q) {
    const u64 *r = rpcs + ((size_t)p * rpc_stride + q) * 7u;
    u64 *d = srec + (size_t)(off + q) * 7u;
    d[0] = (r[0] & 0xFFFFFFFF00000000ull) | (u64)i;
#pragma unroll
    for (int k = 1; k < 7; ++k) d[k] = r[k];
  }
  __syncthreads();
  const u32 first = b * RGB_RES_BLOCK, cnt = n - first < RGB_RES_BLOCK ? n - first : RGB_RES_BLOCK;
  ulonglong2 *od = out_dec + (size_t)first * 4u;
  for (u32 k = tid; k < cnt * 4u; k += RGB_RES_BLOCK) od[k] = sdec[k];
  u64 *orp = out_rpcs + (size_t)base * 7u;
  for (u32 k = tid; k < mine * 7u; k += RGB_RES_BLOCK) orp[k] = srec[k];
  if (b == gridDim.x - 1u && tid == 0u) {
    out_hdr[0] = base + mine;
    out_hdr[1] = ctl ? ctl[0] : 0u;
    out_hdr[2] = err[0];
    err[0] = 0u;
  }
}

__host__ __device__ __forceinline__ u32 rgb_undo_pieces_of(const rgb_dev &dev) {
  return RGB_HOT_WORDS / 2u + dev.peer_stride / 2u + dev.max_runs + 2u + RGB_QRY_WORDS / 2u + 1u;
}
__global__ void rgb_undo_kernel(rgb_dev dev, const u32 *__restrict__ ids, u32 n, ulonglong2 *__restrict__ undo, u32 restore) {
  const u32 P = rgb_undo_pieces_of(dev);
  const u64 idx = (u64)blockIdx.x * blockDim.x + threadIdx.x;
  const u32 i = (u32)(idx / P), p = (u32)(idx - (u64)i * P);
  if (i >= n) return;
  const u32 sv = ids[i];
  if (sv >= dev.n_servers) return;
  ulonglong2 *slot = undo + (size_t)i * P + p;
  u32 q = p;
  ulonglong2 *row;
  if (q < RGB_HOT_WORDS / 2u) row = reinterpret_cast<ulonglong2 *>(dev.hot + (size_t)sv * RGB_HOT_WORDS) + q;
  else if ((q -= RGB_HOT_WORDS / 2u) < dev.peer_stride / 2u) row = reinterpret_cast<ulonglong2 *>(dev.peers + (size_t)sv * dev.peer_stride) + q;
  else if ((q -= dev.peer_stride / 2u) < dev.max_runs) row = reinterpret_cast<ulonglong2 *>(dev.runs + (size_t)sv * dev.max_runs * 2u) + q;
  else if ((q -= dev.max_runs) < 2u) row = reinterpret_cast<ulonglong2 *>(dev.cond + (size_t)sv * 4u) + q;
  else if ((q -= 2u) < RGB_QRY_WORDS / 2u) row = reinterpret_cast<ulonglong2 *>(dev.qry + (size_t)sv * RGB_QRY_WORDS) + q;
  else {
    unsigned char *b = dev.seq + rgb_seq_index(sv, dev.n_members, dev.seq_stride);
    if (restore) *b = (unsigned char)slot->x; else *slot = make_ulonglong2((u64)*b, 0);
    return;
  }
  if (restore) *row = *slot; else *slot = *row;
}

}

#define RGB_BLOCK 256
#ifdef RGB_X_ONLY_N
#define RGB_LAUNCH_ALL_N LAUNCH(RGB_X_ONLY_N)
#else
#define RGB_LAUNCH_ALL_N LAUNCH(1) LAUNCH(2) LAUNCH(3) LAUNCH(4) LAUNCH(5) LAUNCH(6) LAUNCH(7) LAUNCH(8)
#endif

template <int KIND, bool SEQXP = (KIND < 0)>
static int launch_tick_kind(const rgb_dev &dev, const rgb_msg *d_msgs, u32 n, const u32 *d_n, rgb_decision *d_dec,
                            rgb_rpc *d_rpcs, u32 rpc_slot_base, u32 msg_index_base, hipStream_t st) {
  dim3 grid((n + RGB_TICK_BLOCK - 1) / RGB_TICK_BLOCK), block(RGB_TICK_BLOCK);
#define LAUNCH(NN)                                                                                   \
  case NN:                                                                                           \
    hipLaunchKernelGGL((rgb_tick_kernel<NN, KIND, SEQXP>), grid, block, 0, st, dev, d_msgs, n, d_n, d_dec, \
                       d_rpcs, rpc_slot_base, msg_index_base);                                       \
    break;
  switch (dev.n_members) {
    RGB_LAUNCH_ALL_N
    default: return -1;
  }
#undef LAUNCH
// ... 442 lines not shown
```

Measured before the change: 13.84 billion.

## Pack peer rows as 32-bit pairs and mirror recent log runs into them

For 3-5 member groups, the per-server peer row now stores match, next and commit-sent indices as packed 32-bit halves when they fit, flagged by a header word. The freed words hold a mirror of the most recent log run entries, anchored to the previous run start. The tick kernel's peer-row LDS load can then serve run lookups without a separate runs-table load, dropping the runs LDS prefetch for that path. Values that exceed 32 bits fall back to the wide layout. The cost is extra header checks, unpack and pack logic, mirror rebuilds on leadership or anchor changes, and added correctness risk.

Measured after the change: 13.21 billion. 4.5% lower.

```diff
diff --git a/ra_amd/csrc/rgb_api.hip b/ra_amd/csrc/rgb_api.hip
--- a/ra_amd/csrc/rgb_api.hip
+++ b/ra_amd/csrc/rgb_api.hip
@@ -385,6 +385,7 @@
   HIPCHK(ctx, hipMalloc((void **)&d.cond, (size_t)S * 4 * sizeof(u64)));
   HIPCHK(ctx, hipMalloc((void **)&d.qry, (size_t)S * RGB_QRY_WORDS * sizeof(u64)));
   HIPCHK(ctx, hipMemsetAsync(d.runs, 0, (size_t)S * d.max_runs * 2 * sizeof(u64), ctx->stream));
+  HIPCHK(ctx, hipMemsetAsync(d.peers, 0, (size_t)S * d.peer_stride * sizeof(u64), ctx->stream));
   d.seq_stride = (((n_groups + RGB_TRAIN_SHARDS - 1u) / RGB_TRAIN_SHARDS) * n_members * RGB_SEQ_SPREAD + 255u) & ~255u;
   HIPCHK(ctx, hipMalloc((void **)&d.seq, (size_t)d.seq_stride * RGB_TRAIN_SHARDS));
   HIPCHK(ctx, hipMemsetAsync(d.seq, 0, (size_t)d.seq_stride * RGB_TRAIN_SHARDS, ctx->stream));
diff --git a/ra_amd/csrc/rgb_internal.h b/ra_amd/csrc/rgb_internal.h
--- a/ra_amd/csrc/rgb_internal.h
+++ b/ra_amd/csrc/rgb_internal.h
@@ -139,6 +139,57 @@
   return (3u * n_members + 7u) & ~7u;
 }
 
+#define RGB_PEERS_HDR_WORD    15u
+#define RGB_PEERS_MIRROR_WORD 8u
+#define RGB_PEERS_MIRROR_MAX  7u
+#ifndef RGB_PEERS_FIT_LIMIT
+#define RGB_PEERS_FIT_LIMIT 0x100000000ull
+#endif
+static inline __host__ __device__ constexpr bool rgb_peers_compact_n(unsigned n_members) { return n_members >= 3u && n_members <= 5u; }
+static inline __host__ __device__ bool rgb_peers_fits(u64 v) { return v < (u64)RGB_PEERS_FIT_LIMIT; }
+static inline __host__ __device__ bool rgb_peers_hdr_compact(u64 hdr) { return (hdr & 15ull) == 1ull; }
+static inline __host__ __device__ unsigned rgb_peers_hdr_m(u64 hdr) { return (unsigned)((hdr >> 4) & 15ull); }
+#define RGB_PEERS_HDR_BUILD 0x100ull
+static inline __host__ __device__ u64 rgb_peers_hdr_anchor(u64 hdr) { return hdr >> 32; }
+static inline __host__ __device__ u64 rgb_peers_hdr(unsigned m, u64 anchor) { return 1ull | ((u64)m << 4) | (anchor << 32); }
+static inline __host__ __device__ u64 rgb_peers_pair(u64 lo, u64 hi) { return (lo & 0xFFFFFFFFull) | (hi << 32); }
+static inline __host__ __device__ unsigned rgb_peers_mirror_usable(u64 hdr, unsigned role, unsigned n_runs, u64 prs) {
+  if (!rgb_peers_hdr_compact(hdr) || (hdr & RGB_PEERS_HDR_BUILD) || role != (unsigned)RGB_ROLE_LEADER || n_runs < 3u ||
+      rgb_peers_hdr_anchor(hdr) != prs) return 0u;
+  const unsigned m = rgb_peers_hdr_m(hdr);
+  return m < n_runs - 2u ? m : n_runs - 2u;
+}
+static inline __host__ __device__ bool rgb_peers_row_compact(const u64 *w, unsigned N) {
+  return rgb_peers_compact_n(N) && rgb_peers_hdr_compact(w[RGB_PEERS_HDR_WORD]);
+}
+static inline __host__ __device__ u64 rgb_peers_mi(const u64 *w, unsigned N, unsigned i) {
+  return rgb_peers_row_compact(w, N) ? (w[i] & 0xFFFFFFFFull) : w[PEER_MI(i, N)];
+}
+static inline __host__ __device__ u64 rgb_peers_ni(const u64 *w, unsigned N, unsigned i) {
+  return rgb_peers_row_compact(w, N) ? (w[i] >> 32) : w[PEER_NI(i, N)];
+}
+static inline __host__ __device__ u64 rgb_peers_cs(const u64 *w, unsigned N, unsigned i) {
+  const unsigned q = 2u * N + i;
+  return rgb_peers_row_compact(w, N) ? ((w[q >> 1] >> (32u * (q & 1u))) & 0xFFFFFFFFull) : w[PEER_CS(i, N)];
+}
+static inline __host__ __device__ bool rgb_peers_put_row(u64 *w, unsigned N, const uint64_t *mi, const uint64_t *ni, const uint64_t *cs,
+                                                         unsigned stride) {
+  bool fits = rgb_peers_compact_n(N);
+  for (unsigned i = 0; i < N && fits; ++i) fits = rgb_peers_fits(mi[i]) && rgb_peers_fits(ni[i]) && rgb_peers_fits(cs[i]);
+  for (unsigned i = 0; i < stride; ++i) w[i] = 0;
+  if (!fits) {
+    for (unsigned i = 0; i < N; ++i) { w[PEER_MI(i, N)] = mi[i]; w[PEER_NI(i, N)] = ni[i]; w[PEER_CS(i, N)] = cs[i]; }
+    return false;
+  }
+  for (unsigned i = 0; i < N; ++i) {
+    const unsigned q = 2u * N + i;
+    w[i] = rgb_peers_pair((u64)mi[i], (u64)ni[i]);
+    w[q >> 1] |= (u64)cs[i] << (32u * (q & 1u));
+  }
+  w[RGB_PEERS_HDR_WORD] = rgb_peers_hdr(0u, 0ull);
+  return true;
+}
+
 struct rgb_dev {
   u64 *hot;
   u64 *peers;
diff --git a/ra_amd/csrc/rgb_kernels.hip b/ra_amd/csrc/rgb_kernels.hip
--- a/ra_amd/csrc/rgb_kernels.hip
+++ b/ra_amd/csrc/rgb_kernels.hip
@@ -18,6 +18,18 @@
 #endif
 #ifndef RGB_MIN_WAVES
 #define RGB_MIN_WAVES(N) 2
+#endif
+
+#ifdef RGB_X_MIRROR_CHECK
+#ifdef RGB_HOST_EMULATION
+extern "C" { __attribute__((weak)) unsigned long long rgb_x_peers_counters[8]; }
+extern "C" __attribute__((weak)) void rgb_x_peers_counters_read(unsigned long long *out) { memcpy(out, rgb_x_peers_counters, sizeof rgb_x_peers_counters); }
+#else
+__device__ unsigned long long rgb_x_peers_counters[8];
+extern "C" void rgb_x_peers_counters_read(unsigned long long *out) {
+  (void)hipMemcpyFromSymbol(out, HIP_SYMBOL(rgb_x_peers_counters), sizeof rgb_x_peers_counters);
+}
+#endif
 #endif
 
 namespace {
@@ -164,8 +176,9 @@
 __device__ __forceinline__ unsigned slot8to4(unsigned s) { return s >= 8u ? SLOT_NONE4 : s; }
 __device__ __forceinline__ unsigned slot4to8(unsigned s) { return s >= 8u ? (unsigned)RGB_NONE : s; }
 
-template <bool COH, bool WC = false, bool SEQX = false>
+template <bool COH, bool WC = false, bool SEQX = false, bool MIR = false>
 struct LaneT {
+  static constexpr bool mirror = MIR;
   static constexpr bool coh = COH;
   static constexpr bool seqx_ok = SEQX;
   static constexpr bool walk_cache = WC;
@@ -202,6 +215,7 @@
   unsigned pdirty;
   unsigned dcs_ci;
   bool peers_loaded;
+  u64 phdr;
   u64 *qry_base;
   u64 qself, qp[8];
   bool q_loaded;
@@ -222,22 +236,41 @@
 __device__ __forceinline__ void load_peers(Lane &L) {
   if (L.peers_loaded) return;
   constexpr int PS = (3 * N + 7) & ~7;
+  constexpr bool CN = rgb_peers_compact_n((unsigned)N);
   u64 w[PS];
   if ((PS == 16 || PS == 24) && L.peers_lds != nullptr) {
     const unsigned sw = PS == 24 ? L.peers_swz << 1 : L.peers_swz;
 #pragma unroll
     for (int k = 0; k < PS / 2; ++k) {
-      if (2 * k < 3 * N) { ulonglong2 v = L.peers_lds[(unsigned)k ^ sw]; w[2 * k] = v.x; w[2 * k + 1] = v.y; }
-    }
+      if (2 * k < 3 * N || (CN && k == 7)) { ulonglong2 v = L.peers_lds[(unsigned)k ^ sw]; w[2 * k] = v.x; w[2 * k + 1] = v.y; }
+    }
+#pragma unroll
+    for (int i = 0; i < N; ++i) { L.pmi[i] = w[PEER_MI(i, N)]; L.pni[i] = w[PEER_NI(i, N)]; L.pcs[i] = w[PEER_CS(i, N)]; }
+    if (CN && Lane::coh) L.phdr = w[PS - 1];
   } else {
     const ulonglong2 *pp = reinterpret_cast<const ulonglong2 *>(L.peers);
 #pragma unroll
     for (int k = 0; k < PS / 2; ++k) {
-      if (2 * k < 3 * N) { ulonglong2 v = ldg16(L.coh, pp + k); w[2 * k] = v.x; w[2 * k + 1] = v.y; }
-    }
-  }
-#pragma unroll
-  for (int i = 0; i < N; ++i) { L.pmi[i] = w[PEER_MI(i, N)]; L.pni[i] = w[PEER_NI(i, N)]; L.pcs[i] = w[PEER_CS(i, N)]; }
+      if (2 * k < 3 * N || (CN && k == 7)) { ulonglong2 v = ldg16(L.coh, pp + k); w[2 * k] = v.x; w[2 * k + 1] = v.y; }
+    }
+#pragma unroll
+    for (int i = 0; i < N; ++i) { L.pmi[i] = w[PEER_MI(i, N)]; L.pni[i] = w[PEER_NI(i, N)]; L.pcs[i] = w[PEER_CS(i, N)]; }
+    if (CN && Lane::coh) L.phdr = w[PS - 1];
+    if (CN && rgb_peers_hdr_compact(w[PS - 1])) {
+#define RGB_PW(j) (((j) & 1) ? L.pni[(j) >> 1] : L.pmi[(j) >> 1])
+#pragma unroll
+      for (int i = 0; i < N; ++i) {
+        const int q = 2 * N + i;
+        L.pcs[i] = (RGB_PW(q >> 1) >> (32 * (q & 1))) & 0xFFFFFFFFull;
+      }
+#pragma unroll
+      for (int i = N - 1; i >= 0; --i) {
+        const u64 v = RGB_PW(i);
+        L.pmi[i] = v & 0xFFFFFFFFull; L.pni[i] = v >> 32;
+      }
+#undef RGB_PW
+    }
+  }
   L.peers_loaded = true;
 }
 
@@ -288,8 +321,32 @@
 #ifndef RGB_TRAIN_RUNS_LDS
 #define RGB_TRAIN_RUNS_LDS 1
 #endif
+#ifdef RGB_X_MIRROR_CHECK
+#define RGB_X_COUNT(i) atomicAdd(&rgb_x_peers_counters[i], 1ull)
+__device__ __forceinline__ void rgb_x_mirror_check(bool coh, const u64 *runs, int k, ulonglong2 got) {
+  const ulonglong2 t = ldg16(coh, reinterpret_cast<const ulonglong2 *>(runs) + k);
+  if (k < 0 || t.y != got.y || (k > 0 ? t.x != got.x : t.x < got.x)) RGB_X_COUNT(4);
+}
+#else
+#define RGB_X_COUNT(i) do { } while (0)
+#endif
 template <class Lane>
 __device__ __forceinline__ ulonglong2 run_pair(const Lane &L, int k) {
+  if (Lane::mirror) {
+    if (L.runs_lds != nullptr) {
+      const ulonglong2 meta = L.runs_lds[7u ^ L.peers_swz];
+      const unsigned j = (unsigned)((int)meta.y - k);
+      if (j < (unsigned)meta.x) {
+        const ulonglong2 r = L.runs_lds[j ^ L.peers_swz];
+#ifdef RGB_X_MIRROR_CHECK
+        RGB_X_COUNT(0); rgb_x_mirror_check(L.coh, L.runs, k, r);
+#endif
+        return r;
+      }
+      RGB_X_COUNT(1);
+    }
+    return ldg16(L.coh, reinterpret_cast<const ulonglong2 *>(L.runs) + k);
+  }
   if (L.runs_lds != nullptr && k < RGB_RUNS_LDS) return L.runs_lds[(unsigned)k ^ L.peers_swz];
   return ldg16(L.coh, reinterpret_cast<const ulonglong2 *>(L.runs) + k);
 }
@@ -298,7 +355,7 @@
 #ifdef RGB_PROFILE
   const_cast<Lane &>(L).prof_nloads += 1;
 #endif
-  if (L.runs_lds != nullptr && i < 2 * RGB_RUNS_LDS) {
+  if (!Lane::mirror && L.runs_lds != nullptr && i < 2 * RGB_RUNS_LDS) {
     const ulonglong2 v = L.runs_lds[(unsigned)(i >> 1) ^ L.peers_swz];
     return (i & 1) ? v.y : v.x;
   }
@@ -1038,7 +1095,11 @@
 template <int N, class Lane>
 __device__ __forceinline__ void become_leader(Lane &L) {
   const u64 ni = next_log_index(L);
-  load_peers<N>(L);
+  if (!L.peers_loaded) {
+#pragma unroll
+    for (int i = 0; i < N; ++i) { L.pmi[i] = 0; L.pni[i] = 0; L.pcs[i] = 0; }
+    L.peers_loaded = true;
+  }
 #pragma unroll
   for (int i = 0; i < N; ++i) {
     if (!present(L, i)) continue;
@@ -1785,7 +1846,9 @@
                                                 const ulonglong2 *pre = nullptr, unsigned swz = 0,
                                                 const ulonglong2 *prepeers = nullptr,
                                                 const ulonglong2 *preruns = nullptr, ulonglong2 *rpc_stash = nullptr) {
-  LaneT<TR, (N >= 6 && KIND == RGB_MSG_AER), SEQXP> L;
+  constexpr bool MIR = PRE && TR && rgb_peers_compact_n((unsigned)N) &&
+                       (KIND == RGB_MSG_AER_REPLY || KIND == RGB_MSG_APPEND || KIND == RGB_MSG_PIPELINE_RPCS);
+  LaneT<TR, (N >= 6 && KIND == RGB_MSG_AER), SEQXP, MIR> L;
   L.rpc_stash = rpc_stash;
   L.wc_k = -1; L.wc_start = L.wc_term = L.wc_next = 0;
   L.server = (u32)(m0.x & 0xFFFFFFFFull);
@@ -1834,7 +1897,7 @@
   L.runs = dev.runs + (size_t)L.server * dev.max_runs * 2;
   L.peers = dev.peers + (size_t)L.server * dev.peer_stride;
   L.max_runs = dev.max_runs;
-  L.peers_loaded = false; L.dmi = L.dni = L.dcs = 0; L.dcs_ci = 0;
+  L.peers_loaded = false; L.dmi = L.dni = L.dcs = 0; L.dcs_ci = 0; L.phdr = UNDEF;
   L.peers_lds = prepeers; L.peers_swz = swz; L.pdirty = 0;
   L.runs_lds = preruns;
 #ifndef RGB_X_COMMIT_WAIT
@@ -1848,6 +1911,9 @@
 #endif
 #ifndef RGB_X_REREAD_TICK
 #define RGB_X_REREAD_TICK 1
+#endif
+#ifndef RGB_X_REREAD
+#define RGB_X_REREAD 0
 #endif
   constexpr bool PL = (TR ? RGB_X_PL : RGB_X_PL_TICK) && PRE && rgb_class_slice(1, (unsigned)N) == 32u &&
                       (KIND == RGB_MSG_AER_REPLY || KIND == RGB_MSG_APPEND || KIND == RGB_MSG_PIPELINE_RPCS);
@@ -1918,6 +1984,12 @@
 #ifdef RGB_PROFILE
   if (t_loaded && RGB_KNOB(dev, 16u)) t_loaded[2] = wall_clock64();
 #endif
+#ifdef RGB_X_MIRROR_CHECK
+  if (rgb_peers_compact_n((unsigned)N) && L.kind == RGB_MSG_SNAPSHOT_WRITTEN && !rc && role_of(L) == RGB_ROLE_LEADER &&
+      L.n_runs < n_runs0 &&
+      rgb_peers_mirror_usable(ldg8(TR, L.peers + RGB_PEERS_HDR_WORD), RGB_ROLE_LEADER, n_runs0, h6.y) != 0u)
+    RGB_X_COUNT(3);
+#endif
   if (rc) {
     make_decision(out, L.server, role0, RGB_NONE, 0, L.kind, RGB_F_INVARIANT, (u32)rc, 0, 0, 0, 0, ci0, la0);
     return;
@@ -1963,22 +2035,81 @@
     for (int i = 0; i < N; ++i)
       if (q_reset || (L.q_dirty & (2u << i))) q[1 + i] = L.qp[i];
   }
-  if (PL) {
-    if (L.pdirty | L.dcs_ci) {
-#pragma unroll
-      for (int w = 0; w < 2 * N; ++w)
-        if (L.pdirty & (1u << w)) ST8(L.peers + w, prow_get(L, (unsigned)w));
-#pragma unroll
-      for (int k = 0; k < N; ++k)
-        if (L.dcs_ci & (1u << k)) ST8(L.peers + PEER_CS(k, N), L.ci);
-    }
-  } else if (L.dmi | L.dni | L.dcs | L.dcs_ci) {
-#pragma unroll
-    for (int k = 0; k < N; ++k) {
-      if (L.dmi & (1u << k)) ST8(L.peers + PEER_MI(k, N), L.pmi[k]);
-      if (L.dni & (1u << k)) ST8(L.peers + PEER_NI(k, N), L.pni[k]);
-      if (L.dcs & (1u << k)) ST8(L.peers + PEER_CS(k, N), L.pcs[k]);
-      else if (L.dcs_ci & (1u << k)) ST8(L.peers + PEER_CS(k, N), L.ci);
+  {
+    constexpr bool CN = rgb_peers_compact_n((unsigned)N);
+    constexpr bool Lane_coh = TR;
+    const bool pdirty = PL ? (L.pdirty | L.dcs_ci) != 0u : (L.dmi | L.dni | L.dcs | L.dcs_ci) != 0u;
+    u64 hdr = 0;
+    if (CN && pdirty) hdr = PL ? prow_get(L, RGB_PEERS_HDR_WORD) : (Lane_coh && L.phdr != UNDEF) ? L.phdr : ldg8(TR, L.peers + RGB_PEERS_HDR_WORD);
+    bool compact = CN && rgb_peers_hdr_compact(hdr);
+    if (CN && compact && pdirty) {
+      bool fits = true;
+#pragma unroll
+      for (int k = 0; k < N; ++k) {
+        if (PL) {
+          if (L.pdirty & (1u << (2 * k))) fits = fits && rgb_peers_fits(prow_get(L, PEER_MI(k, N)));
+          if (L.pdirty & (2u << (2 * k))) fits = fits && rgb_peers_fits(prow_get(L, PEER_NI(k, N)));
+        } else {
+          if (L.dmi & (1u << k)) fits = fits && rgb_peers_fits(L.pmi[k]);
+          if (L.dni & (1u << k)) fits = fits && rgb_peers_fits(L.pni[k]);
+          if (L.dcs & (1u << k)) fits = fits && rgb_peers_fits(L.pcs[k]);
+        }
+      }
+      if (L.dcs_ci) fits = fits && rgb_peers_fits(L.ci);
+      if (!fits) {
+        RGB_X_COUNT(2);
+#pragma unroll 1
+        for (unsigned k = 0; k < (unsigned)N; ++k) {
+          const unsigned q = 2u * (unsigned)N + k;
+          ST8(L.peers + q, (ldg8(TR, L.peers + (q >> 1)) >> (32u * (q & 1u))) & 0xFFFFFFFFull);
+        }
+#pragma unroll 1
+        for (unsigned k = (unsigned)N; k-- > 0u;) {
+          const u64 v = ldg8(TR, L.peers + k);
+          ST8(L.peers + 2u * k, v & 0xFFFFFFFFull); ST8(L.peers + 2u * k + 1u, v >> 32);
+        }
+#pragma unroll 1
+        for (unsigned w = 3u * (unsigned)N; w < 16u; ++w) ST8(L.peers + w, 0ull);
+        compact = false;
+      }
+    }
+    if (CN && compact) {
+      if (pdirty) {
+        u32 *p32 = reinterpret_cast<u32 *>(L.peers);
+#pragma unroll
+        for (int k = 0; k < N; ++k) {
+          if (PL) {
+            if (L.pdirty & (1u << (2 * k))) p32[2 * k] = (u32)prow_get(L, PEER_MI(k, N));
+            if (L.pdirty & (2u << (2 * k))) p32[2 * k + 1] = (u32)prow_get(L, PEER_NI(k, N));
+            if (L.dcs_ci & (1u << k)) p32[2 * N + k] = (u32)L.ci;
+          } else {
+            if (L.dmi & (1u << k)) p32[2 * k] = (u32)L.pmi[k];
+            if (L.dni & (1u << k)) p32[2 * k + 1] = (u32)L.pni[k];
+            if (L.dcs & (1u << k)) p32[2 * N + k] = (u32)L.pcs[k];
+            else if (L.dcs_ci & (1u << k)) p32[2 * N + k] = (u32)L.ci;
+          }
+        }
+      }
+      if (!PL && (L.flags & RGB_F_BECAME_LEADER) != 0u && !RGB_KNOB(dev, 1u)) {
+        ST8(L.peers + RGB_PEERS_HDR_WORD, rgb_peers_hdr(0u, 0ull) | RGB_PEERS_HDR_BUILD);
+      }
+    } else if (PL) {
+      if (L.pdirty | L.dcs_ci) {
+#pragma unroll
+        for (int w = 0; w < 2 * N; ++w)
+          if (L.pdirty & (1u << w)) ST8(L.peers + w, prow_get(L, (unsigned)w));
+#pragma unroll
+        for (int k = 0; k < N; ++k)
+          if (L.dcs_ci & (1u << k)) ST8(L.peers + PEER_CS(k, N), L.ci);
+      }
+    } else if (L.dmi | L.dni | L.dcs | L.dcs_ci) {
+#pragma unroll
+      for (int k = 0; k < N; ++k) {
+        if (L.dmi & (1u << k)) ST8(L.peers + PEER_MI(k, N), L.pmi[k]);
+        if (L.dni & (1u << k)) ST8(L.peers + PEER_NI(k, N), L.pni[k]);
+        if (L.dcs & (1u << k)) ST8(L.peers + PEER_CS(k, N), L.pcs[k]);
+        else if (L.dcs_ci & (1u << k)) ST8(L.peers + PEER_CS(k, N), L.ci);
+      }
     }
   }
   if (((pkhi0 >> (PK_PENDX_SH - 56)) & 1u) && !RGB_KNOB(dev, 1u)) {
@@ -2260,6 +2391,11 @@
       if (m1.x > wn[i]) { ni_new = m1.x; ni_dirty = true; }
     }
   }
+  bool row_compact = false;
+  if (rgb_peers_compact_n((unsigned)N) && PROW) {
+    row_compact = rgb_peers_hdr_compact(prow[7u ^ swz].y);
+    if (row_compact && !(rgb_peers_fits(mi_new) && rgb_peers_fits(ni_new))) return false;
+  }
   u64 v[N + 1]; bool use[N + 1]; int n = 1;
   v[N] = lwi; use[N] = true;
 #pragma unroll
@@ -2275,13 +2411,39 @@
     else {
       bool found = false;
       const ulonglong2 *rt = reinterpret_cast<const ulonglong2 *>(dev.runs + (size_t)server * dev.max_runs * 2u);
+      if (rgb_peers_compact_n((unsigned)N)) {
+        unsigned usable = 0;
+        if (rrow != nullptr) {
+          usable = (unsigned)rrow[7u ^ swz].x;
+#pragma unroll
+          for (unsigned j = 0; j < RGB_PEERS_MIRROR_MAX; ++j) {
+            if (!found && j < usable) {
+              const ulonglong2 r = rrow[j ^ swz];
+              if (p >= r.x) {
+                t = r.y; found = true;
+#ifdef RGB_X_MIRROR_CHECK
+                RGB_X_COUNT(0); rgb_x_mirror_check(TR, dev.runs + (size_t)server * dev.max_runs * 2u, (int)n_runs - 3 - (int)j, r);
+#endif
+              }
+            }
+          }
+#ifdef RGB_X_MIRROR_CHECK
+          if (!found) RGB_X_COUNT(1);
+#endif
+        }
+#pragma unroll 1
+        for (int k = (int)n_runs - 3 - (int)usable; k >= 0 && !found; --k) {
+          const ulonglong2 r = ldg16(TR, rt + k);
+          if (p >= r.x) { t = r.y; found = true; }
+        }
+      }
       const int lds_runs = rrow != nullptr ? RGB_RUNS_LDS : 0;
 #pragma unroll 1
-      for (int k = (int)n_runs - 3; k >= lds_runs && !found; --k) {
+      for (int k = (int)n_runs - 3; !rgb_peers_compact_n((unsigned)N) && k >= lds_runs && !found; --k) {
         const ulonglong2 r = ldg16(TR, rt + k);
         if (p >= r.x) { t = r.y; found = true; }
       }
-      if (rrow != nullptr) {
+      if (!rgb_peers_compact_n((unsigned)N) && rrow != nullptr) {
 #pragma unroll
         for (int k = RGB_RUNS_LDS - 1; k >= 0; --k) {
           if (!found && (unsigned)k + 3u <= n_runs) {
@@ -2300,7 +2462,10 @@
   if (t != UNDEF && t == ct) ci = p;
   if (ci > ci0) flags |= RGB_F_AUX_EVAL;
   if (ci > la) { const u64 to = li < ci ? li : ci; if (to >= la + 1) { nla = to; flags |= RGB_F_APPLIED; } }
-  if (mi_dirty | ni_dirty) ST16(reinterpret_cast<ulonglong2 *>(peers) + peer, make_ulonglong2(mi_new, ni_new));
+  if (mi_dirty | ni_dirty) {
+    if (row_compact) ST8(peers + peer, rgb_peers_pair(mi_new, ni_new));
+    else ST16(reinterpret_cast<ulonglong2 *>(peers) + peer, make_ulonglong2(mi_new, ni_new));
+  }
   if (ci != ci0 || nla != la)
     ST16(reinterpret_cast<ulonglong2 *>(dev.hot + (size_t)server * RGB_HOT_WORDS) + HOT_P_CI, make_ulonglong2(ci, nla));
   make_decision(out, server, RGB_ROLE_LEADER, RGB_NONE, 0, RGB_MSG_AER_REPLY, flags, 0, 0, 0, 0, 0, ci, nla);
@@ -2462,7 +2627,8 @@
   const bool lead_cls = rgb_lead_class(cls);
   constexpr bool PEERS_LDS = rgb_class_slice(1, (unsigned)N) == 32u;
   constexpr bool PEERS_WIDE = TR && rgb_train_class_slice(1, (unsigned)N) == 32u && !PEERS_LDS;
-  const bool RUNS_LDS = TR && RGB_TRAIN_RUNS_LDS && (PEERS_LDS || PEERS_WIDE) && dev.max_runs >= (u32)RGB_RUNS_LDS;
+  const bool RUNS_LDS = TR && RGB_TRAIN_RUNS_LDS && PEERS_WIDE && dev.max_runs >= (u32)RGB_RUNS_LDS;
+  constexpr bool MIRROR_LDS = TR && RGB_TRAIN_RUNS_LDS && PEERS_LDS;
   bool AER_RUNS = false;
 #if defined(RGB_X_TRAIN_TIMELINE) && !defined(RGB_HOST_EMULATION)
   u64 tt[7] = {0, 0, 0, 0, 0, 0, 0};
@@ -2612,19 +2778,68 @@
         glds16<ROWS>(reinterpret_cast<const ulonglong2 *>(dev.peers + (size_t)sj * 16u) + ((lane & 7u) ^ ((r >> 1) & 7u)),
                      io + (4 + k) * RGB_TICK_BLOCK);
       }
-      if (RUNS_LDS) {
-#pragma unroll
-        for (int k = 0; k < 4; ++k) {
-          const u32 r = 8 * k + (lane >> 3);
-          const u32 sj = __shfl(srv, (int)r, 64);
-          glds16<ROWS>(reinterpret_cast<const ulonglong2 *>(dev.runs + (size_t)sj * dev.max_runs * 2u) + ((lane & 7u) ^ ((r >> 1) & 7u)),
-                       io + (8 + k) * RGB_TICK_BLOCK);
+    }
+    glds_wait();
+  }
+  lds_barrier();
+  if (PEERS_LDS && lead_cls && active && sv < dev.n_servers) {
+    ulonglong2 *pw = io + 4 * RGB_TICK_BLOCK + lane * 8;
+    const unsigned sw = (lane >> 1) & 7u;
+    const u64 hdr = pw[7u ^ sw].y;
+    if (MIRROR_LDS) {
+      ulonglong2 *mw = io + 8 * RGB_TICK_BLOCK + lane * 8;
+      const u64 hpk = io[lane * 8 + (HOT_P_TERM ^ sw)].y, hprs = io[lane * 8 + (HOT_P_LRT ^ sw)].y;
+      const unsigned nr = (unsigned)pk_get(hpk, PK_NRUNS_SH, 5);
+      unsigned usable = rgb_peers_mirror_usable(hdr, (unsigned)pk_get(hpk, PK_ROLE_SH, 3), nr, hprs);
+      const u64 anchor_now = (nr >= 2u && rgb_peers_fits(hprs)) ? hprs : 0ull;
+      if (rgb_peers_hdr_compact(hdr) && pk_get(hpk, PK_ROLE_SH, 3) == RGB_ROLE_LEADER &&
+          ((hdr & RGB_PEERS_HDR_BUILD) || rgb_peers_hdr_anchor(hdr) != anchor_now)) {
+        u64 *prow_mem = dev.peers + (size_t)sv * 16u;
+        const ulonglong2 *rt = reinterpret_cast<const ulonglong2 *>(dev.runs + (size_t)sv * dev.max_runs * 2u);
+        const unsigned want = (nr >= 3u && rgb_peers_fits(hprs)) ? (nr - 2u < RGB_PEERS_MIRROR_MAX ? nr - 2u : RGB_PEERS_MIRROR_MAX) : 0u;
+        ulonglong2 rr[RGB_PEERS_MIRROR_MAX];
+#pragma unroll
+        for (unsigned j = 0; j < RGB_PEERS_MIRROR_MAX; ++j) rr[j] = j < want ? ldg16(TR, rt + (nr - 3u - j)) : make_ulonglong2(0, 0);
+        unsigned m = 0; bool open = true;
+#pragma unroll
+        for (unsigned j = 0; j < RGB_PEERS_MIRROR_MAX; ++j) {
+          open = open && j < want && rgb_peers_fits(rr[j].x) && rgb_peers_fits(rr[j].y);
+          if (open) { ST8(prow_mem + RGB_PEERS_MIRROR_WORD + j, rgb_peers_pair(rr[j].x, rr[j].y)); mw[j ^ sw] = rr[j]; m = j + 1u; }
         }
-      }
-    }
-    glds_wait();
-  }
-  lds_barrier();
+        const u64 nh = rgb_peers_hdr(m, anchor_now);
+        if (nh != hdr) ST8(prow_mem + RGB_PEERS_HDR_WORD, nh);
+        pw[7u ^ sw].y = nh;
+        usable = m;
+      } else if (usable != 0u) {
+#pragma unroll
+        for (unsigned q = 0; q < 4u; ++q) {
+          const ulonglong2 v = pw[(4u + q) ^ sw];
+          mw[(2u * q) ^ sw] = make_ulonglong2(v.x & 0xFFFFFFFFull, v.x >> 32);
+          if (q < 3u) mw[(2u * q + 1u) ^ sw] = make_ulonglong2(v.y & 0xFFFFFFFFull, v.y >> 32);
+        }
+      }
+      mw[7u ^ sw] = make_ulonglong2((u64)usable, (u64)(long long)((int)nr - 3));
+    }
+    if (rgb_peers_hdr_compact(hdr)) {
+      u64 w[16], ww[16];
+#pragma unroll
+      for (unsigned q = 0; q < 4u; ++q) { const ulonglong2 v = pw[q ^ sw]; w[2u * q] = v.x; w[2u * q + 1u] = v.y; }
+#pragma unroll
+      for (unsigned q = 8u; q < 16u; ++q) w[q] = 0;
+      w[RGB_PEERS_HDR_WORD] = hdr;
+#pragma unroll
+      for (unsigned q = 0; q < 16u; ++q) ww[q] = 0;
+#pragma unroll
+      for (unsigned i = 0; i < (unsigned)N; ++i) {
+        ww[PEER_MI(i, N)] = rgb_peers_mi(w, (unsigned)N, i); ww[PEER_NI(i, N)] = rgb_peers_ni(w, (unsigned)N, i);
+        ww[PEER_CS(i, N)] = rgb_peers_cs(w, (unsigned)N, i);
+      }
+      ww[RGB_PEERS_HDR_WORD] = hdr;
+#pragma unroll
+      for (unsigned q = 0; q < 8u; ++q)
+        if (2u * q < 3u * (unsigned)N) pw[q ^ sw] = make_ulonglong2(ww[2u * q], ww[2u * q + 1u]);
+    }
+  }
   RGB_TT(3);
   if (TR && RGB_X_TICKET_AT == 1 && ticket_ctr != nullptr) *next_ticket = rgb_take_ticket(ticket_ctr, ctl);
   const ulonglong2 *hrow = io + lane * 8;
@@ -2632,7 +2847,7 @@
   const ulonglong2 *prow = (PEERS_LDS && lead_cls) ? io + 4 * RGB_TICK_BLOCK + lane * 8
                            : (PEERS_WIDE && lead_cls) ? io + 4 * RGB_TICK_BLOCK + lane * 16 : nullptr;
   const ulonglong2 *rrow = (RUNS_LDS && PEERS_WIDE && lead_cls) ? io + 12 * RGB_TICK_BLOCK + lane * 8
-                           : ((RUNS_LDS && PEERS_LDS && lead_cls) || (!PEERS_LDS && AER_RUNS)) ? io + 8 * RGB_TICK_BLOCK + lane * 8 : nullptr;
+                           : ((MIRROR_LDS && lead_cls) || (!PEERS_LDS && AER_RUNS)) ? io + 8 * RGB_TICK_BLOCK + lane * 8 : nullptr;
 #ifndef RGB_HOST_EMULATION
   asm volatile("" ::"v"(pf0), "v"(pf1));
 #endif
@@ -3225,7 +3440,7 @@
       if (RGB_KNOB(dev, 128u) && v >= 75 && v < 80) v = 0;
       const int j = other(l, r >> 16);
       const u64 *pr = dev.peers + (size_t)sid(l) * dev.peer_stride;
-      const u64 mi = pr[PEER_MI(j, N)];
+      const u64 mi = rgb_peers_mi(pr, (unsigned)N, (unsigned)j);
       LaneT<false> T;
       syn_lane(T, ld, dev.runs + (size_t)sid(l) * dev.max_runs * 2);
       if (v < 75) {
@@ -3433,9 +3648,16 @@
     hot[HOT_PK] = pk;
   }
   u64 *pr = dev.peers + (size_t)s * dev.peer_stride;
-  for (unsigned i = 0; i < dev.peer_stride; ++i) pr[i] = 0;
-  for (unsigned i = 0; i < N; ++i) {
-    pr[PEER_MI(i, N)] = h.match_index[i]; pr[PEER_NI(i, N)] = h.next_index[i]; pr[PEER_CS(i, N)] = h.commit_index_sent[i];
+  if (rgb_peers_put_row(pr, N, h.match_index, h.next_index, h.commit_index_sent, dev.peer_stride)) {
+    unsigned m = 0;
+    if (nr >= 3u && rgb_peers_fits(prs)) {
+      for (unsigned j = 0; j < RGB_PEERS_MIRROR_MAX && j < nr - 2u; ++j) {
+        const u64 rs = runs[2 * (nr - 3u - j)], rt = runs[2 * (nr - 3u - j) + 1];
+        if (!(rgb_peers_fits(rs) && rgb_peers_fits(rt))) break;
+        pr[RGB_PEERS_MIRROR_WORD + j] = rgb_peers_pair(rs, rt); m = j + 1u;
+      }
+    }
+    pr[RGB_PEERS_HDR_WORD] = rgb_peers_hdr(m, (nr >= 2u && rgb_peers_fits(prs)) ? prs : 0ull);
   }
   u64 *cd = dev.cond + (size_t)s * 4;
   for (int i = 0; i < 4; ++i) cd[i] = h.cond_reply[i];
@@ -3459,7 +3681,7 @@
   for (int i = 0; i < 4; ++i) h.cond_reply[i] = cd[i];
   const u64 *pr = dev.peers + (size_t)s * dev.peer_stride;
   for (unsigned i = 0; i < N; ++i) {
-    h.match_index[i] = pr[PEER_MI(i, N)]; h.next_index[i] = pr[PEER_NI(i, N)]; h.commit_index_sent[i] = pr[PEER_CS(i, N)];
+    h.match_index[i] = rgb_peers_mi(pr, N, i); h.next_index[i] = rgb_peers_ni(pr, N, i); h.commit_index_sent[i] = rgb_peers_cs(pr, N, i);
   }
   unsigned nr = (unsigned)pk_get(pk, PK_NRUNS_SH, 5);
   const u64 *runs = dev.runs + (size_t)s * dev.max_runs * 2;
@@ -3573,7 +3795,7 @@
   x = fnv_word(x, (dev.qry + (size_t)s * RGB_QRY_WORDS)[QRY_MACVER]);
   const u64 *pr = dev.peers + (size_t)s * dev.peer_stride;
   for (unsigned i = 0; i < N; ++i) {
-    x = fnv_word(x, pr[PEER_MI(i, N)]); x = fnv_word(x, pr[PEER_NI(i, N)]); x = fnv_word(x, pr[PEER_CS(i, N)]);
+    x = fnv_word(x, rgb_peers_mi(pr, N, i)); x = fnv_word(x, rgb_peers_ni(pr, N, i)); x = fnv_word(x, rgb_peers_cs(pr, N, i));
   }
   const u64 *runs = dev.runs + (size_t)s * dev.max_runs * 2;
   for (unsigned r = 0; r < nr; ++r) { x = fnv_word(x, runs[2 * r]); x = fnv_word(x, runs[2 * r + 1]); }
```
